# lh3/pangene

Measured on AMD Instinct MI355X. Metric: M PAF hits/sec through filter+overlap+graph, higher is better.
Workload: dtype int32

## Files before the change

### pangene_amd/csrc/hip/k_branch.hpp

```cpp
#pragma once

struct InWalkX { const uint32_t *flags; __device__ __forceinline__ I32 operator()(int64_t i) const { return I32{(flags[i] & (PGA_F_FLT | PGA_F_SHADOW)) ? 0 : 1}; } };
struct OutRank {
	int32_t *rx; const uint32_t *flags;
	__device__ __forceinline__ void operator()(int64_t i, I32, I32 ex) const
	{
		rx[i] = ex.v | ((flags[i] & F_CSTIE) ? (int32_t)0x80000000 : 0);
	}
};

constexpr int RK_T = 1024;
__device__ __forceinline__ void rank_genome_body(const uint32_t *flags, const int32_t *goff, int32_t *rx, const int g, int (*wtot)[RK_T / WAVE])
{
	const int h0 = goff[g], h1 = goff[g + 1], tid = threadIdx.x, lane = tid & 63, w = tid >> 6;
	const unsigned long long lt = lane == 0 ? 0ull : (~0ull >> (64 - lane));
	int carry = 0, par = 0;
	for (int base = h0; base < h1; base += RK_T, par ^= 1) {
		const int i = base + tid;
		const uint32_t f = i < h1 ? flags[i] : (uint32_t)PGA_F_FLT;
		const unsigned long long m = __ballot(!(f & (PGA_F_FLT | PGA_F_SHADOW)));
		if (lane == 0) wtot[par][w] = __popcll(m);
		__syncthreads();
		int pre = carry, tot = 0;
#pragma unroll
		for (int k = 0; k < RK_T / WAVE; ++k) { const int t = wtot[par][k]; tot += t; if (k < w) pre += t; }
		if (i < h1) rx[i] = (pre + __popcll(m & lt)) | ((f & F_CSTIE) ? (int32_t)0x80000000 : 0);
		carry += tot;
	}
}
constexpr int RK_CHUNK = 2048;
template <int NT>
__device__ __forceinline__ void rank_chunk_body(const uint32_t *flags, const int32_t *goff, int32_t *rx, const int g, const int k, int (*wtot)[NT / WAVE])
{
	const int h0 = goff[g], h1 = goff[g + 1], tid = threadIdx.x, lane = tid & 63, w = tid >> 6;
	const int64_t lo64 = (int64_t)h0 + (int64_t)k * RK_CHUNK;
	if (lo64 >= h1) return;
	const int lo = (int)lo64, hi = h1 - lo > RK_CHUNK ? lo + RK_CHUNK : h1;
	int cnt = 0;
	for (int i = h0 + tid; i < lo; i += NT) cnt += !(flags[i] & (PGA_F_FLT | PGA_F_SHADOW));
	cnt = wave_sum(cnt);
	if (lane == 0) wtot[0][w] = cnt;
	__syncthreads();
	int carry = 0;
#pragma unroll
	for (int q = 0; q < NT / WAVE; ++q) carry += wtot[0][q];
	const unsigned long long lt = lane == 0 ? 0ull : (~0ull >> (64 - lane));
	int par = 1;
	for (int base = lo; base < hi; base += NT, par ^= 1) {
		const int i = base + tid;
		const uint32_t f = i < hi ? flags[i] : (uint32_t)PGA_F_FLT;
		const unsigned long long m = __ballot(!(f & (PGA_F_FLT | PGA_F_SHADOW)));
		if (lane == 0) wtot[par][w] = __popcll(m);
		__syncthreads();
		int pre = carry, tot = 0;
#pragma unroll
		for (int q = 0; q < NT / WAVE; ++q) { const int t = wtot[par][q]; tot += t; if (q < w) pre += t; }
		if (i < hi) rx[i] = (pre + __popcll(m & lt)) | ((f & F_CSTIE) ? (int32_t)0x80000000 : 0);
		carry += tot;
	}
}

__global__ __launch_bounds__(RK_T) void k_rank_genome(const uint32_t *flags, const int32_t *goff, int32_t *rx, Gate gate)
{
	__shared__ int wtot[2][RK_T / WAVE];
	if (gate_closed(gate)) return;
	rank_genome_body(flags, goff, rx, blockIdx.x, wtot);
}

constexpr int RP_FULL = 0, RP_COMPACT = 1, RP_WIDE = 2;
__global__ __launch_bounds__(BLOCK) void k_tie_bounds(const int4 *A, const uint32_t *flags, int n, int2 *tg)
{
	const int x = blockIdx.x * BLOCK + threadIdx.x;
	if (x >= n || !(flags[x] & F_CSTIE)) return;
	const int4 ah = A[x];
	int ta = x, tb = x + 1;
	while (ta > 0) { const int4 ap = A[ta - 1]; if (ap.y != ah.y || ap.x != ah.x) break; --ta; }
	while (tb < n) { const int4 ap = A[tb]; if (ap.y != ah.y || ap.x != ah.x) break; ++tb; }
	tg[x] = make_int2(ta, tb);
}

struct RepFill {
	const int2 *tg;
	int64_t n_ent; int GL, Q, N , NZ ; const int32_t *zx, *zy, *zg; const int2 *zst; const int32_t *zoff; const uint32_t *hbk; uint32_t tag;
	const int4 *A; const int32_t *gid; const uint32_t *flags; const int32_t *rx, *goff, *ctg_base;
	void *rp_out; int32_t *iv; int64_t *dcnt; int32_t *hz_list;
	const int32_t *vfirst; const int64_t *vbase;
	Gate gate;
};

template <int FORM>
__device__ __forceinline__ void rep_absent(const RepFill &a, int64_t e0, int n)
{
	for (int k = 0; k < n; ++k) {
		if (FORM == RP_COMPACT) ((int2 *)a.rp_out)[e0 + k] = make_int2(0, -1); else ((int4 *)a.rp_out)[e0 + k] = make_int4(-1, 0, 0, 0);
	}
}
template <int FORM>
__global__ __launch_bounds__(BLOCK) void k_rep_clear(void *rp_out, int64_t n_ent, Gate gate)
{
	if (gate_closed(gate)) return;
	const int64_t e = (int64_t)blockIdx.x * BLOCK + threadIdx.x;
	if (e >= n_ent) return;
	if (FORM == RP_COMPACT) ((int2 *)rp_out)[e] = make_int2(0, -1); else ((int4 *)rp_out)[e] = make_int4(-1, 0, 0, 0);
}

template <int FORM, bool CLEARED>
__device__ __forceinline__ void rep_fill_body(const RepFill &a, const int t)
{
	if (!CLEARED && t < a.Q && a.zoff[t] == a.zoff[t + 1]) rep_absent<FORM>(a, (int64_t)t * a.GL, a.GL);
	if (t >= a.NZ) return;
	const int z = t;
	const int g = a.zg[z], y = a.zy[z] & 0x7fffffff, j = y >> 1;
	const bool has_n = z + 1 < a.NZ;
	const int gn = has_n ? a.zg[z + 1] : -1, yn = has_n ? (a.zy[z + 1] & 0x7fffffff) : 0;
	const uint32_t kb = a.hbk[z];
	if (gn == g && (yn >> 1) == j) return;
	const int z0 = a.zoff[g], gj = a.goff[j], cb = a.ctg_base[j], xz = a.zx[z];
	const int2 st_z = a.zst[z];
	const int64_t e = (int64_t)g * a.GL + j;
	if (!CLEARED) {
		int gs = z;
		while (gs > z0 && ((a.zy[gs - 1] & 0x7fffffff) >> 1) == j) --gs;
		if (gs == z0 && j > 0) rep_absent<FORM>(a, (int64_t)g * a.GL, j);
		const int jn = gn == g ? (yn >> 1) : a.GL;
		if (jn > j + 1) rep_absent<FORM>(a, e + 1, jn - j - 1);
	}
	int q = z;
	if (!hx_walk(kb, a.tag)) {
		q = z - 1;
		while (q >= z0 && ((a.zy[q] & 0x7fffffff) >> 1) == j && !hx_walk(a.hbk[q], a.tag)) --q;
		if (q < z0 || ((a.zy[q] & 0x7fffffff) >> 1) != j) { if (!CLEARED) rep_absent<FORM>(a, e, 1); return; }
	}
	const int h = q == z ? xz : a.zx[q];
	const int2 st = q == z ? st_z : a.zst[q];
	const int rxh = a.rx[h], r = (rxh & 0x7fffffff) - (a.rx[gj] & 0x7fffffff);
	int ivl = 0;
	if (rxh < 0) {
		const int hi = a.goff[j + 1];
		const int2 tgb = a.tg[h];
		const int ta = tgb.x, tb = tgb.y;
		const int re = tb < hi ? (a.rx[tb] & 0x7fffffff) : (a.rx[tb - 1] & 0x7fffffff) + ((a.flags[tb - 1] & (PGA_F_FLT | PGA_F_SHADOW)) ? 0 : 1);
		const int nb = (rxh & 0x7fffffff) - (a.rx[ta] & 0x7fffffff), na = re - (rxh & 0x7fffffff) - 1;
		if (nb + na > 0) {
			bool same_gene = false;
			for (int p = ta; p < tb; ++p) same_gene = same_gene || (p != h && a.gid[p] == g && !(a.flags[p] & (PGA_F_FLT | PGA_F_SHADOW)));
			if (same_gene || nb > 0xffff || na > 0xffff) {
				atomicAdd((unsigned long long *)&a.dcnt[6], 1ull);
				hz_note(&a.dcnt[14], a.hz_list, st.y);
			} else ivl = nb << 16 | na;
		}
	}
	const int cmw = st.x | (ivl ? (int)0x80000000 : 0);
	if (FORM == RP_COMPACT) {
		((int2 *)a.rp_out)[e] = make_int2(cmw, (st.y - cb) << 20 | r);
		if (ivl) a.iv[e] = ivl;
	} else if (FORM == RP_WIDE) {
		const long long cm64 = (long long)st.x + a.vbase[st.y];
		((int4 *)a.rp_out)[e] = make_int4(a.vfirst[st.y], r | (ivl ? (int)0x80000000 : 0), (int)(unsigned)(unsigned long long)cm64, (int)((unsigned long long)cm64 >> 32));
		if (ivl) a.iv[e] = ivl;
	} else ((int4 *)a.rp_out)[e] = make_int4(st.y, r, cmw, ivl);
}
template <int FORM, bool CLEARED>
__global__ __launch_bounds__(BLOCK) void k_rep_fill(RepFill a)
{
	if (gate_closed(a.gate)) return;
	rep_fill_body<FORM, CLEARED>(a, blockIdx.x * BLOCK + threadIdx.x);
}

struct NLocalHz { const int32_t *iv; const int32_t *ctg_base; int64_t *dcnt; int32_t *list; };

__device__ __noinline__ bool nl_hazard(const NLocalHz &z, int cc, int iv1, int iv2, int seg1, int seg2, int local_count)
{
	const int lo = cc - (iv1 >> 16) - (iv2 & 0xffff), hi = cc + (iv1 & 0xffff) + (iv2 >> 16);
	const bool all_in = lo >= -local_count && hi <= local_count, all_out = hi < -local_count || lo > local_count;
	if (all_in || all_out) return true;
	atomicAdd((unsigned long long *)&z.dcnt[6], 1ull);
	if (iv1) hz_note(&z.dcnt[14], z.list, seg1);
	if (iv2) hz_note(&z.dcnt[14], z.list, seg2);
	return false;
}

constexpr int nl_lanes_for(int GL) { return GL <= 256 ? 16 : GL <= 640 ? 32 : 64; }

template <int FORM, int NL_LANES>
__global__ __launch_bounds__(BLOCK) void k_n_local(const int32_t *pairs, int64_t n_cap, const int64_t *np_dev, int GL, const void *rp_in,
                                                     int local_dist, int local_count, int frag_mode, int32_t *cnt, NLocalHz hz, Gate gate)
{
	constexpr int NL_PAIRS = WAVE / NL_LANES;
	constexpr unsigned long long NL_MASK = NL_LANES == 64 ? ~0ull : ((1ull << (NL_LANES & 63)) - 1);
	if (gate_closed(gate)) return;
	const int lane = threadIdx.x & 63, grp = lane / NL_LANES, sub = lane & (NL_LANES - 1);
	int64_t n_pair = np_dev ? *np_dev : n_cap;
	if (n_pair > n_cap) return;
	const int64_t stride = (int64_t)gridDim.x * (BLOCK / WAVE) * NL_PAIRS;
	for (int64_t k0 = ((int64_t)blockIdx.x * (BLOCK / WAVE) + (threadIdx.x >> 6)) * NL_PAIRS; k0 < n_pair; k0 += stride) {
		const int64_t k = k0 + grp;
		const bool have = k < n_pair;
		const int64_t kk = have ? k : n_pair - 1;
		const int64_t g1 = (int64_t)pairs[2 * kk] * GL, g2 = (int64_t)pairs[2 * kk + 1] * GL;
		int c = 0;
		bool open = have;
		for (int j0 = 0; j0 < GL; j0 += NL_LANES) {
			if (__ballot(open) == 0) break;
			const int j = j0 + sub;
			const bool in = open && j < GL;
			const int jj = j < GL ? j : 0;
			bool hit = false, sure = false;
			if (FORM == RP_WIDE) {
				const int4 a = ((const int4 *)rp_in)[g1 + jj], b = ((const int4 *)rp_in)[g2 + jj];
				const long long d = (long long)((unsigned long long)(unsigned)a.w << 32 | (unsigned)a.z) - (long long)((unsigned long long)(unsigned)b.w << 32 | (unsigned)b.z);
				const int cc = (a.y & 0x7fffffff) - (b.y & 0x7fffffff);
				const bool cmp = in && a.x >= 0 && b.x >= 0 && (frag_mode || a.x == b.x);
				const bool near = d >= -(long long)local_dist && d <= (long long)local_dist;
				hit = cmp && (near || (cc >= -local_count && cc <= local_count));
				sure = hit;
				if (cmp && !near && (a.y | b.y) < 0) sure = nl_hazard(hz, cc, a.y < 0 ? hz.iv[g1 + jj] : 0, b.y < 0 ? hz.iv[g2 + jj] : 0, a.x, b.x, local_count) && hit;
			} else if (FORM == RP_COMPACT) {
				const int2 a = ((const int2 *)rp_in)[g1 + jj], b = ((const int2 *)rp_in)[g2 + jj];
				const int d = (a.x & 0x7fffffff) - (b.x & 0x7fffffff);
				const int cc = (a.y & 0xfffff) - (b.y & 0xfffff);
				const bool cmp = in && (a.y | b.y) >= 0 && (frag_mode || ((a.y ^ b.y) >> 20) == 0);
				const bool near = d >= -local_dist && d <= local_dist;
				hit = cmp && (near || (cc >= -local_count && cc <= local_count));
				sure = hit;
				if (cmp && !near && (a.x | b.x) < 0)
					sure = nl_hazard(hz, cc, a.x < 0 ? hz.iv[g1 + jj] : 0, b.x < 0 ? hz.iv[g2 + jj] : 0, hz.ctg_base[jj] + (a.y >> 20), hz.ctg_base[jj] + (b.y >> 20), local_count) && hit;
			} else {
				const int4 a = ((const int4 *)rp_in)[g1 + jj], b = ((const int4 *)rp_in)[g2 + jj];
				const int d = (a.z & 0x7fffffff) - (b.z & 0x7fffffff);
				const int cc = a.y - b.y;
				const bool cmp = in && a.x >= 0 && b.x >= 0 && (frag_mode || a.x == b.x);
				const bool near = d >= -local_dist && d <= local_dist;
				hit = cmp && (near || (cc >= -local_count && cc <= local_count));
				sure = hit;
				if (cmp && !near && (a.z | b.z) < 0) sure = nl_hazard(hz, cc, a.w, b.w, a.x, b.x, local_count) && hit;
			}
			const unsigned long long mh = __ballot(hit), ms = __ballot(sure);
			c += __popcll((mh >> (grp * NL_LANES)) & NL_MASK);
			if ((ms >> (grp * NL_LANES)) & NL_MASK) open = false;
		}
		if (have && sub == 0) cnt[k] = c;
	}
}

__global__ __launch_bounds__(BLOCK) void k_br_prep(const uint64_t *ax, int64_t n_arc, const int32_t *seg_gid, int32_t *agid, int32_t *vs, int32_t *ve)
{
	int64_t i = (int64_t)blockIdx.x * BLOCK + threadIdx.x;
	if (i >= n_arc) return;
	const uint64_t x = ax[i];
	const uint32_t v = (uint32_t)(x >> 32);
	agid[i] = seg_gid[(uint32_t)x >> 1];
	if (i == 0 || (uint32_t)(ax[i - 1] >> 32) != v) vs[v] = (int32_t)i;
	if (i == n_arc - 1 || (uint32_t)(ax[i + 1] >> 32) != v) ve[v] = (int32_t)i + 1;
}

__global__ __launch_bounds__(BLOCK) void k_seg_gid(const int32_t *g2s, int Q, int n_seg, int32_t *seg_gid)
{
	int g = blockIdx.x * BLOCK + threadIdx.x;
	if (g < Q) { int s = g2s[g]; if (s >= 0 && s < n_seg) seg_gid[s] = g; }
}

__global__ __launch_bounds__(BLOCK) void k_cur_prep(const pga_arc_part_t *arcs, int64_t n_arc, const int32_t *seg_gid, uint64_t *ax, int32_t *s1, int32_t *agid,
                                                      int32_t *vs, int32_t *ve)
{
	int64_t i = (int64_t)blockIdx.x * BLOCK + threadIdx.x;
	if (i >= n_arc) return;
	const pga_arc_part_t a = arcs[i];
	const uint32_t v = (uint32_t)(a.x >> 32);
	ax[i] = a.x;
	s1[i] = (int32_t)((double)a.sum_s1 / a.n_genome + .499);
	agid[i] = seg_gid[(uint32_t)a.x >> 1];
	if (i == 0 || (uint32_t)(arcs[i - 1].x >> 32) != v) vs[v] = (int32_t)i;
	if (i == n_arc - 1 || (uint32_t)(arcs[i + 1].x >> 32) != v) ve[v] = (int32_t)i + 1;
}

__global__ __launch_bounds__(BLOCK) void k_curx_table(const pga_arc_part_t *arcs, const int64_t *n_dev, int64_t cap, const int32_t *seg_gid, int n_vtx, uint64_t *ax, int32_t *s1, int32_t *agid, uint8_t *aw,
                                                        int32_t *vs, int32_t *ve, int32_t *deg, uint8_t *vwk)
{
	const int64_t i = (int64_t)blockIdx.x * BLOCK + threadIdx.x, n_arc = *n_dev;
	if (i >= n_arc) {
		if (i < cap) return;
		const int64_t u = (n_arc ? (int64_t)(uint32_t)(arcs[n_arc - 1].x >> 32) + 1 : 0) + (i - cap);
		if (u < n_vtx) vs[u] = 0, ve[u] = 0, deg[u] = 0, vwk[u] = 0;
		return;
	}
	const pga_arc_part_t a = arcs[i];
	const uint32_t v = (uint32_t)(a.x >> 32);
	ax[i] = a.x;
	s1[i] = (int32_t)((double)a.sum_s1 / a.n_genome + .499);
	agid[i] = seg_gid[(uint32_t)a.x >> 1];
	aw[i] = 0;
	const int64_t pv = i ? (int64_t)(uint32_t)(arcs[i - 1].x >> 32) : -1;
	if (pv == (int64_t)v) return;
	int64_t e = i + 1;
	while (e < n_arc && (uint32_t)(arcs[e].x >> 32) == v) ++e;
	vs[v] = (int32_t)i, ve[v] = (int32_t)e, deg[v] = (int32_t)(e - i), vwk[v] = 0;
	for (int64_t u = pv + 1; u < (int64_t)v; ++u) vs[u] = 0, ve[u] = 0, deg[u] = 0, vwk[u] = 0;
}

__global__ __launch_bounds__(BLOCK) void k_deg(const int32_t *vs, const int32_t *ve, int n_vtx, int32_t *deg)
{
	int v = blockIdx.x * BLOCK + threadIdx.x;
	if (v < n_vtx) deg[v] = ve[v] - vs[v];
}

__device__ __forceinline__ int br_count_one(const int v, const int32_t *vs, const int32_t *ve, const int32_t *s1, const double bd)
{
	const int a0 = vs[v], n = ve[v] - a0;
	if (n < 2) return 0;
	int max_s1 = 0, n_max = 0, n_weak = 0;
	for (int i = 0; i < n; ++i) max_s1 = max_s1 > s1[a0 + i] ? max_s1 : s1[a0 + i];
	for (int i = 0; i < n; ++i) {
		n_max += s1[a0 + i] == max_s1;
		n_weak += (1.0 - (double)s1[a0 + i] / max_s1) > bd;
	}
	return n_max * n_weak + n * (n - 1) / 2;
}
__global__ __launch_bounds__(BLOCK) void k_br_count(int n_vtx, const int32_t *vs, const int32_t *ve, const int32_t *s1, double bd, int32_t *pc, Gate gate)
{
	const int v = blockIdx.x * BLOCK + threadIdx.x;
	if (v >= n_vtx || gate_closed(gate)) return;
	pc[v] = br_count_one(v, vs, ve, s1, bd);
}

constexpr int PO_THREADS = 1024, PO_MAX_ITEMS = 64;
__global__ __launch_bounds__(PO_THREADS) void k_pair_offsets(const int32_t *pc, int n, int32_t *poff, int64_t *dcnt, int64_t *host_box, long long cap , Gate gate)
{
	__shared__ int32_t part[PO_THREADS];
	if (gate_closed(gate)) return;
	const int t = threadIdx.x, per = (n + PO_THREADS - 1) / PO_THREADS, i0 = t * per, i1 = i0 + per < n ? i0 + per : n;
	int32_t s = 0;
	for (int i = i0; i < i1; ++i) s += pc[i];
	part[t] = s;
	__syncthreads();
	for (int d = 1; d < PO_THREADS; d <<= 1) {
		const int32_t v = t >= d ? part[t - d] : 0;
		__syncthreads();
		part[t] += v;
		__syncthreads();
	}
	int32_t run = part[t] - s;
	for (int i = i0; i < i1; ++i) { poff[i] = run; run += pc[i]; }
	if (t == PO_THREADS - 1) { dcnt[15] = part[t]; if (cap >= 0 && part[t] > cap) { dcnt[11] = 1; if (part[t] > dcnt[16]) dcnt[16] = part[t]; } }
	__syncthreads();
	if (t < 16) sys_store(&host_box[t], dcnt[t]);
}

template <int MODE>
__device__ void br_vertex_seq(int a0, int n, const int32_t *s1, const int32_t *agid, double bd, int64_t k, int32_t *pairs, const int32_t *cnt,
                              double bdist, double bcut, uint8_t *weak, int32_t *grp, int32_t *ndl_out, int64_t *dcnt)
{
	int max_s1 = 0;
	for (int i = 0; i < n; ++i) max_s1 = max_s1 > s1[a0 + i] ? max_s1 : s1[a0 + i];
	for (int i = 0; i < n; ++i) {
		const double r = 1.0 - (double)s1[a0 + i] / max_s1;
		if (!(r > bd)) continue;
		int n_local = 0;
		for (int j = 0; j < n; ++j) {
			if (s1[a0 + j] != max_s1) continue;
			if (MODE == 1) pairs[2 * k] = agid[a0 + j], pairs[2 * k + 1] = agid[a0 + i];
			if (MODE == 2) n_local += cnt[k];
			++k;
		}
		if (MODE == 2) {
			weak[a0 + i] = ((n_local == 0 && r > bdist) || r > bcut) ? 2 : 1;
			if (dcnt) atomicAdd((unsigned long long *)&dcnt[weak[a0 + i] - 1], 1ull);
		}
	}
	int n_group = 0;
	for (int i = 0; i < n; ++i) {
		if (MODE == 2 && grp[a0 + i] == 0) grp[a0 + i] = ++n_group;
		for (int j = i + 1; j < n; ++j) {
			if (MODE == 1) pairs[2 * k] = agid[a0 + i], pairs[2 * k + 1] = agid[a0 + j];
			if (MODE == 2 && cnt[k] > 0 && grp[a0 + j] == 0) grp[a0 + j] = grp[a0 + i];
			++k;
		}
	}
	if (MODE == 2) *ndl_out = n_group;
}

constexpr int BR_WIDE_CAP = 2048;
template <int MODE>
__device__ void br_vertex_wide(const int lane, int a0, int n, const int32_t *s1, const int32_t *agid, double bd, int64_t k0, int32_t *pairs, const int32_t *cnt,
                               double bdist, double bcut, uint8_t *weak, uint16_t *grp , int32_t *ndl_out, int64_t *dcnt)
{
	const unsigned long long lt = lane == 0 ? 0ull : (~0ull >> (64 - lane));
	int max_s1 = 0;
	for (int c = 0; c < n; c += WAVE) { const int j = c + lane; const int v = j < n ? s1[a0 + j] : 0; max_s1 = max_s1 > v ? max_s1 : v; }
	max_s1 = wave_max(max_s1);
	int n_max = 0;
	for (int c = 0; c < n; c += WAVE) { const int j = c + lane; n_max += __popcll(__ballot(j < n && s1[a0 + j] == max_s1)); }
	int64_t k = k0;
	for (int ci = 0; ci < n; ci += WAVE) {
		const int ii = ci + lane;
		const double r_l = ii < n ? 1.0 - (double)s1[a0 + ii] / max_s1 : 0.0;
		unsigned long long m_weak = __ballot(ii < n && r_l > bd);
		for (; m_weak; m_weak &= m_weak - 1, k += n_max) {
			const int bit = __ffsll((long long)m_weak) - 1, i = ci + bit;
			const int gid_i = agid[a0 + i];
			bool any_local = false;
			int base = 0;
			for (int cj = 0; cj < n; cj += WAVE) {
				const int j = cj + lane;
				const bool is_max = j < n && s1[a0 + j] == max_s1;
				const unsigned long long mm = __ballot(is_max);
				const int64_t kk = k + base + __popcll(mm & lt);
				if (MODE == 1) { if (is_max) pairs[2 * kk] = agid[a0 + j], pairs[2 * kk + 1] = gid_i; }
				else any_local = any_local || __ballot(is_max && cnt[kk] != 0) != 0;
				base += __popcll(mm);
			}
			if (MODE == 2 && lane == bit) {
				const int wk = ((!any_local && r_l > bdist) || r_l > bcut) ? 2 : 1;
				weak[a0 + i] = (uint8_t)wk;
				if (dcnt) atomicAdd((unsigned long long *)&dcnt[wk - 1], 1ull);
			}
		}
	}
	if (MODE == 2) { for (int j = lane; j < n; j += WAVE) grp[j] = 0; wave_sync(); }
	int n_group = 0;
	for (int i = 0; i < n; ++i) {
		const int64_t row = k + (int64_t)i * n - (int64_t)i * (i + 1) / 2 - i - 1;
		if (MODE == 1) {
			const int gid_i = agid[a0 + i];
			for (int j = i + 1 + lane; j < n; j += WAVE) pairs[2 * (row + j)] = gid_i, pairs[2 * (row + j) + 1] = agid[a0 + j];
		} else {
			int gi = grp[i];
			if (gi == 0) { gi = ++n_group; if (lane == 0) grp[i] = (uint16_t)gi; }
			for (int j = i + 1 + lane; j < n; j += WAVE) if (grp[j] == 0 && cnt[row + j] > 0) grp[j] = (uint16_t)gi;
			wave_sync();
		}
	}
	if (MODE == 2 && lane == 0) *ndl_out = n_group;
}

template <int MODE>
__device__ __forceinline__ void br_wave_body(const int v, const int lane, uint16_t *s_grp , const int64_t k0 , const int32_t *vs, const int32_t *ve, const int32_t *s1g, const int32_t *agidg, double bd,
                                             int32_t *pairs, int64_t pair_cap, const int32_t *pcnt, const int32_t *cnt, double bdist, double bcut,
                                             uint8_t *weak, int32_t *grpg, int32_t *ndl, int64_t *dcnt, uint8_t *vwk)
{
	const int a0 = vs[v], n = ve[v] - a0;
	if (n < 2) { if (MODE == 2 && lane == 0) ndl[v] = 0; return; }
	if (MODE == 1 && k0 + pcnt[v] > pair_cap) return;
	if (n > WAVE && n <= BR_WIDE_CAP) {
		int32_t g = 0;
		br_vertex_wide<MODE>(lane, a0, n, s1g, agidg, bd, k0, pairs, cnt, bdist, bcut, weak, MODE == 2 ? s_grp + (threadIdx.x >> 6) * BR_WIDE_CAP : (uint16_t *)nullptr, &g, dcnt);
		if (MODE == 2 && lane == 0) ndl[v] = g, vwk[v] = 1;
		return;
	}
	if (n > WAVE) {
		if (lane == 0) {
			int32_t g = 0;
			if (MODE == 2) for (int i = 0; i < n; ++i) grpg[a0 + i] = 0;
			br_vertex_seq<MODE>(a0, n, s1g, agidg, bd, k0, pairs, cnt, bdist, bcut, weak, grpg, &g, dcnt);
			if (MODE == 2) ndl[v] = g, vwk[v] = 1;
		}
		return;
	}
	const bool in = lane < n;
	const int my_s1 = in ? s1g[a0 + lane] : 0, my_gid = in ? agidg[a0 + lane] : 0;
	const int max_s1 = wave_max(my_s1);
	const double r = in ? 1.0 - (double)my_s1 / max_s1 : 0.0;
	const bool is_weak = in && r > bd, is_max = in && my_s1 == max_s1;
	const unsigned long long m_weak = __ballot(is_weak), m_max = __ballot(is_max);
	if (MODE == 2 && lane == 0 && m_weak) vwk[v] = 1;
	const unsigned long long lt = lane == 0 ? 0ull : (~0ull >> (64 - lane));
	const int n_max = __popcll(m_max), mrank = __popcll(m_max & lt);
	int wb = 0;
	for (unsigned long long m = m_weak; m; m &= m - 1, ++wb) {
		const int i = __ffsll((long long)m) - 1;
		const int gid_i = __builtin_amdgcn_readlane(my_gid, i);
		const int64_t k = k0 + (int64_t)wb * n_max + mrank;
		if (MODE == 1) { if (is_max) pairs[2 * k] = my_gid, pairs[2 * k + 1] = gid_i; }
		else {
			const bool none_local = __ballot(is_max && cnt[k] != 0) == 0;
			if (lane == i) {
				const int wk = ((none_local && r > bdist) || r > bcut) ? 2 : 1;
				weak[a0 + i] = (uint8_t)wk;
				if (dcnt) atomicAdd((unsigned long long *)&dcnt[wk - 1], 1ull);
			}
		}
	}
	const int64_t k2 = k0 + (int64_t)n_max * __popcll(m_weak);
	int grp = 0, n_group = 0;
	for (int i = 0; i < n; ++i) {
		const int64_t k = k2 + (int64_t)i * n - (int64_t)i * (i + 1) / 2 + (lane - i - 1);
		if (MODE == 1) {
			const int gid_i = __builtin_amdgcn_readlane(my_gid, i);
			if (lane > i && in) pairs[2 * k] = gid_i, pairs[2 * k + 1] = my_gid;
		} else {
			int gi = __builtin_amdgcn_readlane(grp, i);
			if (gi == 0) { gi = ++n_group; if (lane == i) grp = gi; }
			if (lane > i && in && grp == 0 && cnt[k] > 0) grp = gi;
		}
	}
	if (MODE == 2 && lane == 0) ndl[v] = n_group;
}
template <int MODE>
__global__ __launch_bounds__(BLOCK) void k_br_wave(int n_vtx, const int32_t *vs, const int32_t *ve, const int32_t *s1g, const int32_t *agidg, double bd,
                                                     const int32_t *poff, int32_t *pairs, int64_t pair_cap , const int32_t *pcnt , const int32_t *cnt, double bdist, double bcut,
                                                     uint8_t *weak, int32_t *grpg, int32_t *ndl, int64_t *dcnt, uint8_t *vwk ,
                                                     const int64_t *np_dev = nullptr , Gate gate = Gate{nullptr, 0})
{
	__shared__ uint16_t s_grp[MODE == 2 ? (BLOCK / WAVE) * BR_WIDE_CAP : 1];
	const int v = blockIdx.x * (BLOCK / WAVE) + (threadIdx.x >> 6), lane = threadIdx.x & 63;
	if (v >= n_vtx || gate_closed(gate)) return;
	if (MODE == 2 && np_dev && *np_dev > pair_cap) return;
	br_wave_body<MODE>(v, lane, s_grp, poff[v], vs, ve, s1g, agidg, bd, pairs, pair_cap, pcnt, cnt, bdist, bcut, weak, grpg, ndl, dcnt, vwk);
}

struct LoopFront {
	int n_vtx, nbc, GL; const int32_t *vs, *ve, *s1; double bd; int32_t *pc, *poff, *btot;
	const uint32_t *flags; const int32_t *goff; int32_t *rx;
	void *rp_out; int64_t n_ent; int clear_bytes;
	Gate gate;
};
__global__ __launch_bounds__(RK_T) void k_loop_front1(LoopFront a)
{
	__shared__ int wtot[2][RK_T / WAVE];
	if (gate_closed(a.gate)) return;
	const int b = blockIdx.x, tid = threadIdx.x;
	if (b < a.nbc) {
		const int v = b * RK_T + tid, lane = tid & 63, w = tid >> 6;
		const int pc = v < a.n_vtx ? br_count_one(v, a.vs, a.ve, a.s1, a.bd) : 0;
		const I32 incl = wave_scan_incl(I32{pc}, OpSum{}, lane);
		if (lane == 63) wtot[0][w] = incl.v;
		__syncthreads();
		int pre = 0, tot = 0;
#pragma unroll
		for (int k = 0; k < RK_T / WAVE; ++k) { const int t = wtot[0][k]; tot += t; if (k < w) pre += t; }
		if (v < a.n_vtx) a.pc[v] = pc, a.poff[v] = pre + incl.v - pc;
		if (tid == 0) a.btot[b] = tot;
	} else if (b < a.nbc + a.GL) {
		rank_genome_body(a.flags, a.goff, a.rx, b - a.nbc, wtot);
	} else {
		const int64_t e = (int64_t)(b - a.nbc - a.GL) * RK_T + tid;
		if (e < a.n_ent) { if (a.clear_bytes == 8) ((int2 *)a.rp_out)[e] = make_int2(0, -1); else ((int4 *)a.rp_out)[e] = make_int4(-1, 0, 0, 0); }
	}
}
struct LoopFront2 {
	int nb_rep, n_vtx, nbc; const int32_t *vs, *ve, *s1, *agid; double bd; int32_t *poff; const int32_t *btot, *pc; int32_t *pairs; int64_t pair_cap; int64_t *dcnt;
};
template <int FORM, bool CLEARED>
__global__ __launch_bounds__(BLOCK) void k_loop_front2(RepFill rf, LoopFront2 a)
{
	if (gate_closed(rf.gate)) return;
	if ((int)blockIdx.x < a.nb_rep) { rep_fill_body<FORM, CLEARED>(rf, blockIdx.x * BLOCK + threadIdx.x); return; }
	const int v = (blockIdx.x - a.nb_rep) * (BLOCK / WAVE) + (threadIdx.x >> 6), lane = threadIdx.x & 63;
	if (v >= a.n_vtx) return;
	const int part = lane < a.nbc ? a.btot[lane] : 0, bv = v / RK_T;
	const int base = wave_sum(lane < bv ? part : 0);
	const int64_t k0 = (int64_t)base + a.poff[v];
	if (lane == 0) a.poff[v] = (int32_t)k0;
	if (v == 0) {
		const int tot = wave_sum(part);
		if (lane == 0) { a.dcnt[15] = tot; if (tot > a.pair_cap) { a.dcnt[11] = 1; if (tot > a.dcnt[16]) a.dcnt[16] = tot; } }
	}
	br_wave_body<1>(v, lane, nullptr, k0, a.vs, a.ve, a.s1, a.agid, a.bd, a.pairs, a.pair_cap, a.pc, nullptr, 0.0, 0.0, nullptr, nullptr, nullptr, a.dcnt, nullptr);
}

__global__ __launch_bounds__(BLOCK) void k_round_filter(int S, const int32_t *seg_cnt, const int32_t *deg, const int32_t *ndl, int max_tot_cnt, int max_degree, int max_dist_loci, uint8_t *del)
{
	const int s = blockIdx.x * BLOCK + threadIdx.x;
	if (s >= S) return;
	const int l0 = ndl[2 * s], l1 = ndl[2 * s + 1];
	del[s] = (seg_cnt[S + s] > max_tot_cnt || deg[2 * s] > max_degree || deg[2 * s + 1] > max_degree || (l0 > l1 ? l0 : l1) > max_dist_loci) ? 1 : 0;
}

__global__ __launch_bounds__(BLOCK) void k_round_del(int S, const int32_t *ndl, int max_tot_cnt, int max_degree, int max_dist_loci, const int32_t *seg_gid, int32_t *g2s, int32_t *vs, int32_t *ve, int32_t *deg, int32_t *seg_cnt, uint8_t *vwk, uint8_t *alive, int4 *gmeta ,
                 int32_t *stamp = nullptr , int round = 0)
{
	const int s = blockIdx.x * BLOCK + threadIdx.x;
	if (s >= S || !alive[s]) return;
	const int l0 = ndl[2 * s], l1 = ndl[2 * s + 1];
	if (!(seg_cnt[S + s] > max_tot_cnt || deg[2 * s] > max_degree || deg[2 * s + 1] > max_degree || (l0 > l1 ? l0 : l1) > max_dist_loci)) return;
	alive[s] = 0;
	if (stamp) stamp[0] = round;
	g2s[seg_gid[s]] = -1;
	vs[2 * s] = ve[2 * s] = vs[2 * s + 1] = ve[2 * s + 1] = 0;
	deg[2 * s] = deg[2 * s + 1] = 0;
	seg_cnt[s] = seg_cnt[S + s] = 0;
	vwk[2 * s] = vwk[2 * s + 1] = 0;
	if (gmeta) gmeta[s] = make_int4(0, 0, 0, 0);
}

__device__ __forceinline__ int arc_weak(const uint64_t *ax, const uint8_t *aw, int64_t n, uint64_t x)
{
	int64_t lo = 0, hi = n;
	while (lo < hi) { int64_t mid = (lo + hi) >> 1; if (ax[mid] < x) lo = mid + 1; else hi = mid; }
	return (lo < n && ax[lo] == x) ? aw[lo] : 0;
}

__device__ __forceinline__ int arc_weak_v(const uint64_t *ax, const uint8_t *aw, const int32_t *vs, const int32_t *ve, uint32_t v, uint32_t w)
{
	const int e = ve[v];
	for (int i = vs[v]; i < e; i += 4) {
		const uint32_t t0 = (uint32_t)ax[i], t1 = i + 1 < e ? (uint32_t)ax[i + 1] : ~0u, t2 = i + 2 < e ? (uint32_t)ax[i + 2] : ~0u, t3 = i + 3 < e ? (uint32_t)ax[i + 3] : ~0u;
		const int k = t0 == w ? 0 : t1 == w ? 1 : t2 == w ? 2 : t3 == w ? 3 : -1;
		if (k >= 0) return aw[i + k];
	}
	return 0;
}

__global__ __launch_bounds__(BLOCK) void k_mark_hits(const int32_t *val, const int32_t *prev, const int4 *YA, const int4 *YB, const int32_t *g2s, int n,
                                                       const uint64_t *ax, const uint8_t *aw, int64_t n_arc, const int32_t *vs, const int32_t *ve, const uint8_t *vwk, int32_t *weak_new)
{
	int y = blockIdx.x * BLOCK + threadIdx.x;
	if (y >= n || val[y] < 0) return;
	int p = prev[y];
	if (p < 0) return;
	const int4 aA = YA[y], bA = YA[p];
	if (aA.x != bA.x) return;
	const int aw_ = YB[y].w, bw_ = YB[p].w;
	uint32_t w = (uint32_t)g2s[aA.y] << 1 | (uint32_t)(aw_ & 1);
	uint32_t v = (uint32_t)g2s[bA.y] << 1 | (uint32_t)(bw_ & 1);
	if (vwk && !vwk[v] && !vwk[w ^ 1]) return;
	int e1 = vs ? arc_weak_v(ax, aw, vs, ve, v, w) : arc_weak(ax, aw, n_arc, (uint64_t)v << 32 | w);
	if (e1) atomicMax(&weak_new[bw_ >> 1], e1);
	int e2 = vs ? arc_weak_v(ax, aw, vs, ve, w ^ 1, v ^ 1) : arc_weak(ax, aw, n_arc, (uint64_t)(w ^ 1) << 32 | (v ^ 1));
	if (e2) atomicMax(&weak_new[aw_ >> 1], e2);
}

__global__ __launch_bounds__(BLOCK) void k_weak_merge(uint32_t *flags, const int32_t *weak_new, int n, int64_t *cnt)
{
	int h = blockIdx.x * BLOCK + threadIdx.x;
	const bool in = h < n;
	if (!in) h = n - 1;
	uint32_t f = flags[h];
	int cur = in ? (int)((f & PGA_F_WEAK_MASK) >> PGA_F_WEAK_SHIFT) : 0, nw = in ? weak_new[h] : 0;
	if (nw > cur) { cur = nw; flags[h] = (f & ~PGA_F_WEAK_MASK) | (uint32_t)nw << PGA_F_WEAK_SHIFT; }
	if (cnt) {
		const unsigned long long m = __ballot(cur != 0);
		if (m && (threadIdx.x & 63) == (unsigned)__ffsll((long long)m) - 1) atomicAdd((unsigned long long *)cnt, (unsigned long long)__popcll(m));
	}
}
```

### pangene_amd/csrc/hip/k_genes.hpp

```cpp
#pragma once


__global__ __launch_bounds__(BLOCK) void k_zkey(const int32_t *gid, int n, uint64_t *key, uint32_t *val)
{
	int h = blockIdx.x * BLOCK + threadIdx.x;
	if (h < n) key[h] = (uint64_t)(uint32_t)gid[h], val[h] = (uint32_t)h;
}

struct InLiveX { const uint32_t *flags; __device__ __forceinline__ I32 operator()(int64_t i) const { return I32{(flags[i] & PGA_F_FLT) ? 0 : 1}; } };
struct OutLiveX {
	uint32_t *flags; int32_t *lx; const int32_t *gid; uint64_t *key; uint32_t *val; int64_t n;
	__device__ __forceinline__ void operator()(int64_t i, I32 in, I32 ex) const
	{
		const uint32_t f = flags[i], nf = (f & PGA_F_FLT) ? (f & ~F_MEMBER) : (f | F_MEMBER);
		if (nf != f) flags[i] = nf;
		lx[i] = ex.v;
		if (!(f & PGA_F_FLT)) key[ex.v] = (uint64_t)(uint32_t)gid[i], val[ex.v] = (uint32_t)i;
		if (i == n - 1) lx[n] = in.v;
	}
};
struct InLiveY { const uint32_t *flags; const int32_t *yperm; __device__ __forceinline__ I32 operator()(int64_t y) const { return I32{(flags[yperm[y]] & PGA_F_FLT) ? 0 : 1}; } };
struct OutLiveY {
	const uint32_t *flags; const int32_t *yperm; int32_t *ylist;
	__device__ __forceinline__ void operator()(int64_t y, I32, I32 ex) const { const int x = yperm[y]; if (!(flags[x] & PGA_F_FLT)) ylist[ex.v] = x; }
};
__global__ __launch_bounds__(BLOCK) void k_live_records(const uint32_t *flags, const int32_t *lx, const int4 *A, const int4 *B, const int4 *C, int n, int4 *cA, int4 *cB, int4 *cC, int32_t *cx)
{
	const int x = blockIdx.x * BLOCK + threadIdx.x;
	if (x >= n || !(flags[x] & F_MEMBER)) return;
	const int i = lx[x];
	cA[i] = A[x], cB[i] = B[x], cC[i] = C[x], cx[i] = x;
}
__global__ __launch_bounds__(BLOCK) void k_ovl_records(const int32_t *ov_pos, const int32_t *lpos, int64_t t, const int4 *A, const int4 *B, const int4 *C, int4 *cA, int4 *cB, int4 *cC, int32_t *cx)
{
	const int64_t k = (int64_t)blockIdx.x * BLOCK + threadIdx.x;
	if (k >= t || lpos[k] < 0) return;
	const int i = lpos[k], x = ov_pos[k];
	cA[i] = A[x], cB[i] = B[x], cC[i] = C[x], cx[i] = x;
}
struct InSegMaxListL { const int4 *A; const int32_t *lpos; __device__ __forceinline__ SegMax operator()(int64_t i) const { const int p = lpos[i]; if (p < 0) return SegMax{SEG_EMPTY, 0}; const int4 a = A[p]; return SegMax{a.y, a.z}; } };
struct OutSegMaxListL { int4 *A; const int32_t *lpos; __device__ __forceinline__ void operator()(int64_t i, SegMax in, SegMax) const { const int p = lpos[i]; if (p >= 0) ((int32_t *)&A[p])[3] = in.v; } };

__global__ void k_mail_live(const int32_t *lx, int64_t n, int64_t *dcnt, int64_t *host_box)
{
	if (threadIdx.x == 0) dcnt[10] = lx[n];
	__syncthreads();
	if (threadIdx.x < 16) sys_store(&host_box[threadIdx.x], dcnt[threadIdx.x]);
}

struct ZIndex { int32_t *zx, *zy, *zg; int2 *zst; int32_t *zpos; };
__global__ __launch_bounds__(BLOCK) void k_zrec(const uint32_t *perm, const uint64_t *ks, const int32_t *ctg_base, int n_genome, const uint32_t *flags, const int32_t *cm, const int32_t *seg, int n, ZIndex o)
{
	const int z = blockIdx.x * BLOCK + threadIdx.x, lane = threadIdx.x & 63;
	const bool v = z < n;
	const int x = v ? (int)perm[z] : 0;
	const int sg = v ? seg[x] : 0;
	const int gn = v ? genome_of(ctg_base, n_genome, sg) : -1;
	const unsigned long long kz = v ? ks[z] : ~0ull;
	int gn_p = __shfl_up(gn, 1, WAVE), gn_n = __shfl_down(gn, 1, WAVE);
	unsigned long long k_p = (unsigned long long)(unsigned)__shfl_up((int)(unsigned)(kz >> 32), 1, WAVE) << 32 | (unsigned)__shfl_up((int)(unsigned)kz, 1, WAVE);
	unsigned long long k_n = (unsigned long long)(unsigned)__shfl_down((int)(unsigned)(kz >> 32), 1, WAVE) << 32 | (unsigned)__shfl_down((int)(unsigned)kz, 1, WAVE);
	if (lane == 0) { const bool h = v && z > 0; k_p = h ? ks[z - 1] : ~0ull; gn_p = h ? genome_of(ctg_base, n_genome, seg[(int)perm[z - 1]]) : -1; }
	if (lane == 63) { const bool h = v && z + 1 < n; k_n = h ? ks[z + 1] : ~0ull; gn_n = h ? genome_of(ctg_base, n_genome, seg[(int)perm[z + 1]]) : -1; }
	if (!v) return;
	const bool grp_prev = z > 0 && k_p == kz && gn_p == gn, grp_next = z + 1 < n && k_n == kz && gn_n == gn;
	o.zx[z] = x, o.zg[z] = (int)kz;
	o.zy[z] = gn << 1 | ((flags[x] & PGA_F_REV) ? 1 : 0) | ((grp_prev || grp_next) ? 0 : (int)0x80000000);
	o.zst[z] = make_int2(cm[x], sg);
	o.zpos[x] = z;
}

__global__ __launch_bounds__(BLOCK) void k_zoff(const uint64_t *ks, int n, int Q, int32_t *zoff)
{
	int g = blockIdx.x * BLOCK + threadIdx.x;
	if (g > Q) return;
	int lo = 0, hi = n;
	while (lo < hi) { const int mid = (lo + hi) >> 1; if (ks[mid] < (uint64_t)g) lo = mid + 1; else hi = mid; }
	zoff[g] = lo;
}

struct WrecSrc { const int32_t *yperm, *seg, *gid, *cm, *sori, *sdom, *pdom0, *prot_gid; const uint32_t *flags; const int32_t *zpos; const int32_t *vfirst; const int64_t *vbase; };
__device__ __forceinline__ void pack_wrec_one(const WrecSrc &s, int64_t y, int4 *W)
{
	const int a = s.yperm[y], p0 = s.pdom0[a];
	int sg = s.seg[a], cmv = s.cm[a];
	if (s.vfirst) { cmv = (int)(unsigned)((unsigned long long)s.vbase[sg] + (unsigned long long)(long long)cmv); sg = s.vfirst[sg]; }
	W[2 * y] = make_int4(sg, s.gid[a] << 1 | ((s.flags[a] & PGA_F_REV) ? 1 : 0), cmv, s.sori[a]);
	W[2 * y + 1] = make_int4(s.sdom[a], p0 < 0 ? -1 : s.prot_gid[p0], s.zpos[a], 0);
}
__global__ __launch_bounds__(BLOCK) void k_pack_wrec(WrecSrc s, int n, int4 *W)
{
	const int y = blockIdx.x * BLOCK + threadIdx.x;
	if (y < n) pack_wrec_one(s, y, W);
}
__global__ __launch_bounds__(BLOCK) void k_pack_wrec_list(WrecSrc s, const int32_t *pos, int64_t T, int4 *W)
{
	const int64_t t = (int64_t)blockIdx.x * BLOCK + threadIdx.x;
	if (t < T && pos[t] >= 0) pack_wrec_one(s, pos[t], W);
}

constexpr int WK_FEW_FROM = 1 << 25;
struct Walk {
	const uint32_t *__restrict__ flags; const int32_t *__restrict__ yperm; const int4 *__restrict__ W; const int32_t *__restrict__ g2s;
	uint32_t *__restrict__ hfk, *__restrict__ hbk; int4 *__restrict__ hfp, *__restrict__ hbp;
	uint32_t tag; int ori; int n; int64_t *dcnt; int32_t *hz_list; Gate gate;
};
__device__ __forceinline__ int walk_score(const int4 w0, const int4 w1, int ori, const int32_t *g2s)
{
	return (ori || w0.w > w1.x || w1.y < 0 || g2s[w1.y] >= 0) ? w0.w : w1.x;
}
struct WalkRide { int n_ride, GL, cpg; const int32_t *goff; int32_t *rx; void *rp_out; int64_t n_clear; int clear_bytes; };
template <int WK_IPT>
__global__ __launch_bounds__(BLOCK) void k_walk(Walk a, WalkRide rd)
{
	constexpr int WK_TILE = BLOCK * WK_IPT;
	__shared__ int32_t s_wave[BLOCK / WAVE], s_carry;
	if (gate_closed(a.gate)) return;
	if ((int)blockIdx.x < rd.n_ride) {
		__shared__ int wtot[2][BLOCK / WAVE];
		const int b = (int)blockIdx.x;
		if (b < rd.GL * rd.cpg) rank_chunk_body<BLOCK>(a.flags, rd.goff, rd.rx, b / rd.cpg, b % rd.cpg, wtot);
		else {
			const int64_t e = (int64_t)(b - rd.GL * rd.cpg) * BLOCK + threadIdx.x;
			if (e < rd.n_clear) { if (rd.clear_bytes == 8) ((int2 *)rd.rp_out)[e] = make_int2(0, -1); else ((int4 *)rd.rp_out)[e] = make_int4(-1, 0, 0, 0); }
		}
		return;
	}
	const int tid = threadIdx.x, lane = tid & 63, w = tid >> 6;
	const int64_t tile0 = (int64_t)((int)blockIdx.x - rd.n_ride) * WK_TILE, base = tile0 + (int64_t)tid * WK_IPT;
	int mark[WK_IPT];
#pragma unroll
	for (int k = 0; k < WK_IPT; ++k) { const int64_t i = base + k; mark[k] = (i < a.n && !(a.flags[a.yperm[i]] & (PGA_F_FLT | PGA_F_SHADOW))) ? (int)i : -1; }
	if (w == 0) {
		int carry = -1;
		for (int64_t j0 = tile0 - 1; j0 >= 0 && carry < 0; j0 -= 64) {
			const int64_t j = j0 - lane;
			const bool ok = j >= 0 && !(a.flags[a.yperm[j]] & (PGA_F_FLT | PGA_F_SHADOW));
			const unsigned long long mk = __ballot(ok);
			if (mk) carry = (int)(j0 - (__ffsll((long long)mk) - 1));
		}
		if (lane == 0) s_carry = carry;
	}
	int t_max = mark[0];
#pragma unroll
	for (int k = 1; k < WK_IPT; ++k) t_max = t_max > mark[k] ? t_max : mark[k];
	I32 incl = wave_scan_incl(I32{t_max}, OpMax{}, lane);
	if (lane == 63) s_wave[w] = incl.v;
	__syncthreads();
	int run = s_carry;
	for (int k = 0; k < w; ++k) run = run > s_wave[k] ? run : s_wave[k];
	{ const int pv = incl.shfl_up(1).v; if (lane > 0) run = run > pv ? run : pv; }
	int prev[WK_IPT];
#pragma unroll
	for (int k = 0; k < WK_IPT; ++k) { prev[k] = run; run = mark[k] >= 0 ? mark[k] : run; }
	int4 A0[WK_IPT], A1[WK_IPT], B0[WK_IPT], B1[WK_IPT];
#pragma unroll
	for (int k = 0; k < WK_IPT; ++k) {
		const int i = mark[k] >= 0 ? mark[k] : 0, pp = prev[k] >= 0 ? prev[k] : i;
		if (mark[k] >= 0) A0[k] = a.W[2 * (int64_t)i], A1[k] = a.W[2 * (int64_t)i + 1], B0[k] = a.W[2 * (int64_t)pp], B1[k] = a.W[2 * (int64_t)pp + 1];
	}
	int SA[WK_IPT], SB[WK_IPT];
#pragma unroll
	for (int k = 0; k < WK_IPT; ++k)
		if (mark[k] >= 0 && prev[k] >= 0 && B0[k].x == A0[k].x) SA[k] = walk_score(A0[k], A1[k], a.ori, a.g2s), SB[k] = walk_score(B0[k], B1[k], a.ori, a.g2s);
#pragma unroll
	for (int k = 0; k < WK_IPT; ++k) {
		if (mark[k] < 0) continue;
		const int p = prev[k];
		const int4 a0 = A0[k], a1 = A1[k], b0 = B0[k], b1 = B1[k];
		const int zi = a1.z, zp = b1.z;
		uint32_t key = a.tag << HA_TAG_SHIFT | HA_NONE;
		if (p >= 0 && b0.x == a0.x) {
			const uint32_t wv = (uint32_t)a0.y, v = (uint32_t)b0.y;
			const int sa = SA[k], sb = SB[k], d = (int)((unsigned)a0.z - (unsigned)b0.z);
			if (a0.z == b0.z) { atomicAdd((unsigned long long *)&a.dcnt[5], 1ull); hz_note(&a.dcnt[14], a.hz_list, a0.x); }
			a.hfk[zp] = a.tag << HA_TAG_SHIFT | wv, a.hfp[zp] = make_int4(d, sb, sa, 0);
			key = a.tag << HA_TAG_SHIFT | (v ^ 1u), a.hbp[zi] = make_int4(d, sa, sb, 0);
		}
		a.hbk[zi] = key;
	}
}

__global__ __launch_bounds__(BLOCK) void k_walk_list(Walk a, const int32_t *pos, int64_t T)
{
	const int64_t t = (int64_t)blockIdx.x * BLOCK + threadIdx.x;
	if (t >= T) return;
	const int i = pos[t];
	if (i < 0) return;
	auto walkable = [&](int y) { return !(a.flags[a.yperm[y]] & (PGA_F_FLT | PGA_F_SHADOW)); };
	const int4 a0 = a.W[2 * (int64_t)i], a1 = a.W[2 * (int64_t)i + 1];
	const int zi = a1.z;
	if (!walkable(i)) { a.hbk[zi] = 0, a.hfk[zi] = 0; return; }
	int p = -1, q = -1;
	for (int j = i - 1; j >= 0; --j) { if (a.W[2 * (int64_t)j].x != a0.x) break; if (walkable(j)) { p = j; break; } }
	for (int j = i + 1; j < a.n; ++j) { if (a.W[2 * (int64_t)j].x != a0.x) break; if (walkable(j)) { q = j; break; } }
	const int sa = walk_score(a0, a1, a.ori, a.g2s);
	uint32_t key = a.tag << HA_TAG_SHIFT | HA_NONE;
	if (p >= 0) {
		const int4 b0 = a.W[2 * (int64_t)p], b1 = a.W[2 * (int64_t)p + 1];
		const int sb = walk_score(b0, b1, a.ori, a.g2s), d = (int)((unsigned)a0.z - (unsigned)b0.z);
		if (a0.z == b0.z) { atomicAdd((unsigned long long *)&a.dcnt[5], 1ull); hz_note(&a.dcnt[14], a.hz_list, a0.x); }
		key = a.tag << HA_TAG_SHIFT | ((uint32_t)b0.y ^ 1u), a.hbp[zi] = make_int4(d, sa, sb, 0);
	}
	a.hbk[zi] = key;
	if (q >= 0) {
		const int4 c0 = a.W[2 * (int64_t)q], c1 = a.W[2 * (int64_t)q + 1];
		const int sc = walk_score(c0, c1, a.ori, a.g2s), d = (int)((unsigned)c0.z - (unsigned)a0.z);
		a.hfk[zi] = a.tag << HA_TAG_SHIFT | (uint32_t)c0.y, a.hfp[zi] = make_int4(d, sa, sc, 0);
	} else a.hfk[zi] = 0;
}

constexpr int GA_CAP_WAVE = 128, GA_CAP = 512;
constexpr int GA_WAVE_HITS = 512;
constexpr int GA_BIG_STAGE = 2048;

struct GeneArcs {
	const int32_t *zy; const int32_t *zoff; const uint32_t *hfk, *hbk; const int4 *hfp, *hbp; const int32_t *g2s;
	int Q, S; uint32_t tag; int cap_log2;
	int32_t *seg_cnt, *seg_gid;
	pga_arc_part_t *stage; int4 *gmeta;
	uint64_t *ax; int32_t *s1, *agid; uint8_t *aw; int32_t *vs, *ve, *deg; uint8_t *vwk;
	int32_t *h_round;
	int32_t *big_list;
	int32_t *big_ctl;
	int64_t *dcnt;
	Gate gate; int32_t *tag_out;
};


template <int CAP, int STAGE> struct GeneTable {
	uint32_t key[CAP]; int32_t ng[CAP], tot[CAP]; unsigned long long sd[CAP], s1[CAP], s2[CAP]; uint16_t dense[CAP];
	int32_t zy[STAGE]; uint32_t fx[STAGE], bx[STAGE];
	int n_tot, n_gen, over, m, m0, base;
};

template <int CAP, int STAGE> struct GeneWin {
	const GeneArcs &a; const GeneTable<CAP, STAGE> &T; int lo, hi;
	__device__ __forceinline__ int zy(int z) const { return ((z >= lo && z < hi) ? T.zy[z - lo] : a.zy[z]) & 0x7fffffff; }
	__device__ __forceinline__ uint32_t fx(int z) const { return (z >= lo && z < hi) ? T.fx[z - lo] : a.hfk[z]; }
	__device__ __forceinline__ uint32_t bx(int z) const { return (z >= lo && z < hi) ? T.bx[z - lo] : a.hbk[z]; }
};

template <int CAP, class Table>
__device__ __forceinline__ bool ga_flush(Table &T, int cap, int cap_log2, uint32_t key, int ng, int tot, unsigned long long sd, unsigned long long s1, unsigned long long s2)
{
	uint32_t slot = (key * 2654435761u) >> (32 - cap_log2);
	int probes = 0;
	for (; probes < cap; ++probes, slot = (slot + 1) & (cap - 1)) {
		const uint32_t old = atomicCAS(&T.key[slot], 0xffffffffu, key);
		if (old == 0xffffffffu || old == key) break;
	}
	if (probes == cap) return false;
	atomicAdd(&T.ng[slot], ng); atomicAdd(&T.tot[slot], tot);
	atomicAdd(&T.sd[slot], sd); atomicAdd(&T.s1[slot], s1); atomicAdd(&T.s2[slot], s2);
	return true;
}

template <int NT, int CAP, int STAGE>
__device__ __forceinline__ bool gene_arcs_one(const GeneArcs &a, GeneTable<CAP, STAGE> &T, const int g, const int sid, const int tid, const int cap_log2)
{
	constexpr int HALO = STAGE >= 1024 ? 32 : 0;
	const int z0 = a.zoff[g], z1 = a.zoff[g + 1], cap = 1 << cap_log2;
	for (int k = tid; k < cap; k += NT) T.key[k] = 0xffffffffu, T.ng[k] = 0, T.tot[k] = 0, T.sd[k] = 0, T.s1[k] = 0, T.s2[k] = 0;
	if (tid == 0) T.n_tot = 0, T.n_gen = 0, T.over = 0, T.m = 0, T.m0 = 0;
	int n_tot = 0, n_gen = 0;
	uint32_t pk[2] = { 0xffffffffu, 0xffffffffu };
	int png[2] = { 0, 0 }, ptot[2] = { 0, 0 };
	unsigned long long psd[2] = { 0, 0 }, ps1[2] = { 0, 0 }, ps2[2] = { 0, 0 };
	for (int c0 = z0; c0 < z1; c0 += STAGE - 2 * HALO) {
		const int c1 = c0 + (STAGE - 2 * HALO) < z1 ? c0 + (STAGE - 2 * HALO) : z1;
		GeneWin<CAP, STAGE> W = { a, T, c0 - HALO > z0 ? c0 - HALO : z0, c1 + HALO < z1 ? c1 + HALO : z1 };
		if (NT == 64) wave_sync(); else __syncthreads();
		for (int z = W.lo + tid; z < W.hi; z += NT) T.zy[z - W.lo] = a.zy[z], T.fx[z - W.lo] = a.hfk[z], T.bx[z - W.lo] = a.hbk[z];
		if (NT == 64) wave_sync(); else __syncthreads();
		for (int z = c0 + tid; z < c1; z += NT) {
			if (!hx_walk(T.bx[z - W.lo], a.tag)) continue;
			const int zyw = T.zy[z - W.lo], zy = zyw & 0x7fffffff, genome = zy >> 1, rev = zy & 1;
			int gs = z, ge = z + 1;
			bool first = true;
			if (zyw >= 0) {
				while (gs > z0 && (W.zy(gs - 1) >> 1) == genome) --gs;
				while (ge < z1 && (W.zy(ge) >> 1) == genome) ++ge;
				for (int q = gs; q < z; ++q) first = first && !hx_walk(W.bx(q), a.tag);
			}
			n_tot += 1, n_gen += first ? 1 : 0;
#pragma unroll
			for (int dir = 0; dir < 2; ++dir) {
				const uint32_t hx = dir ? T.bx[z - W.lo] : T.fx[z - W.lo];
				if (!hx_valid(hx, a.tag)) continue;
				const uint32_t key = (uint32_t)(dir ? !rev : rev) << HA_TAG_SHIFT | (hx & HA_NONE);
				bool leader = true;
				int n = 1;
				for (int q = gs; q < ge && leader && ge - gs > 1; ++q) {
					if (q == z) continue;
					const int rq = W.zy(q) & 1;
#pragma unroll
					for (int d2 = 0; d2 < 2; ++d2) {
						const uint32_t ox = d2 ? W.bx(q) : W.fx(q);
						if (!hx_valid(ox, a.tag) || ((uint32_t)(d2 ? !rq : rq) << HA_TAG_SHIFT | (ox & HA_NONE)) != key) continue;
						if (q < z) { leader = false; break; }
						++n;
					}
				}
				if (!leader) continue;
				const int4 h = dir ? a.hbp[z] : a.hfp[z];
				int m1 = h.y, m2 = h.z;
				unsigned long long sd = (unsigned long long)(long long)h.x;
				if (n > 1)
					for (int q = z + 1; q < ge; ++q) {
						const int rq = W.zy(q) & 1;
#pragma unroll
						for (int d2 = 0; d2 < 2; ++d2) {
							const uint32_t ox = d2 ? W.bx(q) : W.fx(q);
							if (!hx_valid(ox, a.tag) || ((uint32_t)(d2 ? !rq : rq) << HA_TAG_SHIFT | (ox & HA_NONE)) != key) continue;
							const int4 o = d2 ? a.hbp[q] : a.hfp[q];
							sd += (unsigned long long)(long long)o.x, m1 = m1 > o.y ? m1 : o.y, m2 = m2 > o.z ? m2 : o.z;
						}
					}
				m1 = m1 > 0 ? m1 : 0, m2 = m2 > 0 ? m2 : 0;
				const int dg = cvt_i32_x86((double)sd / n + .499);
				if (key != pk[dir]) {
					if (pk[dir] != 0xffffffffu && !ga_flush<CAP>(T, cap, cap_log2, pk[dir], png[dir], ptot[dir], psd[dir], ps1[dir], ps2[dir])) T.over = 1;
					pk[dir] = key, png[dir] = 0, ptot[dir] = 0, psd[dir] = 0, ps1[dir] = 0, ps2[dir] = 0;
				}
				png[dir] += 1, ptot[dir] += n;
				psd[dir] += (unsigned long long)(long long)dg * (unsigned long long)n;
				ps1[dir] += (unsigned long long)(long long)m1, ps2[dir] += (unsigned long long)(long long)m2;
			}
		}
	}
#pragma unroll
	for (int dir = 0; dir < 2; ++dir)
		if (pk[dir] != 0xffffffffu && !ga_flush<CAP>(T, cap, cap_log2, pk[dir], png[dir], ptot[dir], psd[dir], ps1[dir], ps2[dir])) T.over = 1;
	{
		const int wt = wave_sum(n_tot), wg = wave_sum(n_gen);
		if ((tid & 63) == 0) { if (NT == 64) T.n_tot = wt, T.n_gen = wg; else atomicAdd(&T.n_tot, wt), atomicAdd(&T.n_gen, wg); }
	}
	if (NT == 64) wave_sync(); else __syncthreads();
	if (T.over) return false;
	for (int k = tid; k < cap; k += NT)
		if (T.key[k] != 0xffffffffu) { const int at = atomicAdd(&T.m, 1); T.dense[at] = (uint16_t)k; if (!(T.key[k] >> HA_TAG_SHIFT)) atomicAdd(&T.m0, 1); }
	if (NT == 64) wave_sync(); else __syncthreads();
	const int m = T.m;
	if (tid == 0) {
		const int b = 2 * z0, m0 = T.m0;
		T.base = b;
		a.seg_cnt[sid] = T.n_gen, a.seg_cnt[a.S + sid] = T.n_tot, a.seg_gid[sid] = g;
		a.gmeta[sid] = make_int4(b, m0, m - m0, 0);
		a.vs[2 * sid] = b, a.ve[2 * sid] = b + m0, a.vs[2 * sid + 1] = b + m0, a.ve[2 * sid + 1] = b + m;
		a.deg[2 * sid] = m0, a.deg[2 * sid + 1] = m - m0;
		a.vwk[2 * sid] = 0, a.vwk[2 * sid + 1] = 0;
		if (a.h_round) {
			a.h_round[sid] = T.n_gen, a.h_round[a.S + sid] = T.n_tot;
			a.h_round[2 * a.S + 2 * sid] = m0, a.h_round[2 * a.S + 2 * sid + 1] = m - m0;
		}
	}
	if (NT == 64) wave_sync(); else __syncthreads();
	for (int e = tid; e < m; e += NT) {
		const int k = T.dense[e];
		const uint32_t key = T.key[k];
		int r = 0;
		for (int j = 0; j < m; ++j) r += T.key[T.dense[j]] < key;
		pga_arc_part_t o;
		const uint32_t t = key & HA_NONE;
		o.x = (uint64_t)((uint32_t)sid << 1 | (key >> HA_TAG_SHIFT)) << 32 | (uint32_t)((uint32_t)a.g2s[t >> 1] << 1 | (t & 1u));
		o.n_genome = T.ng[k], o.tot_cnt = T.tot[k], o.sum_dist = T.sd[k], o.sum_s1 = (int64_t)T.s1[k], o.sum_s2 = (int64_t)T.s2[k];
		const int at = T.base + r;
		a.stage[at] = o;
		a.ax[at] = o.x;
		a.s1[at] = (int32_t)((double)o.sum_s1 / o.n_genome + .499);
		a.agid[at] = (int32_t)(t >> 1);
		a.aw[at] = 0;
	}
	return true;
}

constexpr int GA_WAVE_NT = 128;
template <int NT, int CAP, int HITS, int CAP_LOG2>
__global__ __launch_bounds__(NT) __attribute__((amdgpu_waves_per_eu(7))) void k_gene_arcs_wave_t(GeneArcs a, RepFill rf, int ride_form)
{
	__shared__ GeneTable<CAP, HITS> T;
	if (gate_closed(a.gate)) return;
	if ((int)blockIdx.x >= a.Q) {
		const int t = ((int)blockIdx.x - a.Q) * NT + (int)threadIdx.x;
		switch (ride_form) {
		case RP_FULL * 2: rep_fill_body<RP_FULL, false>(rf, t); break;
		case RP_FULL * 2 + 1: rep_fill_body<RP_FULL, true>(rf, t); break;
		case RP_COMPACT * 2: rep_fill_body<RP_COMPACT, false>(rf, t); break;
		case RP_COMPACT * 2 + 1: rep_fill_body<RP_COMPACT, true>(rf, t); break;
		case RP_WIDE * 2: rep_fill_body<RP_WIDE, false>(rf, t); break;
		case RP_WIDE * 2 + 1: rep_fill_body<RP_WIDE, true>(rf, t); break;
		}
		return;
	}
	const int g = blockIdx.x, tid = threadIdx.x;
	const int sid = a.g2s[g], z0 = a.zoff[g], z1 = a.zoff[g + 1];
	if (sid < 0) {
		for (int z = z0 + tid; z < z1; z += NT)
			if (hx_walk(a.hbk[z], a.tag)) atomicAdd((unsigned long long *)&a.dcnt[3], 1ull), a.dcnt[11] = 1;
		return;
	}
	const int cl = a.cap_log2 < CAP_LOG2 ? a.cap_log2 : CAP_LOG2;
	const bool done = z1 - z0 <= HITS && gene_arcs_one<NT, CAP, HITS>(a, T, g, sid, tid, cl);
	if (tid == 0 && !done) a.big_list[atomicAdd(&a.big_ctl[0], 1)] = g;
}

constexpr int GA_BIG_NT = 512;
__global__ __launch_bounds__(GA_BIG_NT) __attribute__((amdgpu_waves_per_eu(6))) void k_gene_arcs_big(GeneArcs a)
{
	__shared__ GeneTable<GA_CAP, GA_BIG_STAGE> T;
	if (gate_closed(a.gate)) return;
	if (a.tag_out && blockIdx.x == 0 && threadIdx.x == 0) *a.tag_out = (int32_t)a.tag;
	__shared__ int s_next;
	const int n_big = a.big_ctl[0];
	for (int at = blockIdx.x; at < n_big; ) {
		const int g = a.big_list[at];
		const int sid = a.g2s[g];
		if (!gene_arcs_one<GA_BIG_NT, GA_CAP, GA_BIG_STAGE>(a, T, g, sid, threadIdx.x, a.cap_log2) && threadIdx.x == 0)
			atomicAdd((unsigned long long *)&a.dcnt[9], 1ull), a.dcnt[11] = 1, a.gmeta[sid] = make_int4(0, 0, 0, 0);
		if (threadIdx.x == 0) s_next = (int)gridDim.x + atomicAdd(&a.big_ctl[1], 1);
		__syncthreads();
		at = s_next;
		__syncthreads();
	}
}

struct InGmeta { const int4 *gm; __device__ __forceinline__ I32 operator()(int64_t i) const { const int4 m = gm[i]; return I32{m.y + m.z}; } };

__global__ __launch_bounds__(BLOCK) void k_arc_compact(const int4 *gmeta, const int32_t *off, int S, const pga_arc_part_t *stage, pga_arc_part_t *arcs, int64_t *dcnt, int64_t *host_box)
{
	const int lane = threadIdx.x & 63;
	for (int sid = blockIdx.x * (BLOCK / WAVE) + (threadIdx.x >> 6); sid < S; sid += gridDim.x * (BLOCK / WAVE)) {
		const int4 m = gmeta[sid];
		const int o = off[sid], n = m.y + m.z;
		for (int i = lane; i < n; i += WAVE) arcs[o + i] = stage[m.x + i];
		if (lane == 0 && sid == S - 1) {
			dcnt[10] = o + n;
			for (int t = 0; t < 16; ++t) sys_store(&host_box[t], dcnt[t]);
		}
	}
}

struct I32x2 {
	int32_t a, b;
	__device__ __forceinline__ I32x2 shfl_up(int d) const { return I32x2{__shfl_up(a, d, WAVE), __shfl_up(b, d, WAVE)}; }
	__device__ __forceinline__ I32x2 shfl(int l) const { return I32x2{__shfl(a, l, WAVE), __shfl(b, l, WAVE)}; }
};
struct OpSum2 { __device__ __forceinline__ I32x2 operator()(I32x2 x, I32x2 y) const { return I32x2{x.a + y.a, x.b + y.b}; } };
struct InAliveGmeta { const uint8_t *alive; const int4 *gm; __device__ __forceinline__ I32x2 operator()(int64_t i) const { const int4 m = gm[i]; return I32x2{alive[i] != 0, m.y + m.z}; } };
struct OutExclI32x2 { int32_t *pa, *pb; __device__ __forceinline__ void operator()(int64_t i, I32x2, I32x2 ex) const { pa[i] = ex.a, pb[i] = ex.b; } };

__device__ __forceinline__ int4 arc_final_lo(uint64_t x, const pga_arc_part_t &p) { return make_int4((int32_t)(uint32_t)x, (int32_t)(uint32_t)(x >> 32), p.n_genome, p.tot_cnt); }
__device__ __forceinline__ int4 arc_final_hi(const pga_arc_part_t &p)
{
	return make_int4(cvt_i64lo_x86((double)(int64_t)p.sum_dist / p.tot_cnt + .499), cvt_i32_x86((double)p.sum_s1 / p.n_genome + .499), cvt_i32_x86((double)p.sum_s2 / p.n_genome + .499), 0);
}

__global__ __launch_bounds__(BLOCK) void k_arc_final(const int4 *gmeta, const int32_t *off, const int32_t *newid, int S, const pga_arc_part_t *stage, int4 *out, int64_t cap, int64_t *dcnt)
{
	const int lane = threadIdx.x & 63;
	const int4 ml = gmeta[S - 1];
	const int64_t total = (int64_t)off[S - 1] + ml.y + ml.z;
	if (blockIdx.x == 0 && threadIdx.x == 0) dcnt[10] = total;
	if (total > cap) return;
	for (int sid = blockIdx.x * (BLOCK / WAVE) + (threadIdx.x >> 6); sid < S; sid += gridDim.x * (BLOCK / WAVE)) {
		const int4 m = gmeta[sid];
		const int o = off[sid], n = m.y + m.z;
		for (int i = lane; i < n; i += WAVE) {
			const pga_arc_part_t p = stage[m.x + i];
			const uint32_t v = (uint32_t)(p.x >> 32), w = (uint32_t)p.x;
			const uint32_t sv = v >> 1, sw = w >> 1;
			const uint64_t x = (uint64_t)((uint32_t)(sv < (uint32_t)S ? newid[sv] : 0) << 1 | (v & 1u)) << 32 | ((uint32_t)(sw < (uint32_t)S ? newid[sw] : 0) << 1 | (w & 1u));
			out[2 * (size_t)(o + i)] = arc_final_lo(x, p);
			out[2 * (size_t)(o + i) + 1] = arc_final_hi(p);
		}
	}
}

__global__ void k_arc_final_probe(const pga_arc_part_t *in, int64_t n, int4 *out)
{
	const int64_t i = (int64_t)blockIdx.x * BLOCK + threadIdx.x;
	if (i < n) out[i] = arc_final_hi(in[i]);
}

__global__ __launch_bounds__(BLOCK) void k_xs_compact(const int4 *gmeta, const int32_t *off, int S, const pga_arc_part_t *stage, const int32_t *seg_cnt, int32_t *slot, int64_t arc_cap, const int64_t *dcnt, Gate gate = Gate{nullptr, 0},
                                                        const int32_t *stamp = nullptr , int round = 0)
{
	if (blockIdx.x == 0 && threadIdx.x == 0) slot[3] = (stamp && stamp[1] == round) ? 1 : 0;
	if (gate_closed(gate)) return;
	const int lane = threadIdx.x & 63;
	int32_t *segc = slot + XS_HDR;
	pga_arc_part_t *arcs = (pga_arc_part_t *)(slot + XS_HDR + xs_seg_words(S));
	for (int sid = blockIdx.x * (BLOCK / WAVE) + (threadIdx.x >> 6); sid < S; sid += gridDim.x * (BLOCK / WAVE)) {
		const int4 m = gmeta[sid];
		const int o = off[sid], n = m.y + m.z;
		if ((int64_t)o + n <= arc_cap)
			for (int i = lane; i < n; i += WAVE) arcs[o + i] = stage[m.x + i];
		if (lane == 0) {
			segc[sid] = seg_cnt[sid], segc[S + sid] = seg_cnt[S + sid];
			if (sid == S - 1) { slot[0] = o + n, slot[1] = dcnt[9] != 0, slot[2] = dcnt[3] != 0; for (int t = 4; t < XS_HDR; ++t) slot[t] = 0; }
		}
	}
}

__global__ __launch_bounds__(BLOCK) void k_mark_hits_z(const int32_t *zx, const int32_t *zy, const int32_t *zg, const uint32_t *hfk, const uint32_t *hbk, uint32_t tag, int n, const int32_t *g2s,
                                                        const uint64_t *ax, const uint8_t *aw, const int32_t *vs, const int32_t *ve, const uint8_t *vwk,
                                                        uint32_t *flags, int64_t *cnt, int then_filter, Gate gate, int32_t *stamp , int round)
{
	int z = blockIdx.x * BLOCK + threadIdx.x;
	bool marked = false;
	if (gate_closed(gate)) return;
	if (z < n) {
		const uint32_t kb = hbk[z], kf = hfk[z];
		const int y = zy[z], g = zg[z];
		if (hx_walk(kb, tag)) {
			const int sid = g2s[g], rev = y & 1;
			int nw = 0;
#pragma unroll
			for (int dir = 0; dir < 2; ++dir) {
				const uint32_t h = dir ? kb : kf;
				if (!hx_valid(h, tag) || sid < 0) continue;
				const uint32_t u = (uint32_t)sid << 1 | (uint32_t)(dir ? !rev : rev), t = h & HA_NONE;
				if (!vwk[u]) continue;
				const uint32_t w = (uint32_t)g2s[t >> 1] << 1 | (t & 1u);
				const int e = arc_weak_v(ax, aw, vs, ve, u, w);
				nw = nw > e ? nw : e;
			}
			if (nw) {
				const int x = zx[z];
				const uint32_t f = flags[x];
				if (nw > (int)((f & PGA_F_WEAK_MASK) >> PGA_F_WEAK_SHIFT)) {
					flags[x] = (f & ~PGA_F_WEAK_MASK) | (uint32_t)nw << PGA_F_WEAK_SHIFT | ((then_filter && nw == 2) ? PGA_F_FLT : 0u);
					if (stamp) stamp[1] = round;
				}
				marked = true;
			}
		}
		if (cnt && !marked) marked = (flags[zx[z]] & PGA_F_WEAK_MASK) != 0;
	}
	if (cnt) {
		const unsigned long long mk = __ballot(marked);
		if (mk && (threadIdx.x & 63) == (unsigned)__ffsll((long long)mk) - 1) atomicAdd((unsigned long long *)cnt, (unsigned long long)__popcll(mk));
	}
}
```

### pangene_amd/csrc/hip/pga_host_branch.hpp

```cpp
#pragma once


struct RepDefer { bool on; RepFill rf; int32_t *rx; unsigned nb; bool cleared; int rode; };

static int rep_pos_impl(pga_ctx *c, RepDefer *df)
{
	const int N = c->N, GL = c->n_genome, Q = c->Q;
	if (df) df->on = false, df->rode = 0;
	const int64_t n_ent = (int64_t)Q * GL;
	RepFill rf; int32_t *rx;
	TRY(rep_fill_args(c, &rf, &rx));
	int4 *rp = (int4 *)rf.rp_out;
	if (N) {
		I32 *tile = (I32 *)c->pool.get(S_TILE, tile_buf_bytes(N));
		if (!tile) return PGA_ERR_NOMEM;
		const int want = c->ride_want;
		c->ride_want = 0;
		TRY(ensure_half_arcs(c, c->ha_ori < 0 ? 0 : c->ha_ori));
		c->ride_want = want;
		TRY(rep_fill_args(c, &rf, &rx));
		static const bool rank_scan = env_has("PANGENE_RANK", "scan");
		const bool defer = df && c->gs_np <= (1 << 15) && !rank_scan;
		const int rode = (defer && c->in_loop && c->ride_done && c->ride_tag == c->round_tag && c->tg_valid) ? c->ride_done : 0;
		if (defer) ;
		else if (c->gs_np <= (1 << 15) && !rank_scan) hipLaunchKernelGGL(k_rank_genome, dim3((unsigned)GL), dim3(RK_T), 0, c->st, (const uint32_t *)c->flags, (const int32_t *)c->goff, rx, c->gate);
		else device_scan<I32>(InWalkX{c->flags}, OutRank{rx, c->flags}, N, tile, OpSum{}, I32{0}, c->st, c->gate);
		if (!c->tg_valid) { hipLaunchKernelGGL(k_tie_bounds, dim3(nblk(N)), dim3(BLOCK), 0, c->st, (const int4 *)c->recA, (const uint32_t *)c->flags, N, c->tg); c->tg_valid = true; }
		if (defer) { df->on = true, df->rf = rf, df->rx = rx, df->cleared = c->live_on, df->nb = nblk(c->live_on ? std::max(c->NL, 1) : std::max(c->NL, Q)), df->rode = rode; return 0; }
		if (c->live_on) {
			const unsigned nb = nblk(std::max(c->NL, 1));
			if (c->rp_form == RP_COMPACT) {
				if (n_ent) hipLaunchKernelGGL((k_rep_clear<RP_COMPACT>), dim3(nblk(n_ent)), dim3(BLOCK), 0, c->st, (void *)rp, n_ent, c->gate);
				hipLaunchKernelGGL((k_rep_fill<RP_COMPACT, true>), dim3(nb), dim3(BLOCK), 0, c->st, rf);
			} else {
				if (n_ent) hipLaunchKernelGGL((k_rep_clear<RP_FULL>), dim3(nblk(n_ent)), dim3(BLOCK), 0, c->st, (void *)rp, n_ent, c->gate);
				if (c->rp_form == RP_WIDE) hipLaunchKernelGGL((k_rep_fill<RP_WIDE, true>), dim3(nb), dim3(BLOCK), 0, c->st, rf);
				else hipLaunchKernelGGL((k_rep_fill<RP_FULL, true>), dim3(nb), dim3(BLOCK), 0, c->st, rf);
			}
		} else {
			const unsigned nb = nblk(std::max(c->NL, Q));
			if (c->rp_form == RP_COMPACT) hipLaunchKernelGGL((k_rep_fill<RP_COMPACT, false>), dim3(nb), dim3(BLOCK), 0, c->st, rf);
			else if (c->rp_form == RP_WIDE) hipLaunchKernelGGL((k_rep_fill<RP_WIDE, false>), dim3(nb), dim3(BLOCK), 0, c->st, rf);
			else hipLaunchKernelGGL((k_rep_fill<RP_FULL, false>), dim3(nb), dim3(BLOCK), 0, c->st, rf);
		}
	} else if (n_ent) {
		hipLaunchKernelGGL(k_fill_i32, dim3(nblk(4 * n_ent)), dim3(BLOCK), 0, c->st, (int32_t *)rp, 4 * n_ent, -1);
	}
	return 0;
}

extern "C" int pga_rep_pos(pga_ctx_t *c) { return rep_pos_impl(c, nullptr); }

static int n_local_dev(pga_ctx *c, const int32_t *d_pairs, int64_t n, const int64_t *np_dev, int32_t local_dist, int32_t local_count, int32_t frag_mode, int32_t **cnt)
{
	int32_t *d_cnt = (int32_t *)c->pool.get(S_NLCNT, sizeof(int32_t) * (size_t)n + 16);
	int4 *rp = (int4 *)c->pool.get(S_RP_SEG, 0);
	if (!d_cnt || !rp) return PGA_ERR_NOMEM;
	*cnt = d_cnt;
	NLocalHz hz = { (const int32_t *)c->pool.get(S_RP_IV, 0), c->ctg_base, c->dcnt, (int32_t *)c->pool.get(S_HZLIST, sizeof(int32_t) * PGA_HAZARD_CAP) };
	if (!hz.iv || !hz.list) return PGA_ERR_NOMEM;
	const int64_t est = np_dev ? (c->br_np_seen > 0 ? c->br_np_seen : std::min<int64_t>(n, 1 << 18)) : n;
	static const int lanes_env = [] { const char *e = getenv("PANGENE_NL_LANES"); return e ? atoi(e) : 0; }();
	const int lanes = (lanes_env == 16 || lanes_env == 32 || lanes_env == 64) ? lanes_env : nl_lanes_for(c->n_genome);
	const unsigned grid = (unsigned)std::max<int64_t>(1, std::min<int64_t>(nblk(est, BLOCK / WAVE * (WAVE / lanes)), 1 << 20));
#define NL_LAUNCH(FORM, LANES) hipLaunchKernelGGL((k_n_local<FORM, LANES>), dim3(grid), dim3(BLOCK), 0, c->st, d_pairs, n, np_dev, c->n_genome, (const void *)rp, local_dist, local_count, frag_mode, d_cnt, hz, c->gate)
#define NL_FORM(FORM) do { if (lanes == 16) NL_LAUNCH(FORM, 16); else if (lanes == 32) NL_LAUNCH(FORM, 32); else NL_LAUNCH(FORM, 64); } while (0)
	if (n && c->rp_form == RP_COMPACT) NL_FORM(RP_COMPACT);
	else if (n && c->rp_form == RP_WIDE) NL_FORM(RP_WIDE);
	else if (n) NL_FORM(RP_FULL);
#undef NL_FORM
#undef NL_LAUNCH
	return 0;
}

extern "C" int pga_n_local(pga_ctx_t *c, const int32_t *pairs, int64_t n, int32_t local_dist, int32_t local_count, int32_t frag_mode, int32_t **cnt)
{
	int32_t *d_pairs = (int32_t *)c->pool.get(S_PAIRS, sizeof(int32_t) * 2 * (size_t)n + 16);
	if (!d_pairs) return PGA_ERR_NOMEM;
	if (n) TRY(upload(c, d_pairs, pairs, 2 * (size_t)n));
	TRY(n_local_dev(c, d_pairs, n, nullptr, local_dist, local_count, frag_mode, cnt));
	return sync_st(c);
}

static inline bool loop_cap_forced(const pga_ctx *c) { static const bool on = getenv("PANGENE_LOOP_PAIR_CAP") != nullptr; return on && c->in_loop && !c->loop_room_given; }
static inline size_t loop_btot_at(int n_vtx) { return ((size_t)n_vtx + 7) & ~(size_t)3; }

static void rep_launch_deferred(pga_ctx *c, const RepDefer &d)
{
	const RepFill &rf = d.rf;
	if (d.rode >= 2) return;
	if (d.rode == 0) hipLaunchKernelGGL(k_rank_genome, dim3((unsigned)rf.GL), dim3(RK_T), 0, c->st, rf.flags, rf.goff, d.rx, rf.gate);
	const int form = c->rp_form;
	if (d.cleared) {
		if (d.rode) ;
		else if (rf.n_ent && form == RP_COMPACT) hipLaunchKernelGGL((k_rep_clear<RP_COMPACT>), dim3(nblk(rf.n_ent)), dim3(BLOCK), 0, c->st, rf.rp_out, rf.n_ent, rf.gate);
		else if (rf.n_ent) hipLaunchKernelGGL((k_rep_clear<RP_FULL>), dim3(nblk(rf.n_ent)), dim3(BLOCK), 0, c->st, rf.rp_out, rf.n_ent, rf.gate);
		if (form == RP_COMPACT) hipLaunchKernelGGL((k_rep_fill<RP_COMPACT, true>), dim3(d.nb), dim3(BLOCK), 0, c->st, rf);
		else if (form == RP_WIDE) hipLaunchKernelGGL((k_rep_fill<RP_WIDE, true>), dim3(d.nb), dim3(BLOCK), 0, c->st, rf);
		else hipLaunchKernelGGL((k_rep_fill<RP_FULL, true>), dim3(d.nb), dim3(BLOCK), 0, c->st, rf);
	} else {
		if (form == RP_COMPACT) hipLaunchKernelGGL((k_rep_fill<RP_COMPACT, false>), dim3(d.nb), dim3(BLOCK), 0, c->st, rf);
		else if (form == RP_WIDE) hipLaunchKernelGGL((k_rep_fill<RP_WIDE, false>), dim3(d.nb), dim3(BLOCK), 0, c->st, rf);
		else hipLaunchKernelGGL((k_rep_fill<RP_FULL, false>), dim3(d.nb), dim3(BLOCK), 0, c->st, rf);
	}
}

static int branch_enumerate(pga_ctx *c, int32_t **cnt, const RepDefer *df = nullptr)
{
	const int n_vtx = 2 * c->br_S;
	int32_t *s1 = (int32_t *)c->pool.get(S_BR_S1, 0), *agid = (int32_t *)c->pool.get(S_BR_GID, 0), *vs = (int32_t *)c->pool.get(S_BR_VS, 0), *ve = (int32_t *)c->pool.get(S_BR_VE, 0);
	int32_t *poff = (int32_t *)c->pool.get(S_BR_POFF, 0);
	int32_t *pairs = (int32_t *)c->pool.get(S_PAIRS, sizeof(int32_t) * 2 * (size_t)c->br_cap + 16);
	if (!pairs || !s1 || !agid || !vs || !ve || !poff) return PGA_ERR_NOMEM;
	if (df) {
		const int32_t *pc = (const int32_t *)c->pool.get(S_BR_PC, 0);
		const unsigned nb_rep = df->rode >= 2 ? 0u : df->nb;
		const LoopFront2 a = { (int)nb_rep, n_vtx, (n_vtx + RK_T - 1) / RK_T, vs, ve, s1, agid, c->br_par.diff, poff, pc + loop_btot_at(n_vtx), pc, pairs, c->br_cap, c->dcnt };
		const dim3 grid(nb_rep + nblk(n_vtx, BLOCK / WAVE));
		const int form = c->rp_form;
		if (df->cleared) {
			if (form == RP_COMPACT) hipLaunchKernelGGL((k_loop_front2<RP_COMPACT, true>), grid, dim3(BLOCK), 0, c->st, df->rf, a);
			else if (form == RP_WIDE) hipLaunchKernelGGL((k_loop_front2<RP_WIDE, true>), grid, dim3(BLOCK), 0, c->st, df->rf, a);
			else hipLaunchKernelGGL((k_loop_front2<RP_FULL, true>), grid, dim3(BLOCK), 0, c->st, df->rf, a);
		} else {
			if (form == RP_COMPACT) hipLaunchKernelGGL((k_loop_front2<RP_COMPACT, false>), grid, dim3(BLOCK), 0, c->st, df->rf, a);
			else if (form == RP_WIDE) hipLaunchKernelGGL((k_loop_front2<RP_WIDE, false>), grid, dim3(BLOCK), 0, c->st, df->rf, a);
			else hipLaunchKernelGGL((k_loop_front2<RP_FULL, false>), grid, dim3(BLOCK), 0, c->st, df->rf, a);
		}
	} else
	hipLaunchKernelGGL((k_br_wave<1>), dim3(nblk(n_vtx, BLOCK / WAVE)), dim3(BLOCK), 0, c->st, n_vtx, vs, ve, s1, agid, c->br_par.diff, poff, pairs, c->br_cap, (const int32_t *)c->pool.get(S_BR_PC, 0),
	                   (const int32_t *)nullptr, 0.0, 0.0, (uint8_t *)nullptr, (int32_t *)nullptr, (int32_t *)nullptr, c->dcnt, (uint8_t *)nullptr, (const int64_t *)nullptr, c->gate);
	return n_local_dev(c, pairs, c->br_cap, c->dcnt + 15, c->br_par.local_dist, c->br_par.local_count, c->br_par.frag_mode, cnt);
}

static int branch_pairs_impl(pga_ctx *c, const uint64_t *arc_x, const int32_t *arc_s1, int64_t n_arc, const int32_t *seg_gid, int32_t n_seg,
                             double branch_diff, int32_t local_dist, int32_t local_count, int32_t frag_mode, int32_t **cnt, int64_t *n_pairs, const RepDefer *df)
{
	if (arc_x == nullptr) n_arc = c->br_n, n_seg = c->br_S;
	const int n_vtx = 2 * n_seg;
	uint64_t *ax = (uint64_t *)c->pool.get(S_ARCX, sizeof(uint64_t) * (size_t)n_arc + 16);
	uint8_t *aw = (uint8_t *)c->pool.get(S_ARCW, (size_t)n_arc + 16);
	int32_t *s1 = (int32_t *)c->pool.get(S_BR_S1, sizeof(int32_t) * (size_t)n_arc + 16), *agid = (int32_t *)c->pool.get(S_BR_GID, sizeof(int32_t) * (size_t)n_arc + 16);
	int32_t *vs = (int32_t *)c->pool.get(S_BR_VS, sizeof(int32_t) * (size_t)n_vtx + 16), *ve = (int32_t *)c->pool.get(S_BR_VE, sizeof(int32_t) * (size_t)n_vtx + 16);
	int32_t *pc = (int32_t *)c->pool.get(S_BR_PC, sizeof(int32_t) * (loop_btot_at(n_vtx) + 64) + 16), *poff = (int32_t *)c->pool.get(S_BR_POFF, sizeof(int32_t) * (size_t)n_vtx + 16);
	int32_t *sg = (int32_t *)c->pool.get(S_BR_SEGGID, sizeof(int32_t) * (size_t)n_seg + 16);
	if (!ax || !aw || !s1 || !agid || !vs || !ve || !pc || !poff || !sg) return PGA_ERR_NOMEM;
	c->br_n = n_arc, c->br_S = n_seg, c->br_np = -1;
	c->br_par.diff = branch_diff, c->br_par.local_dist = local_dist, c->br_par.local_count = local_count, c->br_par.frag_mode = frag_mode;
	if (n_pairs) *n_pairs = 0;
	*cnt = (int32_t *)c->pool.get(S_NLCNT, 16);
	if (df && !df->on) df = nullptr;
	if (n_arc == 0 || n_vtx == 0) { if (df) rep_launch_deferred(c, *df); c->br_np = 0; return sync_st(c); }
	if (arc_x) {
		TRY(upload(c, ax, arc_x, (size_t)n_arc)); TRY(upload(c, s1, arc_s1, (size_t)n_arc)); TRY(upload(c, sg, seg_gid, (size_t)n_seg));
		HIPCHK(hipMemsetAsync(vs, 0, sizeof(int32_t) * (size_t)n_vtx, c->st)); HIPCHK(hipMemsetAsync(ve, 0, sizeof(int32_t) * (size_t)n_vtx, c->st));
		hipLaunchKernelGGL(k_br_prep, dim3(nblk(n_arc)), dim3(BLOCK), 0, c->st, ax, n_arc, sg, agid, vs, ve);
		HIPCHK(hipMemsetAsync(aw, 0, (size_t)n_arc, c->st));
	}
	static const bool general_scan = getenv("PANGENE_PAIR_SCAN_GENERAL") != nullptr;
	const bool one_wg = n_vtx <= PO_THREADS * PO_MAX_ITEMS && !general_scan;
	if (df && !(one_wg && n_pairs == nullptr)) { rep_launch_deferred(c, *df); df = nullptr; }
	if (df) {
		const int nbc = (n_vtx + RK_T - 1) / RK_T;
		const RepFill &rf = df->rf;
		const int64_t n_clear = (df->cleared && !df->rode) ? rf.n_ent : 0;
		const int gl = df->rode ? 0 : rf.GL;
		const LoopFront a = { n_vtx, nbc, gl, vs, ve, s1, branch_diff, pc, poff, pc + loop_btot_at(n_vtx), rf.flags, rf.goff, df->rx, rf.rp_out, n_clear, c->rp_form == RP_COMPACT ? 8 : 16, c->gate };
		hipLaunchKernelGGL(k_loop_front1, dim3((unsigned)(nbc + gl + (n_clear + RK_T - 1) / RK_T)), dim3(RK_T), 0, c->st, a);
		if (c->br_cap < 4 * (int64_t)n_vtx && !loop_cap_forced(c)) c->br_cap = 4 * (int64_t)n_vtx;
		return branch_enumerate(c, cnt, df);
	}
	hipLaunchKernelGGL(k_br_count, dim3(nblk(n_vtx)), dim3(BLOCK), 0, c->st, n_vtx, vs, ve, s1, branch_diff, pc, c->gate);
	if (one_wg) hipLaunchKernelGGL(k_pair_offsets, dim3(1), dim3(PO_THREADS), 0, c->st, (const int32_t *)pc, n_vtx, poff, c->dcnt, c->h_box, n_pairs ? -1ll : loop_cap_forced(c) ? (long long)c->br_cap : (long long)std::max<int64_t>(c->br_cap, 4 * (int64_t)n_vtx), c->gate);
	else {
		I32 *tile = (I32 *)c->pool.get(S_TILE, tile_buf_bytes(n_vtx));
		device_scan<I32>(InI32{pc}, OutExclI32{poff}, n_vtx, tile, OpSum{}, I32{0}, c->st, c->gate);
		hipLaunchKernelGGL(k_mail_pairs, dim3(1), dim3(64), 0, c->st, poff + (n_vtx - 1), pc + (n_vtx - 1), c->dcnt, c->h_box);
	}
	if (n_pairs) {
		TRY(sync_st(c));
		c->br_np = c->h_cnt[15], *n_pairs = c->br_np;
		c->br_cap = std::max<int64_t>(c->br_cap, std::max<int64_t>(c->br_np, 16));
		return c->br_np ? branch_enumerate(c, cnt) : 0;
	}
	if (c->br_cap < 4 * (int64_t)n_vtx && !loop_cap_forced(c)) c->br_cap = 4 * (int64_t)n_vtx;
	return branch_enumerate(c, cnt);
}

extern "C" int pga_branch_pairs(pga_ctx_t *c, const uint64_t *arc_x, const int32_t *arc_s1, int64_t n_arc, const int32_t *seg_gid, int32_t n_seg,
                                double branch_diff, int32_t local_dist, int32_t local_count, int32_t frag_mode, int32_t **cnt, int64_t *n_pairs)
{
	return branch_pairs_impl(c, arc_x, arc_s1, n_arc, seg_gid, n_seg, branch_diff, local_dist, local_count, frag_mode, cnt, n_pairs, nullptr);
}

struct RoundFilter { int on; int32_t max_tot_cnt, max_degree, max_dist_loci; uint8_t *del_host; };

static int decide_impl(pga_ctx *c, double branch_diff, double branch_diff_dist, double branch_diff_cut, uint8_t *arc_weak,
                       int32_t *n_dist_loci, int64_t *n_flt1, int64_t *n_flt2, const RoundFilter *rf)
{
	const int n_vtx = 2 * c->br_S, S = c->br_S;
	const int64_t n_arc = c->br_n;
	if (n_flt1) *n_flt1 = 0;
	if (n_flt2) *n_flt2 = 0;
	if (n_arc == 0 || n_vtx == 0) {
		if (n_vtx && n_dist_loci) memset(n_dist_loci, 0, sizeof(int32_t) * (size_t)n_vtx);
		if (rf && rf->on && S) memset(rf->del_host, 0, (size_t)S);
		return rf ? sync_st(c) : 0;
	}
	uint8_t *aw = (uint8_t *)c->pool.get(S_ARCW, 0);
	int32_t *s1 = (int32_t *)c->pool.get(S_BR_S1, 0), *agid = (int32_t *)c->pool.get(S_BR_GID, 0), *vs = (int32_t *)c->pool.get(S_BR_VS, 0), *ve = (int32_t *)c->pool.get(S_BR_VE, 0);
	int32_t *poff = (int32_t *)c->pool.get(S_BR_POFF, 0);
	int32_t *grp = (int32_t *)c->pool.get(S_BR_GRP, sizeof(int32_t) * (size_t)n_arc + 16);
	uint8_t *vwk = (uint8_t *)c->pool.get(S_VWK, (size_t)n_vtx + 16);
	const size_t need = sizeof(int32_t) * (size_t)n_vtx + 64;
	if (c->h_ndl_cap < need) {
		if (c->h_ndl) HIPCHK(hipStreamSynchronize(c->st));
		c->h_ndl = (int32_t *)c->pin.get(need + need / 2);
		if (!c->h_ndl) return PGA_ERR_NOMEM;
		c->h_ndl_cap = need + need / 2;
	}
	int32_t *ndl_dev = nullptr;
	HIPCHK(hipHostGetDevicePointer((void **)&ndl_dev, c->h_ndl, 0));
	int32_t *ndl_out = ndl_dev;
	if (rf) {
		ndl_out = (int32_t *)c->pool.get(S_BR_NDL, sizeof(int32_t) * (size_t)n_vtx + 16);
		if (!ndl_out) return PGA_ERR_NOMEM;
	}
	if (!grp || !vwk) return PGA_ERR_NOMEM;
	for (int attempt = 0;; ++attempt) {
		int32_t *cnt = (int32_t *)c->pool.get(S_NLCNT, 0);
		if (n_flt1 || n_flt2) HIPCHK(hipMemsetAsync(c->dcnt, 0, 2 * sizeof(int64_t), c->st));
		hipLaunchKernelGGL((k_br_wave<2>), dim3(nblk(n_vtx, BLOCK / WAVE)), dim3(BLOCK), 0, c->st, n_vtx, vs, ve, s1, agid, branch_diff, poff, (int32_t *)nullptr, (int64_t)c->br_cap, (const int32_t *)nullptr, cnt,
		                   branch_diff_dist, branch_diff_cut, aw, grp, ndl_out, (n_flt1 || n_flt2) ? c->dcnt : (int64_t *)nullptr, vwk, c->br_np < 0 ? c->dcnt + 15 : (const int64_t *)nullptr);
		if (rf && rf->on)
			hipLaunchKernelGGL(k_round_filter, dim3(nblk(S)), dim3(BLOCK), 0, c->st, S, (const int32_t *)c->pool.get(S_SEGCNT, 0), (const int32_t *)c->pool.get(S_DEG, 0), (const int32_t *)ndl_out,
			                   rf->max_tot_cnt, rf->max_degree, rf->max_dist_loci, (uint8_t *)ndl_dev);
		if (arc_weak && !c->table_sparse) HIPCHK(hipMemcpyAsync(arc_weak, aw, (size_t)n_arc, hipMemcpyDeviceToHost, c->st));
		if (n_flt1 || n_flt2) hipLaunchKernelGGL(k_mail_flush, dim3(1), dim3(64), 0, c->st, c->dcnt, c->h_box);
		TRY(sync_st(c));
		if (c->br_np >= 0 || c->h_cnt[15] <= c->br_cap || attempt) { if (c->br_np < 0) c->br_np = c->h_cnt[15]; c->br_np_seen = c->br_np; break; }
		c->br_cap = c->h_cnt[15] + c->h_cnt[15] / 2;
		HIPCHK(hipMemsetAsync(aw, 0, (size_t)n_arc, c->st)); HIPCHK(hipMemsetAsync(vwk, 0, (size_t)n_vtx, c->st));
		int32_t *dummy;
		TRY(branch_enumerate(c, &dummy));
	}
	if (n_dist_loci && !rf) memcpy(n_dist_loci, c->h_ndl, sizeof(int32_t) * (size_t)n_vtx);
	if (rf && rf->on) memcpy(rf->del_host, c->h_ndl, (size_t)S);
	if (n_flt1) *n_flt1 = c->h_cnt[0];
	if (n_flt2) *n_flt2 = c->h_cnt[1];
	return 0;
}

extern "C" int pga_branch_decide(pga_ctx_t *c, double branch_diff, double branch_diff_dist, double branch_diff_cut, uint8_t *arc_weak,
                                 int32_t *n_dist_loci, int64_t *n_flt1, int64_t *n_flt2)
{
	if (n_dist_loci == nullptr) return PGA_ERR_ARG;
	return decide_impl(c, branch_diff, branch_diff_dist, branch_diff_cut, arc_weak, n_dist_loci, n_flt1, n_flt2, nullptr);
}

extern "C" int pga_branch_decide_filter(pga_ctx_t *c, double branch_diff, double branch_diff_dist, double branch_diff_cut, int32_t do_filter,
                                        int32_t max_tot_cnt, int32_t max_degree, int32_t max_dist_loci, uint8_t *del)
{
	if (!(c->arc_deferred && !c->arc_done && c->table_sparse) || c->br_S != c->n_seg || (do_filter && del == nullptr)) return 2;
	RoundFilter rf = { do_filter, max_tot_cnt, max_degree, max_dist_loci, del };
	return decide_impl(c, branch_diff, branch_diff_dist, branch_diff_cut, nullptr, nullptr, nullptr, nullptr, &rf);
}

static int64_t x_arc_cap(const pga_ctx *c, const pga_loop_xchg_t *x)
{
	const int64_t m = std::max<int64_t>(c->x_arcs_seen, x->arc_cap_hint);
	return std::max<int64_t>(c->x_arc_floor, c->x_arcs_seen > 0 ? m + m / 8 + 1024 : 5 * m + 4096);
}

struct LoopX { const pga_loop_xchg_t *x; int64_t arc_cap, pair_cap, ecap; int32_t *gbuf; int64_t slot_words; pga_arc_part_t *merged; int64_t *xstat, *d_off; };

static int loop_exchange_table(pga_ctx *c, const LoopX &L, Gate local_gate = Gate{nullptr, 0}, int32_t *stamp = nullptr, int round = 0)
{
	const int S = c->n_seg, n_vtx = 2 * S, W = L.x->world;
	const int64_t mcap = (int64_t)W * L.arc_cap;
	pga_arc_part_t *stage = (pga_arc_part_t *)c->pool.get(S_ARC_STAGE, 0);
	int4 *gmeta = (int4 *)c->pool.get(S_GMETA, 0);
	int32_t *goff = (int32_t *)c->pool.get(S_GOFF, sizeof(int32_t) * (size_t)S);
	int32_t *seg_cnt = (int32_t *)c->pool.get(S_SEGCNT, sizeof(int32_t) * 2 * (size_t)std::max(1, S) * SEGCNT_COPIES);
	I32 *tile = (I32 *)c->pool.get(S_TILE, tile_buf_bytes(std::max<int64_t>(std::max<int64_t>(S, mcap), 2 * (int64_t)c->N + 2)));
	uint64_t *key = (uint64_t *)c->pool.get(S_MG_KEY, sizeof(uint64_t) * (size_t)mcap + 64);
	uint32_t *val = (uint32_t *)c->pool.get(S_MG_VAL, sizeof(uint32_t) * (size_t)mcap + 64);
	int32_t *slot = (int32_t *)c->pool.get(S_MG_SLOT, sizeof(int32_t) * (size_t)mcap + 64);
	if (!goff || !tile || !key || !val || !slot || (c->N && (!stage || !gmeta || !seg_cnt))) return PGA_ERR_NOMEM;
	if (c->N) {
		device_scan<I32>(InGmeta{gmeta}, OutExclI32{goff}, S, tile, OpSum{}, I32{0}, c->st, local_gate);
		hipLaunchKernelGGL(k_xs_compact, dim3(nblk(S, BLOCK / WAVE)), dim3(BLOCK), 0, c->st, gmeta, goff, S, stage, seg_cnt, L.gbuf, L.arc_cap, (const int64_t *)c->dcnt, local_gate, (const int32_t *)stamp, round);
	}
	else HIPCHK(hipMemsetAsync(L.gbuf, 0, sizeof(int32_t) * (size_t)(XS_HDR + xs_seg_words(S)), c->st));
	{ const int rc = L.x->allgather(L.x->user, L.gbuf, L.gbuf + L.slot_words, L.slot_words * (int64_t)sizeof(int32_t)); if (rc) return rc; }
	XSlots X = { L.gbuf + L.slot_words, L.slot_words, L.arc_cap, W, S };
	hipLaunchKernelGGL(k_xs_sum_rank, dim3(nblk(std::max<int64_t>(mcap, n_vtx))), dim3(BLOCK), 0, c->st, X, seg_cnt, L.d_off, c->dcnt, L.xstat, key, val, stamp, round);
	device_scan<I32>(InMgHeadN{key, L.d_off + W}, OutExclI32{slot}, mcap, tile, OpSum{}, I32{0}, c->st);
	hipLaunchKernelGGL(k_mgx_heads_sum, dim3(nblk(mcap)), dim3(BLOCK), 0, c->st, X, (const uint64_t *)key, (const uint32_t *)val, (const int32_t *)slot, (const int64_t *)(L.d_off + W), L.merged, c->dcnt + 10);
	CurTable t;
	TRY(cur_table(c, L.ecap, S, &t));
	hipLaunchKernelGGL(k_curx_table, dim3(nblk(mcap + n_vtx)), dim3(BLOCK), 0, c->st, (const pga_arc_part_t *)L.merged, (const int64_t *)(c->dcnt + 10), mcap, (const int32_t *)t.sg, n_vtx, t.ax, t.s1, t.agid, t.aw, t.vs, t.ve, t.dg, t.vwk);
	c->table_sparse = false, c->cur_tab = L.merged, c->cur_tab_n = 0;
	return 0;
}

extern "C" int pga_arc_round_x(pga_ctx_t *c, int32_t use_ori, int32_t n_seg, const pga_loop_xchg_t *x, int32_t *seg_cnt_host, int32_t *deg_host, int64_t *n_arc)
{
	const int S = n_seg, n_vtx = 2 * S, N = c->N;
	if (x == nullptr || x->world < 1 || x->allgather == nullptr || S != c->n_seg || S == 0 || arc_sort_path_forced()) return 2;
	if (c->x_arcs_seen <= 0 && x->arc_cap_hint <= 0) return 2;
	LoopX L = { x, 0, 0, 0, nullptr, 0, nullptr, nullptr, nullptr };
	L.arc_cap = x_arc_cap(c, x);
	{ const long long ea = xloop_cap(1); if (ea && c->x_arcs_seen == 0) L.arc_cap = std::max<int64_t>(ea, 1); }
	if ((int64_t)x->world * L.arc_cap >= ((int64_t)1 << 31)) return 2;
	L.ecap = std::max<int64_t>(2 * (int64_t)N + 2, (int64_t)x->world * L.arc_cap);
	L.slot_words = xs_slot_words(S, L.arc_cap);
	L.gbuf = (int32_t *)c->pool.get(S_XG_BUF, sizeof(int32_t) * (size_t)L.slot_words * ((size_t)x->world + 1) + 64);
	L.merged = (pga_arc_part_t *)c->pool.get(S_XG_OUT, sizeof(pga_arc_part_t) * (size_t)x->world * (size_t)L.arc_cap + 64);
	L.xstat = (int64_t *)c->pool.get(S_XSTAT, sizeof(int64_t) * 8);
	L.d_off = (int64_t *)c->pool.get(S_MG_SRC, sizeof(int64_t) * ((size_t)x->world + 2));
	if (!L.gbuf || !L.merged || !L.xstat || !L.d_off) return PGA_ERR_NOMEM;
	const size_t need = sizeof(int32_t) * (2 * (size_t)n_vtx) + 8 * sizeof(int64_t) + 64;
	if (c->h_round_cap < need) {
		if (c->h_round) HIPCHK(hipStreamSynchronize(c->st));
		c->h_round = (int32_t *)c->pin.get(need + need / 2);
		if (!c->h_round) return PGA_ERR_NOMEM;
		c->h_round_cap = need + need / 2;
	}
	c->arc_deferred = false, c->arc_done = false;
	HIPCHK(hipMemsetAsync(L.xstat, 0, sizeof(int64_t) * 8, c->st));
	HIPCHK(hipMemsetAsync(c->dcnt + 9, 0, sizeof(int64_t), c->st));
	HIPCHK(hipMemsetAsync(c->dcnt + 11, 0, sizeof(int64_t), c->st));
	CurTable t;
	TRY(cur_table(c, L.ecap, S, &t));
	if (N) { int32_t *seg_cnt, *deg; TRY(arc_round_genes(c, use_ori, &seg_cnt, &deg, nullptr, false)); }
	hipLaunchKernelGGL(k_seg_gid, dim3(nblk(c->Q)), dim3(BLOCK), 0, c->st, c->g2s, c->Q, S, t.sg);
	TRY(loop_exchange_table(c, L));
	int32_t *seg_cnt = (int32_t *)c->pool.get(S_SEGCNT, 0);
	int64_t *tail = (int64_t *)(c->h_round + 2 * (size_t)n_vtx + ((2 * (size_t)n_vtx) & 1));
	HIPCHK(hipMemcpyAsync(c->h_round, seg_cnt, sizeof(int32_t) * (size_t)n_vtx, hipMemcpyDeviceToHost, c->st));
	HIPCHK(hipMemcpyAsync(c->h_round + n_vtx, t.dg, sizeof(int32_t) * (size_t)n_vtx, hipMemcpyDeviceToHost, c->st));
	HIPCHK(hipMemcpyAsync(tail, L.xstat, 8 * sizeof(int64_t), hipMemcpyDeviceToHost, c->st));
	hipLaunchKernelGGL(k_mail_flush, dim3(1), dim3(64), 0, c->st, c->dcnt, c->h_box);
	TRY(sync_st(c));
	c->br_n = L.ecap, c->br_S = S, c->br_np = 0;
	if (tail[4] || c->h_cnt[3]) return PGA_ERR_INVARIANT;
	c->x_arcs_run = std::max<int64_t>(c->x_arcs_run, tail[1]);
	if (tail[2]) c->x_arcs_seen = std::max<int64_t>(c->x_arcs_seen, tail[1]), c->x_arc_floor = std::max<int64_t>(c->x_arc_floor, tail[1] + tail[1] / 4 + 1024);
	if (tail[2] || tail[3]) { c->x_redo = true; return 1; }
	memcpy(seg_cnt_host, c->h_round, sizeof(int32_t) * (size_t)n_vtx), memcpy(deg_host, c->h_round + n_vtx, sizeof(int32_t) * (size_t)n_vtx);
	c->cur_tab = L.merged, c->cur_tab_n = c->h_cnt[10], c->table_sparse = false;
	*n_arc = c->h_cnt[10];
	return 0;
}

extern "C" int pga_branch_loop(pga_ctx_t *c, int32_t n_round, const pga_branch_par_t *par, const int32_t *max_tot_cnt, const int32_t *max_degree,
                               const int32_t *max_dist_loci, uint8_t *seg_alive, const pga_loop_xchg_t *x, int32_t *seg_cnt_host, int32_t *ndl_host)
{
	static const bool off = getenv("PANGENE_BRANCH_LOOP_HOST") != nullptr;
	const int S = c->n_seg, n_vtx = 2 * S, N = c->N;
	if (off || n_round <= 0 || par == nullptr || seg_alive == nullptr || N == 0 || S == 0 || c->br_S != S || n_vtx > PO_THREADS * PO_MAX_ITEMS) return 2;
	if (par->final_on && (seg_cnt_host == nullptr || ndl_host == nullptr)) return 2;
	if (x == nullptr ? !(c->arc_deferred && !c->arc_done && c->table_sparse) : (c->table_sparse || c->arc_deferred || x->world < 1 || x->allgather == nullptr || x->allreduce_i32_sum == nullptr)) return 2;
	uint8_t *alive = (uint8_t *)c->pool.get(S_MISC, (size_t)S + 64);
	int32_t *ndl = (int32_t *)c->pool.get(S_BR_NDL, sizeof(int32_t) * (size_t)n_vtx + 16);
	if (!alive || !ndl) return PGA_ERR_NOMEM;
	HIPCHK(hipMemsetAsync(alive, 1, (size_t)S, c->st));
	const int64_t br_cap_before = c->br_cap;
	LoopX L = { x, 0, 0, 0, nullptr, 0, nullptr, nullptr, nullptr };
	if (x == nullptr) {
		int64_t dmax = 8;
		for (int r = 1; r < n_round; ++r) dmax = std::max<int64_t>(dmax, max_degree[r]);
		c->br_cap = std::max<int64_t>(c->br_cap, std::min<int64_t>((int64_t)n_vtx * dmax * dmax, (int64_t)1 << 26));
		static const long long cap_env = [] { const char *e = getenv("PANGENE_LOOP_PAIR_CAP"); return e ? atoll(e) : 0ll; }();
		if (cap_env > 0 && !c->loop_room_given) c->br_cap = cap_env;
	} else {
		int64_t dmax = 8;
		for (int r = 1; r < n_round; ++r) dmax = std::max<int64_t>(dmax, max_degree[r]);
		const int64_t worst = std::min<int64_t>((int64_t)n_vtx * dmax * dmax, (int64_t)1 << 26);
		L.pair_cap = std::min<int64_t>(worst, c->x_pairs_seen > 0 ? c->x_pairs_seen + c->x_pairs_seen / 8 + 4096 : std::max<int64_t>((int64_t)1 << 20, 4 * (int64_t)n_vtx));
		L.pair_cap = std::max<int64_t>(std::max<int64_t>(L.pair_cap, std::min<int64_t>(worst, c->x_pair_floor)), 4 * (int64_t)n_vtx);
		L.arc_cap = x_arc_cap(c, x);
		if (c->x_pairs_seen == 0) {
			const long long ep = xloop_cap(0), ea = xloop_cap(1);
			if (ep) L.pair_cap = std::max<int64_t>(ep, 4 * (int64_t)n_vtx);
			if (ea && c->x_arcs_seen == 0) L.arc_cap = std::max<int64_t>(ea, 1);
		}
		c->br_cap = L.pair_cap;
		if ((int64_t)x->world * L.arc_cap >= ((int64_t)1 << 31)) return 2;
		L.ecap = std::max<int64_t>(2 * (int64_t)N + 2, (int64_t)x->world * L.arc_cap);
		L.slot_words = xs_slot_words(S, L.arc_cap);
		L.gbuf = (int32_t *)c->pool.get(S_XG_BUF, sizeof(int32_t) * (size_t)L.slot_words * ((size_t)x->world + 1) + 64);
		L.merged = (pga_arc_part_t *)c->pool.get(S_XG_OUT2, sizeof(pga_arc_part_t) * (size_t)x->world * (size_t)L.arc_cap + 64);
		L.xstat = (int64_t *)c->pool.get(S_XSTAT, sizeof(int64_t) * 8);
		L.d_off = (int64_t *)c->pool.get(S_MG_SRC, sizeof(int64_t) * ((size_t)x->world + 2));
		if (!L.gbuf || !L.merged || !L.xstat || !L.d_off) return PGA_ERR_NOMEM;
		HIPCHK(hipMemsetAsync(L.xstat, 0, sizeof(int64_t) * 8, c->st));
		HIPCHK(hipMemsetAsync(c->dcnt + 11, 0, sizeof(int64_t), c->st));
		HIPCHK(hipMemsetAsync(c->dcnt + 9, 0, sizeof(int64_t), c->st));
		CurTable t;
		const pga_arc_part_t *tab = c->cur_tab; const int64_t n0 = c->cur_tab_n;
		if (n0 > L.ecap) return 2;
		TRY(cur_table(c, L.ecap, S, &t));
		if (!c->pool.get(S_BR_GRP, sizeof(int32_t) * (size_t)L.ecap + 16)) return PGA_ERR_NOMEM;
		zero_multi(c, t.vs, sizeof(int32_t) * (size_t)n_vtx, t.ve, sizeof(int32_t) * (size_t)n_vtx, t.aw, (size_t)L.ecap, t.vwk, (size_t)n_vtx);
		if (n0) {
			hipLaunchKernelGGL(k_seg_gid, dim3(nblk(c->Q)), dim3(BLOCK), 0, c->st, c->g2s, c->Q, S, t.sg);
			hipLaunchKernelGGL(k_cur_prep, dim3(nblk(n0)), dim3(BLOCK), 0, c->st, tab, n0, t.sg, t.ax, t.s1, t.agid, t.vs, t.ve);
		}
		hipLaunchKernelGGL(k_deg, dim3(nblk(n_vtx)), dim3(BLOCK), 0, c->st, t.vs, t.ve, n_vtx, t.dg);
		c->br_n = L.ecap;
	}
	bool first_x = true;
	if (par->pre_on) {
		HIPCHK(hipMemsetAsync(ndl, 0, sizeof(int32_t) * (size_t)n_vtx, c->st));
		int32_t *vs = (int32_t *)c->pool.get(S_BR_VS, 0), *ve = (int32_t *)c->pool.get(S_BR_VE, 0), *sg = (int32_t *)c->pool.get(S_BR_SEGGID, 0), *dg = (int32_t *)c->pool.get(S_DEG, 0), *seg_cnt = (int32_t *)c->pool.get(S_SEGCNT, 0);
		uint8_t *vwk = (uint8_t *)c->pool.get(S_VWK, (size_t)n_vtx + 16);
		if (!vs || !ve || !sg || !dg || !seg_cnt || !vwk) return PGA_ERR_NOMEM;
		hipLaunchKernelGGL(k_round_del, dim3(nblk(S)), dim3(BLOCK), 0, c->st, S, (const int32_t *)ndl, par->pre_max_tot_cnt, par->pre_max_degree, par->pre_max_dist_loci, (const int32_t *)sg, c->g2s, vs, ve, dg, seg_cnt, vwk, alive,
		                   (x || par->final_on) ? (int4 *)c->pool.get(S_GMETA, 0) : (int4 *)nullptr);
		hipLaunchKernelGGL(k_flag_vtx, dim3(nblk(N)), dim3(BLOCK), 0, c->st, c->flags, c->gid, N, c->g2s, 1);
		c->walk_valid = false, c->ha_valid = false;
		int32_t *sc2, *deg2;
		TRY(arc_round_genes(c, par->use_ori, &sc2, &deg2, nullptr, false));
		c->br_n = 2 * (int64_t)N + 2, c->br_S = S, c->br_np = 0;
		if (x) { TRY(loop_exchange_table(c, L)); c->br_n = L.ecap; first_x = false; }
	}
	static const bool no_skip = env_has("PANGENE_LOOP", "noskip");
	const bool gated = !no_skip && (int64_t)c->round_tag + n_round + 4 < (int64_t)HA_TAG_MAX;
	struct GateScope { pga_ctx *c; ~GateScope() { c->gate = Gate{nullptr, 0}, c->loop_gated = false, c->in_loop = false, c->ride_want = 0, c->ride_done = 0; } } gate_scope{c};
	c->loop_gated = gated, c->in_loop = true;
	static const int ride_env = [] { const char *e = getenv("PANGENE_LOOP_RIDE"); const int v = e ? atoi(e) : 2; return v < 0 ? 0 : v > 2 ? 2 : v; }();
	int ride = 0;
	c->ride_want = 0, c->ride_done = 0;
	if (ride_env && x == nullptr && !c->timing_rounds && !env_has("PANGENE_LOOP_FUSE", "0") && !env_has("PANGENE_RANK", "scan") && c->gs_np <= (1 << 15)) {
		int64_t maxg = 0;
		for (size_t g = 0; g + 1 < c->h_goff.size(); ++g) maxg = std::max<int64_t>(maxg, (int64_t)c->h_goff[g + 1] - c->h_goff[g]);
		if (maxg <= (1 << 15)) ride = ride_env, c->ride_cpg = (int)std::max<int64_t>(1, (maxg + RK_CHUNK - 1) / RK_CHUNK);
	}
	const uint32_t tag_before = c->round_tag;
	HIPCHK(hipMemsetAsync(c->dcnt + 16, 0, sizeof(int64_t), c->st));
	if (gated) HIPCHK(hipMemsetAsync(c->loopctl, 0xff, 4 * sizeof(int32_t), c->st));
	static const int live_env = [] { const char *e = getenv("PANGENE_LIVE_LISTS"); return e ? atoi(e) : -1; }();
	const bool live_ask = live_env != 0 && (live_env == 2 || N >= (1 << 21));
	for (int r = 0; r < n_round; ++r) {
		c->loop_round = r;
		bool rebuilt = false;
		c->gate = gated ? Gate{c->loopctl, r - 1} : Gate{nullptr, 0};
		static const bool fuse = !env_has("PANGENE_LOOP_FUSE", "0");
		RepDefer df;
		TRY(rep_pos_impl(c, fuse ? &df : nullptr));
		int32_t *cnt;
		TRY(branch_pairs_impl(c, nullptr, nullptr, 0, nullptr, S, par->branch_diff, par->local_dist, par->local_count, par->frag_mode, &cnt, nullptr, fuse ? &df : nullptr));
		if (x) { const int rc = x->allreduce_i32_sum(x->user, cnt, L.pair_cap); if (rc) return rc; }
		{
			const int64_t n_arc = c->br_n;
			uint8_t *aw = (uint8_t *)c->pool.get(S_ARCW, 0), *vwk = (uint8_t *)c->pool.get(S_VWK, (size_t)n_vtx + 16);
			int32_t *s1 = (int32_t *)c->pool.get(S_BR_S1, 0), *agid = (int32_t *)c->pool.get(S_BR_GID, 0), *vs = (int32_t *)c->pool.get(S_BR_VS, 0), *ve = (int32_t *)c->pool.get(S_BR_VE, 0);
			int32_t *poff = (int32_t *)c->pool.get(S_BR_POFF, 0), *grp = (int32_t *)c->pool.get(S_BR_GRP, sizeof(int32_t) * (size_t)n_arc + 16);
			int32_t *sg = (int32_t *)c->pool.get(S_BR_SEGGID, 0), *dg = (int32_t *)c->pool.get(S_DEG, 0), *seg_cnt = (int32_t *)c->pool.get(S_SEGCNT, 0);
			if (!aw || !vwk || !s1 || !agid || !vs || !ve || !poff || !grp || !sg || !dg || !seg_cnt) return PGA_ERR_NOMEM;
			hipLaunchKernelGGL((k_br_wave<2>), dim3(nblk(n_vtx, BLOCK / WAVE)), dim3(BLOCK), 0, c->st, n_vtx, vs, ve, s1, agid, par->branch_diff, poff, (int32_t *)nullptr, (int64_t)c->br_cap, (const int32_t *)nullptr, (const int32_t *)c->pool.get(S_NLCNT, 0),
			                   par->branch_diff_dist, par->branch_diff_cut, aw, grp, ndl, (int64_t *)nullptr, vwk, c->dcnt + 15, c->gate);
			TRY(pga_mark_hits(c, nullptr, nullptr, 0, nullptr, 1));
			c->gate = gated ? Gate{c->loopctl, r} : Gate{nullptr, 0};
			if (r > 0) {
				hipLaunchKernelGGL(k_round_del, dim3(nblk(S)), dim3(BLOCK), 0, c->st, S, (const int32_t *)ndl, max_tot_cnt[r], max_degree[r], max_dist_loci[r], (const int32_t *)sg, c->g2s, vs, ve, dg, seg_cnt, vwk, alive,
				                   (x || par->final_on) ? (int4 *)c->pool.get(S_GMETA, 0) : (int4 *)nullptr,
				                   gated ? c->loopctl : (int32_t *)nullptr, r);
				const bool ask = live_ask && (live_env == 2 || r == 1 || r == 2 || r == 4 || r == 8) && (r + 1 < n_round || par->final_on);
				if (ask) HIPCHK(hipMemsetAsync(c->live_cnt, 0, sizeof(int64_t) * LIVE_CNT_N, c->st));
				static const bool fv_x = env_has("PANGENE_FLAG_VTX", "x");
				if (c->live_on && c->z_valid && !fv_x && (int64_t)c->NL * 5 < (int64_t)N)
					hipLaunchKernelGGL(k_flag_vtx_z, dim3(nblk(std::max(c->NL, 1))), dim3(BLOCK), 0, c->st, c->flags, (const int32_t *)c->zx, (const int32_t *)c->zg, c->NL, (const int32_t *)c->g2s, c->gate, ask ? c->live_cnt : (int64_t *)nullptr);
				else
				hipLaunchKernelGGL(k_flag_vtx, dim3(nblk(N)), dim3(BLOCK), 0, c->st, c->flags, c->gid, N, c->g2s, 1, c->gate, ask ? c->live_cnt : (int64_t *)nullptr);
				c->walk_valid = false, c->ha_valid = false;
				if (ask) {
					hipLaunchKernelGGL(k_live_sum, dim3(1), dim3(BLOCK), 0, c->st, (const int64_t *)c->live_cnt, c->dcnt);
					hipLaunchKernelGGL(k_mail_flush, dim3(1), dim3(64), 0, c->st, c->dcnt, c->h_box);
					TRY(sync_st(c));
					const int64_t left = c->h_cnt[8];
					if (left > 0 && left * 4 <= (int64_t)c->NL * 3) {
						if (getenv("PANGENE_TIMING")) fprintf(stderr, "[pga_branch_loop] round %d: %lld of %d hits are without flt, the lists hold %d: built again\n", r, (long long)left, N, c->NL);
						TRY(build_z(c, left));
						rebuilt = true;
					}
				}
			}
		}
		if (r + 1 < n_round || par->final_on) {
			int32_t *seg_cnt, *deg;
			if (rebuilt || (x && first_x)) c->gate = Gate{nullptr, 0};
			c->ride_want = r + 1 < n_round ? ride : 0;
			const int rc_arc = arc_round_genes(c, par->use_ori, &seg_cnt, &deg, nullptr, false);
			c->ride_want = 0;
			if (rc_arc) return rc_arc;
			c->br_n = 2 * (int64_t)N + 2, c->br_S = S, c->br_np = 0;
			if (x) { TRY(loop_exchange_table(c, L, first_x ? Gate{nullptr, 0} : c->gate, gated ? c->loopctl : (int32_t *)nullptr, r)); c->br_n = L.ecap; first_x = false; }
		}
	}
	c->gate = Gate{nullptr, 0};
	c->arc_deferred = false, c->arc_done = false;
	static const bool no_tail = env_has("PANGENE_LOOP", "notail");
	const bool tail_on = par->final_on && x == nullptr && !no_tail;
	c->shadow_queued = false, c->fin_on = false;
	bool fin_queued = false;
	if (tail_on) {
		TRY(pga_set_filter(c, PGA_FLT_SHADOW));
		TRY(arc_table_final_queue(c, alive, &fin_queued));
	}
	int32_t *h_ctl = nullptr;
	if (gated) {
		if (!c->h_loopctl) c->h_loopctl = (int32_t *)c->pin.get(64);
		h_ctl = c->h_loopctl;
		if (!h_ctl) return PGA_ERR_NOMEM;
		HIPCHK(hipMemcpyAsync(h_ctl, c->loopctl, 4 * sizeof(int32_t), hipMemcpyDeviceToHost, c->st));
	}
	const size_t fetch_need = (((size_t)S + 128 + (par->final_on ? 4 * sizeof(int32_t) * (size_t)S + 64 : 0) + 15) & ~(size_t)15) + 64 + 16;
	if (c->h_fetch_cap < fetch_need) {
		c->h_fetch = c->pin.get(fetch_need + fetch_need / 2 + 512);
		if (!c->h_fetch) return PGA_ERR_NOMEM;
		c->h_fetch_cap = fetch_need + fetch_need / 2 + 512;
	}
	HIPCHK(hipMemcpyAsync(c->h_fetch, alive, (size_t)S, hipMemcpyDeviceToHost, c->st));
	int64_t *h_need = (int64_t *)((char *)c->h_fetch + fetch_need - 16);
	HIPCHK(hipMemcpyAsync(h_need, c->dcnt + 16, sizeof(int64_t), hipMemcpyDeviceToHost, c->st));
	int32_t *h_fin = (int32_t *)((char *)c->h_fetch + (((size_t)S + 127) & ~(size_t)63));
	if (par->final_on) {
		HIPCHK(hipMemcpyAsync(h_fin, (const int32_t *)c->pool.get(S_SEGCNT, 0), sizeof(int32_t) * (size_t)n_vtx, hipMemcpyDeviceToHost, c->st));
		HIPCHK(hipMemcpyAsync(h_fin + n_vtx, ndl, sizeof(int32_t) * (size_t)n_vtx, hipMemcpyDeviceToHost, c->st));
	}
	int64_t *h_x = nullptr;
	if (x) {
		int32_t *flags4 = L.gbuf;
		hipLaunchKernelGGL(k_xs_flags, dim3(1), dim3(64), 0, c->st, c->dcnt, L.xstat, (long long)L.pair_cap, flags4);
		{ const int rc = x->allreduce_i32_sum(x->user, flags4, 4); if (rc) return rc; }
		h_x = (int64_t *)((char *)c->h_fetch + (((size_t)S + 7) & ~(size_t)7));
		HIPCHK(hipMemcpyAsync(h_x, flags4, 16, hipMemcpyDeviceToHost, c->st));
		HIPCHK(hipMemcpyAsync(h_x + 2, L.xstat, 4 * sizeof(int64_t), hipMemcpyDeviceToHost, c->st));
	}
	hipLaunchKernelGGL(k_mail_flush, dim3(1), dim3(64), 0, c->st, c->dcnt, c->h_box);
	TRY(sync_st(c));
	if (gated) {
		c->round_tag = h_ctl[2] >= 0 ? (uint32_t)h_ctl[2] : tag_before;
		if (getenv("PANGENE_TIMING")) fprintf(stderr, "[pga_branch_loop] %d rounds queued; the last round that deleted a segment: %d, that marked a hit: %d (-1: none) -- the rounds after both found their kernels closed\n", n_round, h_ctl[0], h_ctl[1]);
	}
	c->br_np_seen = std::max<int64_t>(c->br_np_seen, c->h_cnt[15]);
	if (getenv("PANGENE_TIMING")) fprintf(stderr, "[pga_branch_loop] counters after %d rounds: invariant %lld, table overflows (last round) %lld, sticky %lld, pairs (last round) %lld of capacity %lld\n", n_round, (long long)c->h_cnt[3], (long long)c->h_cnt[9], (long long)c->h_cnt[11], (long long)c->h_cnt[15], (long long)c->br_cap);
	if (x && par->final_on) c->cur_tab = L.merged, c->cur_tab_n = c->h_cnt[10], c->table_sparse = false;
	if (x) {
		const int32_t *f = (const int32_t *)h_x;
		c->x_pairs_run = std::max<int64_t>(c->x_pairs_run, h_x[2]), c->x_arcs_run = std::max<int64_t>(c->x_arcs_run, h_x[3]);
		if (f[0] && f[2]) {
			c->x_pairs_seen = std::max<int64_t>(c->x_pairs_seen, c->x_pairs_run), c->x_arcs_seen = std::max<int64_t>(c->x_arcs_seen, c->x_arcs_run);
			c->x_pair_floor = std::max<int64_t>(c->x_pair_floor, h_x[2] > L.pair_cap ? std::max<int64_t>(2 * L.pair_cap, h_x[2] + h_x[2] / 4) : L.pair_cap);
			c->x_arc_floor = std::max<int64_t>(c->x_arc_floor, h_x[3] > L.arc_cap ? std::max<int64_t>(2 * L.arc_cap, h_x[3] + h_x[3] / 4) : L.arc_cap);
		}
		else if (!f[0]) c->x_pair_floor = 0, c->x_arc_floor = 0;
		c->br_np_seen = std::max<int64_t>(c->br_np_seen, h_x[2]);
		c->br_cap = std::max<int64_t>(br_cap_before, c->br_cap);
		if (getenv("PANGENE_TIMING")) fprintf(stderr, "[pga_branch_loop] sharded over %d ranks: flags (summed) void %d invariant %d capacity %d hub %d; longest pair list %lld of %lld, largest local table %lld of %lld\n", x->world, f[0], f[1], f[2], f[3],
		                                          (long long)h_x[2], (long long)L.pair_cap, (long long)h_x[3], (long long)L.arc_cap);
		if (f[1]) return PGA_ERR_INVARIANT;
		if (f[0]) return (f[2] && !f[3]) ? 3 : 1;
	}
	else if (c->h_cnt[11]) {
		if (c->h_cnt[3]) return PGA_ERR_INVARIANT;
		const int64_t need = *h_need;
		if (getenv("PANGENE_TIMING")) fprintf(stderr, "[pga_branch_loop] the longest pair list that did not fit: %lld (capacity %lld)\n", (long long)need, (long long)c->br_cap);
		if (need > c->br_cap && c->h_cnt[9] == 0 && need + need / 4 <= ((int64_t)1 << 27)) { c->br_cap = need + need / 4, c->loop_room_given = true; return 4; }
		return 1;
	}
	memcpy(seg_alive, c->h_fetch, (size_t)S);
	c->shadow_queued = tail_on;
	if (fin_queued) c->fin_n = c->h_cnt[10], c->fin_on = c->fin_n >= 0 && c->fin_n <= c->fin_cap;
	if (par->final_on) memcpy(seg_cnt_host, h_fin, sizeof(int32_t) * (size_t)n_vtx), memcpy(ndl_host, h_fin + n_vtx, sizeof(int32_t) * (size_t)n_vtx);
	return 0;
}

extern "C" int pga_mark_hits(pga_ctx_t *c, const uint64_t *arc_x, const uint8_t *arc_weak, int64_t n_arc, int64_t *n_marked, int32_t then_filter)
{
	const int N = c->N;
	if (n_marked) *n_marked = 0;
	if (N == 0) return 0;
	if (arc_x == nullptr) {
		TRY(ensure_half_arcs(c, c->ha_ori < 0 ? 0 : c->ha_ori));
		const uint64_t *ax = (const uint64_t *)c->pool.get(S_ARCX, 0); const uint8_t *aw = (const uint8_t *)c->pool.get(S_ARCW, 0);
		const int32_t *vs = (const int32_t *)c->pool.get(S_BR_VS, 0), *ve = (const int32_t *)c->pool.get(S_BR_VE, 0);
		const uint8_t *vwk = (const uint8_t *)c->pool.get(S_VWK, 0);
		if (!ax || !aw || !vs || !ve || !vwk) return PGA_ERR_NOMEM;
		if (n_marked) HIPCHK(hipMemsetAsync(c->dcnt + 2, 0, sizeof(int64_t), c->st));
		if (c->NL) hipLaunchKernelGGL(k_mark_hits_z, dim3(nblk(c->NL)), dim3(BLOCK), 0, c->st, c->zx, c->zy, c->zg, c->hfk, c->hbk, c->round_tag, c->NL, c->g2s, ax, aw, vs, ve, vwk, c->flags,
		                   n_marked ? c->dcnt + 2 : (int64_t *)nullptr, then_filter, n_marked ? Gate{nullptr, 0} : c->gate, c->gate.w ? c->loopctl : (int32_t *)nullptr, c->loop_round);
		if (then_filter) c->walk_valid = false, c->ha_valid = false;
	} else {
		uint64_t *ax = (uint64_t *)c->pool.get(S_ARCX, sizeof(uint64_t) * (size_t)n_arc + 16);
		uint8_t *aw = (uint8_t *)c->pool.get(S_ARCW, (size_t)n_arc + 16);
		int32_t *wn = (int32_t *)c->pool.get(S_WEAKNEW, sizeof(int32_t) * (size_t)N);
		if (!ax || !aw || !wn) return PGA_ERR_NOMEM;
		TRY(upload(c, ax, arc_x, (size_t)n_arc)); TRY(upload(c, aw, arc_weak, (size_t)n_arc));
		zero_multi(c, wn, sizeof(int32_t) * (size_t)N, c->dcnt + 2, sizeof(int64_t));
		int32_t *val, *prev;
		TRY(walk_prev(c, &val, &prev));
		ensure_yrec(c);
		hipLaunchKernelGGL(k_mark_hits, dim3(nblk(N)), dim3(BLOCK), 0, c->st, val, prev, c->yrecA, c->yrecB, c->g2s, N, ax, aw, n_arc, (const int32_t *)nullptr, (const int32_t *)nullptr, (const uint8_t *)nullptr, wn);
		hipLaunchKernelGGL(k_weak_merge, dim3(nblk(N)), dim3(BLOCK), 0, c->st, c->flags, wn, N, n_marked ? c->dcnt + 2 : (int64_t *)nullptr);
		if (then_filter) TRY(pga_set_filter(c, PGA_FLT_WEAK2));
	}
	if (n_marked) {
		HIPCHK(hipMemcpyAsync(c->h_cnt, c->dcnt, 16 * sizeof(int64_t), hipMemcpyDeviceToHost, c->st));
		TRY(sync_st(c));
		*n_marked = c->h_cnt[2];
	}
	return 0;
}
```

### pangene_amd/csrc/hip/pga_host_context.hpp

```cpp
#pragma once


static inline size_t tile_buf_bytes(int64_t n) { return std::max<size_t>(sizeof(int64_t) * (size_t)(scan_tiles(std::max<int64_t>(rs_table_len(n), n)) + 8), 256 * sizeof(uint32_t) + 64); }

static inline unsigned nblk(int64_t n, int per = BLOCK) { return (unsigned)((n + per - 1) / per); }

struct DevBlock { void *p; size_t cap; int dev; };
static std::atomic<int> g_last_dev{-1};
static int cur_dev() { int d = 0; return hipGetDevice(&d) == hipSuccess ? d : 0; }
static std::mutex g_dev_mu;
static std::vector<DevBlock> g_dev_cache;
static std::condition_variable g_dev_cv; static int g_dev_reserving = 0;
static bool dev_cache_on() { static const bool on = [] { const char *e = getenv("PANGENE_DEV_CACHE"); return !(e && *e == '0'); }(); return on; }

static void *dev_big_alloc(size_t want, size_t *got)
{
	{
		std::unique_lock<std::mutex> lk(g_dev_mu);
		g_dev_cv.wait(lk, [] { return g_dev_reserving == 0; });
		size_t best = (size_t)-1;
		const int dev = cur_dev();
		for (size_t i = 0; i < g_dev_cache.size(); ++i)
			if (g_dev_cache[i].dev == dev && g_dev_cache[i].cap >= want && g_dev_cache[i].cap <= 2 * want + ((size_t)64 << 20) && (best == (size_t)-1 || g_dev_cache[i].cap < g_dev_cache[best].cap)) best = i;
		if (best != (size_t)-1) {
			DevBlock b = g_dev_cache[best];
			g_dev_cache.erase(g_dev_cache.begin() + (long)best);
			*got = b.cap;
			return b.p;
		}
	}
	void *q = nullptr;
	if (dev_cache_on() && want >= ((size_t)1 << 20)) {
		const size_t padded = (want + want / 8 + ((size_t)64 << 20) - 1) & ~(((size_t)64 << 20) - 1);
		if (hipMalloc(&q, padded) == hipSuccess) { *got = padded; return q; }
		(void)hipGetLastError(), q = nullptr;
	}
	if (hipMalloc(&q, want) != hipSuccess) {
		(void)hipGetLastError();
		{
			std::lock_guard<std::mutex> lk(g_dev_mu);
			for (DevBlock &b : g_dev_cache) (void)hipFree(b.p);
			g_dev_cache.clear();
		}
		if (hipMalloc(&q, want) != hipSuccess) { (void)hipGetLastError(); return nullptr; }
	}
	*got = want;
	return q;
}

static void dev_big_free(void *p, size_t cap)
{
	if (p == nullptr) return;
	if (dev_cache_on() && cap >= ((size_t)1 << 20)) {
		std::lock_guard<std::mutex> lk(g_dev_mu);
		if (g_dev_cache.size() >= 2) {
			size_t small = 0;
			for (size_t i = 1; i < g_dev_cache.size(); ++i) if (g_dev_cache[i].cap < g_dev_cache[small].cap) small = i;
			if (g_dev_cache[small].cap >= cap) { (void)hipFree(p); return; }
			(void)hipFree(g_dev_cache[small].p);
			g_dev_cache.erase(g_dev_cache.begin() + (long)small);
		}
		g_dev_cache.push_back(DevBlock{p, cap, cur_dev()});
		return;
	}
	(void)hipFree(p);
}

struct DevPool {
	std::vector<void *> p; std::vector<size_t> cap; std::vector<char> own;
	char *arena = nullptr; size_t arena_cap = 0, arena_off = 0;
	void *get(int slot, size_t bytes)
	{
		if ((int)p.size() <= slot) p.resize(slot + 1, nullptr), cap.resize(slot + 1, 0), own.resize(slot + 1, 0);
		if (bytes == 0) bytes = 16;
		if (cap[slot] < bytes) {
			if (p[slot] && own[slot]) (void)hipFree(p[slot]);
			size_t want = (bytes + bytes / 4 + 256 + 255) & ~(size_t)255;
			if (arena && arena_off + want <= arena_cap) { p[slot] = arena + arena_off, arena_off += want, own[slot] = 0; }
			else if (hipMalloc(&p[slot], want) == hipSuccess) { own[slot] = 1; if (poison_on()) (void)hipMemset(p[slot], 0x5a, want); }
			else { p[slot] = nullptr; cap[slot] = 0; own[slot] = 0; return nullptr; }
			cap[slot] = want;
		}
		return p[slot];
	}
	void release()
	{
		for (size_t i = 0; i < p.size(); ++i) if (p[i] && own[i]) (void)hipFree(p[i]);
		dev_big_free(arena, arena_cap);
		p.clear(); cap.clear(); own.clear(); arena = nullptr; arena_cap = arena_off = 0;
	}
};

struct PinBlock { char *p; size_t cap; };
static std::mutex g_pin_mu;
static std::vector<PinBlock> g_pin_cache;
struct PinArena {
	std::vector<PinBlock> blocks; size_t off = 0;
	void *get(size_t bytes)
	{
		bytes = (bytes + 255) & ~(size_t)255;
		if (blocks.empty() || off + bytes > blocks.back().cap) {
			PinBlock b = { nullptr, 0 };
			{
				std::lock_guard<std::mutex> lk(g_pin_mu);
				for (size_t i = 0; i < g_pin_cache.size(); ++i)
					if (g_pin_cache[i].cap >= bytes) { b = g_pin_cache[i]; g_pin_cache.erase(g_pin_cache.begin() + (long)i); break; }
			}
			if (b.p == nullptr) {
				b.cap = std::max<size_t>(bytes, (size_t)8 << 20);
				if (hipHostMalloc((void **)&b.p, b.cap, hipHostMallocDefault) != hipSuccess) return nullptr;
			}
			blocks.push_back(b), off = 0;
		}
		void *r = blocks.back().p + off;
		off += bytes;
		if (poison_on()) memset(r, 0x5a, bytes);
		return r;
	}
	void release()
	{
		std::lock_guard<std::mutex> lk(g_pin_mu);
		for (PinBlock &b : blocks) { if (g_pin_cache.size() < 16) g_pin_cache.push_back(b); else (void)hipHostFree(b.p); }
		blocks.clear(), off = 0;
	}
};

enum {
	S_KEY_A, S_KEY_B, S_VAL_A, S_VAL_B, S_TABLE, S_TILE, S_I32_A, S_I32_B, S_I32_C, S_TAB_A, S_TAB_B, S_TAB_C, S_TAB_D,
	S_TDIST, S_TS1, S_TS2, S_TGEN, S_SDIST, S_SS1, S_SS2, S_SGEN, S_HEAD, S_SLOT, S_ARCS, S_SEGCNT, S_BITS, S_TRIPLES,
	S_WALK_VAL, S_WALK_PREV, S_PERM, S_OVPOS, S_OVFILE, S_RUNSTART, S_CDN, S_MG_KEY, S_MG_VAL, S_MG_SRC, S_MG_OUT, S_MG_HEAD, S_MG_SLOT, S_MG_RUN, S_BR_S1, S_BR_GID, S_BR_VS, S_BR_VE, S_BR_PC, S_BR_POFF, S_BR_GRP, S_BR_NDL, S_BR_SEGGID, S_PAIRS, S_NLCNT, S_ARCX, S_ARCW, S_WEAKNEW, S_RP_SEG, S_RP_R, S_RP_CM, S_RP_POS, S_RP_IV, S_DL, S_SCRATCH, S_UPLOAD, S_RAW, S_ARC_STAGE, S_GMETA, S_GOFF, S_DEG, S_BIGLIST, S_STAGE_SID, S_STATS, S_G2S, S_MISC, S_SLOW, S_HZLIST, S_VWK, S_XG_BUF, S_XG_OUT, S_XG_OUT2, S_XSTAT, S_GSLIST, S_UPLOAD2, S_BINS, S_FIN_ID, S_FRONT,
	S_COUNT
};

constexpr int LIVE_CNT_N = 1024;
struct TimedLaunch { hipEvent_t a, b; int which; int64_t units; };

struct pga_ctx {
	hipStream_t st = nullptr; bool own_stream = false;
	int32_t n_genome = 0, n_genome_global = 0, P = 0, Q = 0, n_seg_ctg = 0;
	int32_t N = 0, E = 0;
	int n_cu = 256;
	uint32_t sweep_seq = 0;
	pga_params_t par;
	std::vector<int32_t> h_goff, h_ggl;
	int32_t *fidx = 0, *gnm = 0, *seg = 0, *pid = 0, *gid = 0, *cs = 0, *ce = 0, *cm = 0, *cds = 0, *nex = 0, *offx = 0, *sori = 0, *sadj = 0, *pm = 0;
	int32_t *rk = 0;
	int sc_bits = 64;
	int rk_shift = -1;
	int32_t *hrank = 0;
	bool any_multi = true;
	bool exon_regular = true;
	double list_density = 0; int64_t density_tiles = 0;
	bool lists_in_lds = true, density_known = false;
	int rp_form = 0;
	int32_t *vfirst = 0; int64_t *vbase = 0;
	int4 *recA = 0, *recB = 0, *recC = 0;
	int32_t *rank = 0, *sdom = 0, *pdom = 0, *pdom0 = 0; uint32_t *flags = 0;
	int32_t *yperm = 0, *goff = 0, *ggl = 0, *ctg_base = 0, *inv = 0, *headpos = 0, *eoff = 0; int64_t *woff = 0;
	int cs_bits = 1, cm_bits = 1, seg_bits = 1, ctg_bits = 1;
	bool inv_valid = false;
	bool sweep_init = false;
	bool bin_on = false; int32_t *up_grouped = nullptr; int4 *bins = nullptr; int bin_n_small = 0, bin_n_big = 0, bin_np_small = 64, bin_np_big = 64, bin_ctg_bits = 1;
	bool gs_ok = false; int gs_np = 64; int32_t *gs_list = nullptr; int gs_n[3] = { 0, 0, 0 }, gs_np_of[3] = { 64, 64, 64 };
	int2 *exon = 0; int32_t *prot_gid = 0; uint8_t *gene_pref = 0;
	int32_t *max_ori = 0; int64_t *sums = 0; int32_t *vtx_cnt = 0; int32_t *g2s = 0; int32_t n_seg = 0;
	uint64_t sync_epoch_reset = 0;
	bool gf_ok = false;
	bool gf_k32 = false; int gf_pos_bits = 0;
	bool x_redo = false;
	int64_t x_pairs_seen = 0, x_arcs_seen = 0;
	int64_t x_pairs_run = 0, x_arcs_run = 0;
	int64_t x_pair_floor = 0, x_arc_floor = 0;
	int64_t *dcnt = 0;
	int64_t *h_cnt = 0;
	int64_t *h_box = 0;
	void *h_stage = nullptr; size_t h_stage_cap = 0;
	void *h_fetch = nullptr; size_t h_fetch_cap = 0;
	int32_t *h_front = nullptr; size_t h_front_cap = 0;
	bool front_keys_on = true, front_keys_done = false;
	bool front_live = false; unsigned long long front_epoch = 0;
	size_t lds_post_set = 0, lds_vtx_set = 0;
	int32_t *h_g2s = nullptr; size_t h_g2s_cap = 0; hipEvent_t g2s_done = nullptr;
	DevPool pool; PinArena pin;
	bool walk_valid = false;
	int32_t *zx = 0, *zy = 0, *zg = 0; int2 *zst = 0; int32_t *zpos = 0, *zoff = 0;
	bool live_on = false;
	int32_t NL = 0;
	int32_t *lx = 0;
	int32_t *ylist_buf = 0;
	const int32_t *ylist = 0;
	bool z_early = false; hipEvent_t z_ev = nullptr;
	int32_t *ga_ctl = 0;
	int4 *cA = 0, *cB = 0, *cC = 0; int32_t *cx = 0;
	int2 *tg = 0; bool tg_valid = false;
	int64_t *live_cnt = 0;
	int64_t live_hint = -1;
	int4 *wrec = 0; bool wrec_valid = false;
	uint32_t *hfk = 0, *hbk = 0; int4 *hfp = 0, *hbp = 0;
	bool z_valid = false, ha_valid = false; uint32_t round_tag = 0; int ha_ori = -1;
	Gate gate = Gate{nullptr, 0};
	int32_t *loopctl = nullptr;
	int loop_round = 0;
	bool in_loop = false;
	bool loop_room_given = false;
	bool loop_gated = false;
	int32_t *h_loopctl = nullptr;
	int32_t *h_ov = nullptr; size_t h_ov_cap = 0;
	hipEvent_t ov_ev[2] = { nullptr, nullptr }; bool ov_ev_used[2] = { false, false }; unsigned ov_seq = 0;
	bool zposy_stale = false;
	const pga_arc_part_t *cur_tab = nullptr; int64_t cur_tab_n = 0;
	bool table_sparse = false;
	int32_t *h_round = nullptr; size_t h_round_cap = 0;
	void *h_fin = nullptr; int64_t h_fin_cap = 0, fin_cap = 0, fin_n = 0; bool fin_on = false;
	int ride_want = 0, ride_cpg = 1, ride_done = 0; uint32_t ride_tag = 0;
	bool shadow_queued = false;
	unsigned long long sync_epoch = 0, arc_epoch = 0; bool arc_deferred = false, arc_done = false, force_sort_once = false, sweep_done = false; std::vector<int32_t> def_host;
	int4 *yrecA = 0, *yrecB = 0; bool yrec_valid = false;
	int64_t br_np_seen = 0;
	int64_t br_n = 0, br_np = 0, br_cap = 0; int32_t br_S = 0;
	struct { double diff; int32_t local_dist, local_count, frag_mode; } br_par = { 0, 0, 0, 0 };
	int32_t *h_ndl = nullptr; size_t h_ndl_cap = 0;
	std::vector<TimedLaunch> timed; bool timing_on = false;
	bool timing_rounds = false;
	hipEvent_t span_a = nullptr;
	std::vector<void *> owned; void *arena = nullptr; size_t arena_cap = 0;
	std::vector<std::pair<void **, size_t>> plan;
};

template <class T> static int dalloc(pga_ctx *c, T **p, size_t n)
{
	c->plan.emplace_back((void **)p, (((n ? n : 1) * sizeof(T)) + 255) & ~(size_t)255);
	return 0;
}

static int dalloc_commit(pga_ctx *c)
{
	size_t tot = 0;
	if (getenv("PANGENE_NO_ARENA")) {
		for (auto &e : c->plan) { void *q = nullptr; if (hipMalloc(&q, e.second) != hipSuccess) return PGA_ERR_NOMEM; *e.first = q; c->owned.push_back(q); if (poison_on()) (void)hipMemset(q, 0x5a, e.second); }
		c->plan.clear();
		return 0;
	}
	for (auto &e : c->plan) tot += e.second;
	size_t got = 0;
	void *base = dev_big_alloc(tot ? tot : 256, &got);
	if (base == nullptr) return PGA_ERR_NOMEM;
	c->arena = base, c->arena_cap = got;
	if (poison_on()) (void)hipMemset(base, 0x5a, tot ? tot : 256);
	size_t off = 0;
	for (auto &e : c->plan) *e.first = (char *)base + off, off += e.second;
	c->plan.clear();
	return 0;
}
```

### pangene_amd/csrc/hip/pga_host_selftest.hpp

```cpp
#pragma once


extern "C" int pga_selftest_sort(uint64_t *keys, uint32_t *vals, int64_t n, int32_t n_bits)
{
	int ndev = 0;
	if (hipGetDeviceCount(&ndev) != hipSuccess || ndev <= 0) return PGA_ERR_NO_DEVICE;
	uint64_t *ka, *kb; uint32_t *va, *vb, *table; int32_t *tile;
	HIPCHK(hipMalloc((void **)&ka, sizeof(uint64_t) * (size_t)(n + 1))); HIPCHK(hipMalloc((void **)&kb, sizeof(uint64_t) * (size_t)(n + 1)));
	HIPCHK(hipMalloc((void **)&va, sizeof(uint32_t) * (size_t)(n + 1))); HIPCHK(hipMalloc((void **)&vb, sizeof(uint32_t) * (size_t)(n + 1)));
	HIPCHK(hipMalloc((void **)&table, sizeof(uint32_t) * (size_t)(rs_table_len(n) + 1)));
	HIPCHK(hipMalloc((void **)&tile, tile_buf_bytes(n)));
	HIPCHK(hipMemcpy(ka, keys, sizeof(uint64_t) * (size_t)n, hipMemcpyHostToDevice));
	HIPCHK(hipMemcpy(va, vals, sizeof(uint32_t) * (size_t)n, hipMemcpyHostToDevice));
	RadixBufs b = { kb, vb, table, tile };
	uint64_t *kr; uint32_t *vr;
	device_radix_sort(ka, va, n, n_bits, b, &kr, &vr, 0);
	HIPCHK(hipDeviceSynchronize());
	HIPCHK(hipMemcpy(keys, kr, sizeof(uint64_t) * (size_t)n, hipMemcpyDeviceToHost));
	HIPCHK(hipMemcpy(vals, vr, sizeof(uint32_t) * (size_t)n, hipMemcpyDeviceToHost));
	(void)hipFree(ka); (void)hipFree(kb); (void)hipFree(va); (void)hipFree(vb); (void)hipFree(table); (void)hipFree(tile);
	return 0;
}

extern "C" int pga_selftest_merge(const pga_arc_part_t *gathered, const int64_t *count, int32_t W, int64_t slot_sz, pga_arc_part_t *out, int64_t *n_out)
{
	int ndev = 0;
	if (hipGetDeviceCount(&ndev) != hipSuccess || ndev <= 0) return PGA_ERR_NO_DEVICE;
	pga_ctx c;
	HIPCHK(hipStreamCreateWithFlags(&c.st, hipStreamNonBlocking));
	TRY(dalloc(&c, &c.dcnt, 16)); TRY(dalloc_commit(&c));
	HIPCHK(hipHostMalloc((void **)&c.h_cnt, 16 * sizeof(int64_t), hipHostMallocDefault));
	pga_arc_part_t *dg = nullptr, *res = nullptr;
	HIPCHK(hipMalloc((void **)&dg, sizeof(pga_arc_part_t) * (size_t)(W * slot_sz + 1)));
	HIPCHK(hipMemcpy(dg, gathered, sizeof(pga_arc_part_t) * (size_t)(W * slot_sz), hipMemcpyHostToDevice));
	int rc = pga_arc_merge(&c, dg, count, W, slot_sz, &res, n_out);
	if (rc == 0 && *n_out) rc = hipMemcpyAsync(out, res, sizeof(pga_arc_part_t) * (size_t)*n_out, hipMemcpyDeviceToHost, c.st) == hipSuccess ? 0 : PGA_ERR_NO_DEVICE;
	(void)hipStreamSynchronize(c.st);
	(void)hipFree(dg); (void)hipFree(c.dcnt); (void)hipHostFree(c.h_cnt);
	c.pool.release();
	(void)hipStreamDestroy(c.st);
	return rc;
}

__device__ __forceinline__ int64_t cal_perm(int64_t i, int64_t n, int64_t window)
{
	const int64_t base = i & ~(window - 1), span = base + window <= n ? window : 0;
	return span ? base + (((i - base) * 40503 + 12345) & (window - 1)) : i;
}
__global__ __launch_bounds__(BLOCK) void k_cal_read16(const int4 *__restrict__ src, int64_t n, int32_t *sink)
{
	int acc = 0;
	for (int64_t i = (int64_t)blockIdx.x * BLOCK + threadIdx.x; i < n; i += (int64_t)gridDim.x * BLOCK) { const int4 v = src[i]; acc ^= v.x ^ v.y ^ v.z ^ v.w; }
	if (acc == 0x7fffffff) sink[0] = acc;
}
__global__ __launch_bounds__(BLOCK) void k_cal_read4(const int32_t *__restrict__ src, int64_t n, int32_t *sink)
{
	int acc = 0;
	for (int64_t i = (int64_t)blockIdx.x * BLOCK + threadIdx.x; i < n; i += (int64_t)gridDim.x * BLOCK) acc ^= src[i];
	if (acc == 0x7fffffff) sink[0] = acc;
}
__global__ __launch_bounds__(BLOCK) void k_cal_gather4(const int32_t *__restrict__ src, int64_t n, int64_t window, int32_t *sink)
{
	int acc = 0;
	for (int64_t i = (int64_t)blockIdx.x * BLOCK + threadIdx.x; i < n; i += (int64_t)gridDim.x * BLOCK) acc ^= src[cal_perm(i, n, window)];
	if (acc == 0x7fffffff) sink[0] = acc;
}
__global__ __launch_bounds__(BLOCK) void k_cal_gather16(const int4 *__restrict__ src, int64_t n, int64_t window, int32_t *sink)
{
	int acc = 0;
	for (int64_t i = (int64_t)blockIdx.x * BLOCK + threadIdx.x; i < n; i += (int64_t)gridDim.x * BLOCK) { const int4 v = src[cal_perm(i, n, window)]; acc ^= v.x ^ v.w; }
	if (acc == 0x7fffffff) sink[0] = acc;
}
__global__ __launch_bounds__(BLOCK) void k_cal_write16(int4 *__restrict__ dst, int64_t n)
{
	for (int64_t i = (int64_t)blockIdx.x * BLOCK + threadIdx.x; i < n; i += (int64_t)gridDim.x * BLOCK) dst[i] = make_int4((int)i, 1, 2, 3);
}
__global__ __launch_bounds__(BLOCK) void k_cal_write4(int32_t *__restrict__ dst, int64_t n)
{
	for (int64_t i = (int64_t)blockIdx.x * BLOCK + threadIdx.x; i < n; i += (int64_t)gridDim.x * BLOCK) dst[i] = (int)i;
}
__global__ __launch_bounds__(BLOCK) void k_cal_scatter4(int32_t *__restrict__ dst, int64_t n, int64_t window)
{
	for (int64_t i = (int64_t)blockIdx.x * BLOCK + threadIdx.x; i < n; i += (int64_t)gridDim.x * BLOCK) dst[cal_perm(i, n, window)] = (int)i;
}
__global__ __launch_bounds__(BLOCK) void k_cal_scatter16(int4 *__restrict__ dst, int64_t n, int64_t window)
{
	for (int64_t i = (int64_t)blockIdx.x * BLOCK + threadIdx.x; i < n; i += (int64_t)gridDim.x * BLOCK) dst[cal_perm(i, n, window)] = make_int4((int)i, 1, 2, 3);
}

extern "C" int pga_selftest_traffic(int64_t n, int64_t window)
{
	int ndev = 0;
	if (hipGetDeviceCount(&ndev) != hipSuccess || ndev <= 0) return PGA_ERR_NO_DEVICE;
	if (n < 1024) return PGA_ERR_ARG;
	if (window <= 0) { window = 1; while (window * 2 <= n) window *= 2; }
	if (window & (window - 1)) return PGA_ERR_ARG;
	int4 *a = nullptr, *b = nullptr; int32_t *sink = nullptr;
	HIPCHK(hipMalloc((void **)&a, sizeof(int4) * (size_t)n)); HIPCHK(hipMalloc((void **)&b, sizeof(int4) * (size_t)n)); HIPCHK(hipMalloc((void **)&sink, 256));
	HIPCHK(hipMemset(a, 1, sizeof(int4) * (size_t)n)); HIPCHK(hipMemset(b, 2, sizeof(int4) * (size_t)n));
	HIPCHK(hipDeviceSynchronize());
	const unsigned grid = (unsigned)std::min<int64_t>((n + BLOCK - 1) / BLOCK, (int64_t)256 * 64);
	hipLaunchKernelGGL(k_cal_read16, dim3(grid), dim3(BLOCK), 0, 0, (const int4 *)a, n, sink);
	hipLaunchKernelGGL(k_cal_read4, dim3(grid), dim3(BLOCK), 0, 0, (const int32_t *)b, n, sink);
	hipLaunchKernelGGL(k_cal_gather4, dim3(grid), dim3(BLOCK), 0, 0, (const int32_t *)a, n, window, sink);
	hipLaunchKernelGGL(k_cal_gather16, dim3(grid), dim3(BLOCK), 0, 0, (const int4 *)b, n, window, sink);
	hipLaunchKernelGGL(k_cal_write16, dim3(grid), dim3(BLOCK), 0, 0, a, n);
	hipLaunchKernelGGL(k_cal_write4, dim3(grid), dim3(BLOCK), 0, 0, (int32_t *)b, n);
	hipLaunchKernelGGL(k_cal_scatter4, dim3(grid), dim3(BLOCK), 0, 0, (int32_t *)a, n, window);
	hipLaunchKernelGGL(k_cal_scatter16, dim3(grid), dim3(BLOCK), 0, 0, b, n, window);
	HIPCHK(hipDeviceSynchronize());
	(void)hipFree(a); (void)hipFree(b); (void)hipFree(sink);
	return 0;
}

extern "C" int pga_selftest_scan(const int32_t *in, const int32_t *seg, int32_t *out, int64_t n, int32_t mode)
{
	int ndev = 0;
	if (hipGetDeviceCount(&ndev) != hipSuccess || ndev <= 0) return PGA_ERR_NO_DEVICE;
	int32_t *di, *ds, *dout; int64_t *tile;
	HIPCHK(hipMalloc((void **)&di, sizeof(int32_t) * (size_t)(n + 1))); HIPCHK(hipMalloc((void **)&ds, sizeof(int32_t) * (size_t)(n + 1)));
	HIPCHK(hipMalloc((void **)&dout, sizeof(int32_t) * (size_t)(n + 1))); HIPCHK(hipMalloc((void **)&tile, sizeof(int64_t) * (size_t)(scan_tiles(n) + 8)));
	HIPCHK(hipMemcpy(di, in, sizeof(int32_t) * (size_t)n, hipMemcpyHostToDevice));
	if (seg) HIPCHK(hipMemcpy(ds, seg, sizeof(int32_t) * (size_t)n, hipMemcpyHostToDevice));
	if (mode == 0) device_scan<I32>(InI32{di}, OutExclI32{dout}, n, (I32 *)tile, OpSum{}, I32{0}, 0);
	else if (mode == 1) device_scan<I32>(InI32{di}, OutExclI32{dout}, n, (I32 *)tile, OpMax{}, I32{-1}, 0);
	else device_scan<SegMax>(InSegMax{ds, di}, OutSegMax{dout}, n, (SegMax *)tile, OpSegMax{}, SegMax{SEG_EMPTY, 0}, 0);
	HIPCHK(hipDeviceSynchronize());
	HIPCHK(hipMemcpy(out, dout, sizeof(int32_t) * (size_t)n, hipMemcpyDeviceToHost));
	(void)hipFree(di); (void)hipFree(ds); (void)hipFree(dout); (void)hipFree(tile);
	return 0;
}

typedef struct {
	int32_t *recA, *recB, *recC;
	uint32_t *flags;
	int32_t *fidx, *gnm, *yperm;
	int32_t *headpos;
	uint32_t f_head, f_multi, f_cstie;
	int32_t route;
	int32_t n_unit[3];
	int32_t n_cu;
} pga_selftest_stage_a_t;
extern "C" int pga_selftest_stage_a(pga_ctx_t *c, pga_selftest_stage_a_t *out)
{
	if (c == nullptr || out == nullptr) return PGA_ERR_ARG;
	TRY(sync_st(c));
	const size_t N = (size_t)c->N, GL = (size_t)c->n_genome;
	auto fetch = [&](void *dst, const void *src, size_t bytes) { return (dst == nullptr || bytes == 0 || hipMemcpy(dst, src, bytes, hipMemcpyDeviceToHost) == hipSuccess) ? 0 : PGA_ERR_NO_DEVICE; };
	TRY(fetch(out->recA, c->recA, sizeof(int4) * N)); TRY(fetch(out->recB, c->recB, sizeof(int4) * N)); TRY(fetch(out->recC, c->recC, sizeof(int4) * N));
	TRY(fetch(out->flags, c->flags, sizeof(uint32_t) * N));
	TRY(fetch(out->fidx, c->fidx, sizeof(int32_t) * N)); TRY(fetch(out->gnm, c->gnm, sizeof(int32_t) * N)); TRY(fetch(out->yperm, c->yperm, sizeof(int32_t) * N));
	if (N) TRY(fetch(out->headpos, c->headpos, sizeof(int32_t) * (GL + 1)));
	out->f_head = F_HEAD, out->f_multi = F_MULTI, out->f_cstie = F_CSTIE;
	out->route = c->bin_on ? 2 : c->gs_ok ? 1 : 0, out->n_cu = c->n_cu;
	for (int k = 0; k < 3; ++k) out->n_unit[k] = out->route == 1 ? c->gs_n[k] : 0;
	if (out->route == 2) out->n_unit[0] = c->bin_n_small, out->n_unit[1] = c->bin_n_big;
	return 0;
}

extern "C" int pga_selftest_arc_final(const pga_arc_part_t *in, int64_t n, int32_t *out)
{
	int ndev = 0;
	if (hipGetDeviceCount(&ndev) != hipSuccess || ndev <= 0) return PGA_ERR_NO_DEVICE;
	if (n <= 0 || in == nullptr || out == nullptr) return PGA_ERR_ARG;
	pga_arc_part_t *di; int4 *dout;
	HIPCHK(hipMalloc((void **)&di, sizeof(pga_arc_part_t) * (size_t)n)); HIPCHK(hipMalloc((void **)&dout, sizeof(int4) * (size_t)n));
	HIPCHK(hipMemcpy(di, in, sizeof(pga_arc_part_t) * (size_t)n, hipMemcpyHostToDevice));
	hipLaunchKernelGGL(k_arc_final_probe, dim3(nblk(n)), dim3(BLOCK), 0, 0, (const pga_arc_part_t *)di, n, dout);
	HIPCHK(hipDeviceSynchronize());
	HIPCHK(hipMemcpy(out, dout, sizeof(int4) * (size_t)n, hipMemcpyDeviceToHost));
	(void)hipFree(di); (void)hipFree(dout);
	return 0;
}

extern "C" int pga_selftest_post_rep(const int64_t *sums, const int32_t *max_ori, const int32_t *prot_gid, int32_t P, int32_t Q, double min_cnt, int32_t joint_pseudo, int32_t drop_sgl_exon,
                                     int32_t *words, uint8_t *rep, uint8_t *pj)
{
	int ndev = 0;
	if (hipGetDeviceCount(&ndev) != hipSuccess || ndev <= 0) return PGA_ERR_NO_DEVICE;
	if (P <= 0 || Q <= 0 || !sums || !max_ori || !prot_gid || !words || !rep || !pj) return PGA_ERR_ARG;
	const size_t nw = 16 + 3 * (size_t)P + (size_t)Q;
	unsigned long long *d_sums, *d_key; int32_t *d_mx, *d_gid, *d_rep1, *d_words; uint8_t *d_rep;
	HIPCHK(hipMalloc((void **)&d_sums, sizeof(int64_t) * 6 * (size_t)P)); HIPCHK(hipMalloc((void **)&d_key, sizeof(int64_t) * (size_t)Q));
	HIPCHK(hipMalloc((void **)&d_mx, sizeof(int32_t) * (size_t)P)); HIPCHK(hipMalloc((void **)&d_gid, sizeof(int32_t) * (size_t)P));
	HIPCHK(hipMalloc((void **)&d_rep1, sizeof(int32_t) * (size_t)Q));
	HIPCHK(hipMalloc((void **)&d_words, sizeof(int32_t) * nw)); HIPCHK(hipMalloc((void **)&d_rep, 2 * (size_t)P));
	HIPCHK(hipMemcpy(d_sums, sums, sizeof(int64_t) * 6 * (size_t)P, hipMemcpyHostToDevice));
	HIPCHK(hipMemcpy(d_mx, max_ori, sizeof(int32_t) * (size_t)P, hipMemcpyHostToDevice)); HIPCHK(hipMemcpy(d_gid, prot_gid, sizeof(int32_t) * (size_t)P, hipMemcpyHostToDevice));
	HIPCHK(hipMemset(d_key, 0, sizeof(int64_t) * (size_t)Q)); HIPCHK(hipMemset(d_rep1, 0, sizeof(int32_t) * (size_t)Q));
	HIPCHK(hipMemset(d_words, 0, sizeof(int32_t) * 16)); HIPCHK(hipMemset(d_words + 16, 0xff, sizeof(int32_t) * (nw - 16)));
	hipLaunchKernelGGL(k_post_count, dim3(nblk(P)), dim3(BLOCK), 0, 0, d_sums, P, (const int32_t *)d_gid, Q, d_key);
	PostFront a = { d_sums, d_mx, d_gid, P, Q, min_cnt, joint_pseudo ? 1 : 0, drop_sgl_exon ? 1 : 0, d_key, d_rep1, d_rep, d_rep + P, d_words };
	hipLaunchKernelGGL(k_post_rep, dim3(nblk(P)), dim3(BLOCK), 0, 0, a);
	HIPCHK(hipDeviceSynchronize());
	HIPCHK(hipMemcpy(words, d_words, sizeof(int32_t) * nw, hipMemcpyDeviceToHost));
	HIPCHK(hipMemcpy(rep, d_rep, (size_t)P, hipMemcpyDeviceToHost)); HIPCHK(hipMemcpy(pj, d_rep + P, (size_t)P, hipMemcpyDeviceToHost));
	(void)hipFree(d_sums); (void)hipFree(d_key); (void)hipFree(d_mx); (void)hipFree(d_gid); (void)hipFree(d_rep1); (void)hipFree(d_words); (void)hipFree(d_rep);
	return 0;
}
```

Before: 227.4.

## Enumerate branch pairs lazily against first arc, resolve residual pairs in segmented pass

For vertices with at most one wave of arcs, the branch enumeration now emits only the n-1 pairs against the first arc instead of all n(n-1)/2 pairs. Arcs that fail the local-count test get their remaining pairs written to 32 atomically-filled residual segments, which a segmented n_local pass and a new k_br_finish kernel then resolve to assign groups. The residual n_local launch can also ride along with the mark-hits kernel in one fused launch. This is meant to cut pair-enumeration and local-check work, at the cost of extra kernels, atomics, residual capacity limits with an overflow-and-retry path, and more complex control flow.

```diff
diff --git a/pangene_amd/csrc/hip/k_branch.hpp b/pangene_amd/csrc/hip/k_branch.hpp
--- a/pangene_amd/csrc/hip/k_branch.hpp
+++ b/pangene_amd/csrc/hip/k_branch.hpp
@@ -182,21 +182,30 @@
 
 constexpr int nl_lanes_for(int GL) { return GL <= 256 ? 16 : GL <= 640 ? 32 : 64; }
 
+constexpr int BR_RSEG = 32, BR_RSTRIDE = 512;
+struct NLocalArgs { const int32_t *pairs; int64_t n_cap; const int64_t *np_dev; int GL; const void *rp_in; int local_dist, local_count, frag_mode; int32_t *cnt; NLocalHz hz; int seg_shift; };
 template <int FORM, int NL_LANES>
-__global__ __launch_bounds__(BLOCK) void k_n_local(const int32_t *pairs, int64_t n_cap, const int64_t *np_dev, int GL, const void *rp_in,
-                                                     int local_dist, int local_count, int frag_mode, int32_t *cnt, NLocalHz hz, Gate gate)
+__device__ __forceinline__ void n_local_body(const NLocalArgs &a, const unsigned bid, const unsigned nb)
 {
 	constexpr int NL_PAIRS = WAVE / NL_LANES;
 	constexpr unsigned long long NL_MASK = NL_LANES == 64 ? ~0ull : ((1ull << (NL_LANES & 63)) - 1);
-	if (gate_closed(gate)) return;
+	const int32_t *pairs = a.pairs; const int GL = a.GL; const void *rp_in = a.rp_in; const int local_dist = a.local_dist, local_count = a.local_count, frag_mode = a.frag_mode;
+	int32_t *cnt = a.cnt; const NLocalHz hz = a.hz;
 	const int lane = threadIdx.x & 63, grp = lane / NL_LANES, sub = lane & (NL_LANES - 1);
-	int64_t n_pair = np_dev ? *np_dev : n_cap;
-	if (n_pair > n_cap) return;
-	const int64_t stride = (int64_t)gridDim.x * (BLOCK / WAVE) * NL_PAIRS;
-	for (int64_t k0 = ((int64_t)blockIdx.x * (BLOCK / WAVE) + (threadIdx.x >> 6)) * NL_PAIRS; k0 < n_pair; k0 += stride) {
-		const int64_t k = k0 + grp;
-		const bool have = k < n_pair;
-		const int64_t kk = have ? k : n_pair - 1;
+	int64_t wid = (int64_t)bid * (BLOCK / WAVE) + (threadIdx.x >> 6), nw = (int64_t)nb * (BLOCK / WAVE), base = 0;
+	int64_t n_pair = (a.np_dev && a.seg_shift < 0) ? *a.np_dev : a.n_cap;
+	if (a.seg_shift >= 0) {
+		const int s = (int)(wid % BR_RSEG);
+		n_pair = a.np_dev[s * BR_RSTRIDE], base = (int64_t)s << a.seg_shift;
+		if (n_pair > ((int64_t)1 << a.seg_shift)) return;
+		wid /= BR_RSEG, nw /= BR_RSEG;
+	}
+	else if (n_pair > a.n_cap) return;
+	const int64_t stride = nw * NL_PAIRS;
+	for (int64_t k0 = wid * NL_PAIRS; k0 < n_pair; k0 += stride) {
+		const bool have = k0 + grp < n_pair;
+		const int64_t k = base + k0 + grp;
+		const int64_t kk = have ? k : base + n_pair - 1;
 		const int64_t g1 = (int64_t)pairs[2 * kk] * GL, g2 = (int64_t)pairs[2 * kk + 1] * GL;
 		int c = 0;
 		bool open = have;
@@ -242,6 +251,13 @@
 		if (have && sub == 0) cnt[k] = c;
 	}
 }
+template <int FORM, int NL_LANES>
+__global__ __launch_bounds__(BLOCK) void k_n_local(const int32_t *pairs, int64_t n_cap, const int64_t *np_dev, int GL, const void *rp_in,
+                                                     int local_dist, int local_count, int frag_mode, int32_t *cnt, NLocalHz hz, Gate gate, int seg_shift = -1)
+{
+	if (gate_closed(gate)) return;
+	n_local_body<FORM, NL_LANES>(NLocalArgs{pairs, n_cap, np_dev, GL, rp_in, local_dist, local_count, frag_mode, cnt, hz, seg_shift}, blockIdx.x, gridDim.x);
+}
 
 __global__ __launch_bounds__(BLOCK) void k_br_prep(const uint64_t *ax, int64_t n_arc, const int32_t *seg_gid, int32_t *agid, int32_t *vs, int32_t *ve)
 {
@@ -304,7 +320,7 @@
 	if (v < n_vtx) deg[v] = ve[v] - vs[v];
 }
 
-__device__ __forceinline__ int br_count_one(const int v, const int32_t *vs, const int32_t *ve, const int32_t *s1, const double bd)
+__device__ __forceinline__ int br_count_one(const int v, const int32_t *vs, const int32_t *ve, const int32_t *s1, const double bd, const bool lazy = false)
 {
 	const int a0 = vs[v], n = ve[v] - a0;
 	if (n < 2) return 0;
@@ -314,13 +330,14 @@
 		n_max += s1[a0 + i] == max_s1;
 		n_weak += (1.0 - (double)s1[a0 + i] / max_s1) > bd;
 	}
-	return n_max * n_weak + n * (n - 1) / 2;
-}
-__global__ __launch_bounds__(BLOCK) void k_br_count(int n_vtx, const int32_t *vs, const int32_t *ve, const int32_t *s1, double bd, int32_t *pc, Gate gate)
+	return n_max * n_weak + (lazy && n <= WAVE ? n - 1 : n * (n - 1) / 2);
+}
+__global__ __launch_bounds__(BLOCK) void k_br_count(int n_vtx, const int32_t *vs, const int32_t *ve, const int32_t *s1, double bd, int32_t *pc, Gate gate, int64_t *res_len = nullptr )
 {
 	const int v = blockIdx.x * BLOCK + threadIdx.x;
 	if (v >= n_vtx || gate_closed(gate)) return;
-	pc[v] = br_count_one(v, vs, ve, s1, bd);
+	if (v == 0 && res_len) for (int k = 0; k < BR_RSEG; ++k) res_len[k * BR_RSTRIDE] = 0;
+	pc[v] = br_count_one(v, vs, ve, s1, bd, res_len != nullptr);
 }
 
 constexpr int PO_THREADS = 1024, PO_MAX_ITEMS = 64;
@@ -433,10 +450,17 @@
 	if (MODE == 2 && lane == 0) *ndl_out = n_group;
 }
 
+struct BrLazy {
+	int on;
+	int32_t *rpairs; int seg_shift;
+	int64_t *rlen;
+	int32_t *roff;
+	unsigned long long *rmask;
+};
 template <int MODE>
 __device__ __forceinline__ void br_wave_body(const int v, const int lane, uint16_t *s_grp , const int64_t k0 , const int32_t *vs, const int32_t *ve, const int32_t *s1g, const int32_t *agidg, double bd,
                                              int32_t *pairs, int64_t pair_cap, const int32_t *pcnt, const int32_t *cnt, double bdist, double bcut,
-                                             uint8_t *weak, int32_t *grpg, int32_t *ndl, int64_t *dcnt, uint8_t *vwk)
+                                             uint8_t *weak, int32_t *grpg, int32_t *ndl, int64_t *dcnt, uint8_t *vwk, const BrLazy lz = BrLazy{0, nullptr, 0, nullptr, nullptr, nullptr})
 {
 	const int a0 = vs[v], n = ve[v] - a0;
 	if (n < 2) { if (MODE == 2 && lane == 0) ndl[v] = 0; return; }
@@ -481,6 +505,42 @@
 		}
 	}
 	const int64_t k2 = k0 + (int64_t)n_max * __popcll(m_weak);
+	if (lz.on) {
+		const int64_t k = k2 + (lane - 1);
+		if (MODE == 1) {
+			const int gid_0 = __builtin_amdgcn_readlane(my_gid, 0);
+			if (lane > 0 && in) pairs[2 * k] = gid_0, pairs[2 * k + 1] = my_gid;
+			return;
+		}
+		const bool un = lane > 0 && in && !(cnt[k] > 0);
+		const unsigned long long m_un = __ballot(un);
+		int n_group = 1, off = -1;
+		if (m_un) {
+			const int mine = un ? lane - 1 : 0;
+			const int incl = wave_scan_incl(I32{mine}, OpSum{}, lane).v, tot = __builtin_amdgcn_readlane(incl, 63);
+			if (tot == 0) n_group = 2;
+			else {
+				const int seg = v & (BR_RSEG - 1);
+				long long base = 0;
+				if (lane == 0) base = (long long)atomicAdd((unsigned long long *)(lz.rlen + seg * BR_RSTRIDE), (unsigned long long)tot);
+				base = __shfl(base, 0, WAVE);
+				n_group = 0;
+				if (base + tot <= ((long long)1 << lz.seg_shift)) {
+					base += (long long)seg << lz.seg_shift;
+					off = (int)base;
+					const int my_off = incl - mine;
+					for (unsigned long long m = m_un; m; m &= m - 1) {
+						const int j = __ffsll((long long)m) - 1;
+						const int gid_j = __builtin_amdgcn_readlane(my_gid, j), off_j = __builtin_amdgcn_readlane(my_off, j);
+						const int64_t q = base + off_j + (lane - 1);
+						if (lane >= 1 && lane < j) lz.rpairs[2 * q] = my_gid, lz.rpairs[2 * q + 1] = gid_j;
+					}
+				}
+			}
+		}
+		if (lane == 0) ndl[v] = n_group, lz.roff[v] = off, lz.rmask[v] = m_un;
+		return;
+	}
 	int grp = 0, n_group = 0;
 	for (int i = 0; i < n; ++i) {
 		const int64_t k = k2 + (int64_t)i * n - (int64_t)i * (i + 1) / 2 + (lane - i - 1);
@@ -499,13 +559,42 @@
 __global__ __launch_bounds__(BLOCK) void k_br_wave(int n_vtx, const int32_t *vs, const int32_t *ve, const int32_t *s1g, const int32_t *agidg, double bd,
                                                      const int32_t *poff, int32_t *pairs, int64_t pair_cap , const int32_t *pcnt , const int32_t *cnt, double bdist, double bcut,
                                                      uint8_t *weak, int32_t *grpg, int32_t *ndl, int64_t *dcnt, uint8_t *vwk ,
-                                                     const int64_t *np_dev = nullptr , Gate gate = Gate{nullptr, 0})
+                                                     const int64_t *np_dev = nullptr , Gate gate = Gate{nullptr, 0},
+                                                     BrLazy lz = BrLazy{0, nullptr, 0, nullptr, nullptr, nullptr})
 {
 	__shared__ uint16_t s_grp[MODE == 2 ? (BLOCK / WAVE) * BR_WIDE_CAP : 1];
 	const int v = blockIdx.x * (BLOCK / WAVE) + (threadIdx.x >> 6), lane = threadIdx.x & 63;
 	if (v >= n_vtx || gate_closed(gate)) return;
 	if (MODE == 2 && np_dev && *np_dev > pair_cap) return;
-	br_wave_body<MODE>(v, lane, s_grp, poff[v], vs, ve, s1g, agidg, bd, pairs, pair_cap, pcnt, cnt, bdist, bcut, weak, grpg, ndl, dcnt, vwk);
+	br_wave_body<MODE>(v, lane, s_grp, poff[v], vs, ve, s1g, agidg, bd, pairs, pair_cap, pcnt, cnt, bdist, bcut, weak, grpg, ndl, dcnt, vwk, lz);
+}
+
+__global__ __launch_bounds__(BLOCK) void k_br_finish(int n_vtx, const int32_t *vs, const int32_t *ve, const int32_t *rcnt, BrLazy lz, int32_t *ndl, int64_t *dcnt, const int64_t *np_dev, int64_t pair_cap, Gate gate)
+{
+	const int v = blockIdx.x * (BLOCK / WAVE) + (threadIdx.x >> 6), lane = threadIdx.x & 63;
+	if (v >= n_vtx || gate_closed(gate)) return;
+	if (np_dev && *np_dev > pair_cap) return;
+	if (v == 0) {
+		const int64_t l64 = lane < BR_RSEG ? lz.rlen[lane * BR_RSTRIDE] : 0;
+		const int64_t len = wave_max((int)(l64 < 0x7fffffff ? l64 : 0x7fffffff));
+		if (lane == 0) { if (len > dcnt[18]) dcnt[18] = len; if (len > ((int64_t)1 << lz.seg_shift)) dcnt[11] = 1; }
+	}
+	const int n = ve[v] - vs[v];
+	if (n < 2 || n > WAVE) return;
+	const int off = lz.roff[v];
+	if (off < 0) return;
+	const unsigned long long m_un = lz.rmask[v];
+	const bool in = lane < n, un = (m_un >> lane) & 1;
+	const int mine = un ? lane - 1 : 0;
+	const int my_off = wave_scan_incl(I32{mine}, OpSum{}, lane).v - mine;
+	int grp = in && !un ? 1 : 0, n_group = 1;
+	for (int i = 1; i < n; ++i) {
+		if (__ballot(in && grp == 0) == 0) break;
+		int gi = __builtin_amdgcn_readlane(grp, i);
+		if (gi == 0) { gi = ++n_group; if (lane == i) grp = gi; }
+		if (lane > i && un && grp == 0 && rcnt[(int64_t)off + my_off + (i - 1)] > 0) grp = gi;
+	}
+	if (lane == 0) ndl[v] = n_group;
 }
 
 struct LoopFront {
@@ -513,6 +602,7 @@
 	const uint32_t *flags; const int32_t *goff; int32_t *rx;
 	void *rp_out; int64_t n_ent; int clear_bytes;
 	Gate gate;
+	int64_t *res_len;
 };
 __global__ __launch_bounds__(RK_T) void k_loop_front1(LoopFront a)
 {
@@ -521,7 +611,8 @@
 	const int b = blockIdx.x, tid = threadIdx.x;
 	if (b < a.nbc) {
 		const int v = b * RK_T + tid, lane = tid & 63, w = tid >> 6;
-		const int pc = v < a.n_vtx ? br_count_one(v, a.vs, a.ve, a.s1, a.bd) : 0;
+		if (v < BR_RSEG && a.res_len) a.res_len[v * BR_RSTRIDE] = 0;
+		const int pc = v < a.n_vtx ? br_count_one(v, a.vs, a.ve, a.s1, a.bd, a.res_len != nullptr) : 0;
 		const I32 incl = wave_scan_incl(I32{pc}, OpSum{}, lane);
 		if (lane == 63) wtot[0][w] = incl.v;
 		__syncthreads();
@@ -538,7 +629,7 @@
 	}
 }
 struct LoopFront2 {
-	int nb_rep, n_vtx, nbc; const int32_t *vs, *ve, *s1, *agid; double bd; int32_t *poff; const int32_t *btot, *pc; int32_t *pairs; int64_t pair_cap; int64_t *dcnt;
+	int nb_rep, n_vtx, nbc; const int32_t *vs, *ve, *s1, *agid; double bd; int32_t *poff; const int32_t *btot, *pc; int32_t *pairs; int64_t pair_cap; int64_t *dcnt; int lazy;
 };
 template <int FORM, bool CLEARED>
 __global__ __launch_bounds__(BLOCK) void k_loop_front2(RepFill rf, LoopFront2 a)
@@ -555,7 +646,7 @@
 		const int tot = wave_sum(part);
 		if (lane == 0) { a.dcnt[15] = tot; if (tot > a.pair_cap) { a.dcnt[11] = 1; if (tot > a.dcnt[16]) a.dcnt[16] = tot; } }
 	}
-	br_wave_body<1>(v, lane, nullptr, k0, a.vs, a.ve, a.s1, a.agid, a.bd, a.pairs, a.pair_cap, a.pc, nullptr, 0.0, 0.0, nullptr, nullptr, nullptr, a.dcnt, nullptr);
+	br_wave_body<1>(v, lane, nullptr, k0, a.vs, a.ve, a.s1, a.agid, a.bd, a.pairs, a.pair_cap, a.pc, nullptr, 0.0, 0.0, nullptr, nullptr, nullptr, a.dcnt, nullptr, BrLazy{a.lazy, nullptr, 0, nullptr, nullptr, nullptr});
 }
 
 __global__ __launch_bounds__(BLOCK) void k_round_filter(int S, const int32_t *seg_cnt, const int32_t *deg, const int32_t *ndl, int max_tot_cnt, int max_degree, int max_dist_loci, uint8_t *del)
diff --git a/pangene_amd/csrc/hip/k_genes.hpp b/pangene_amd/csrc/hip/k_genes.hpp
--- a/pangene_amd/csrc/hip/k_genes.hpp
+++ b/pangene_amd/csrc/hip/k_genes.hpp
@@ -503,13 +503,16 @@
 	}
 }
 
-__global__ __launch_bounds__(BLOCK) void k_mark_hits_z(const int32_t *zx, const int32_t *zy, const int32_t *zg, const uint32_t *hfk, const uint32_t *hbk, uint32_t tag, int n, const int32_t *g2s,
-                                                        const uint64_t *ax, const uint8_t *aw, const int32_t *vs, const int32_t *ve, const uint8_t *vwk,
-                                                        uint32_t *flags, int64_t *cnt, int then_filter, Gate gate, int32_t *stamp , int round)
-{
-	int z = blockIdx.x * BLOCK + threadIdx.x;
+struct MarkHitsZ {
+	const int32_t *zx, *zy, *zg; const uint32_t *hfk, *hbk; uint32_t tag; int n; const int32_t *g2s;
+	const uint64_t *ax; const uint8_t *aw; const int32_t *vs, *ve; const uint8_t *vwk;
+	uint32_t *flags; int64_t *cnt; int then_filter; Gate gate; int32_t *stamp ; int round;
+};
+__device__ __forceinline__ void mark_hits_z_body(const MarkHitsZ &a, const int z)
+{
+	const int32_t *zx = a.zx, *zy = a.zy, *zg = a.zg, *g2s = a.g2s, *vs = a.vs, *ve = a.ve; const uint32_t *hfk = a.hfk, *hbk = a.hbk; const uint32_t tag = a.tag; const int n = a.n;
+	const uint64_t *ax = a.ax; const uint8_t *aw = a.aw, *vwk = a.vwk; uint32_t *flags = a.flags; int64_t *cnt = a.cnt; const int then_filter = a.then_filter, round = a.round; int32_t *stamp = a.stamp;
 	bool marked = false;
-	if (gate_closed(gate)) return;
 	if (z < n) {
 		const uint32_t kb = hbk[z], kf = hfk[z];
 		const int y = zy[z], g = zg[z];
@@ -543,3 +546,15 @@
 		if (mk && (threadIdx.x & 63) == (unsigned)__ffsll((long long)mk) - 1) atomicAdd((unsigned long long *)cnt, (unsigned long long)__popcll(mk));
 	}
 }
+__global__ __launch_bounds__(BLOCK) void k_mark_hits_z(MarkHitsZ a)
+{
+	if (gate_closed(a.gate)) return;
+	mark_hits_z_body(a, blockIdx.x * BLOCK + threadIdx.x);
+}
+template <int FORM, int NL_LANES>
+__global__ __launch_bounds__(BLOCK) void k_mark_hits_nl(MarkHitsZ a, NLocalArgs nl, int nb_nl)
+{
+	if (gate_closed(a.gate)) return;
+	if ((int)blockIdx.x < nb_nl) { n_local_body<FORM, NL_LANES>(nl, blockIdx.x, (unsigned)nb_nl); return; }
+	mark_hits_z_body(a, (blockIdx.x - nb_nl) * BLOCK + threadIdx.x);
+}
diff --git a/pangene_amd/csrc/hip/pga_host_branch.hpp b/pangene_amd/csrc/hip/pga_host_branch.hpp
--- a/pangene_amd/csrc/hip/pga_host_branch.hpp
+++ b/pangene_amd/csrc/hip/pga_host_branch.hpp
@@ -51,19 +51,25 @@
 
 extern "C" int pga_rep_pos(pga_ctx_t *c) { return rep_pos_impl(c, nullptr); }
 
-static int n_local_dev(pga_ctx *c, const int32_t *d_pairs, int64_t n, const int64_t *np_dev, int32_t local_dist, int32_t local_count, int32_t frag_mode, int32_t **cnt)
-{
-	int32_t *d_cnt = (int32_t *)c->pool.get(S_NLCNT, sizeof(int32_t) * (size_t)n + 16);
+struct NLocalRide { NLocalArgs a; unsigned nb; int lanes; };
+static int mark_hits_resident(pga_ctx *c, int64_t *n_marked, int32_t then_filter, const NLocalRide *ride);
+static int n_local_dev(pga_ctx *c, const int32_t *d_pairs, int64_t n, const int64_t *np_dev, int32_t local_dist, int32_t local_count, int32_t frag_mode, int32_t **cnt, int cnt_slot = S_NLCNT, int64_t seen = -1, int seg_shift = -1,
+                       NLocalRide *ride = nullptr)
+{
+	int32_t *d_cnt = (int32_t *)c->pool.get(cnt_slot, sizeof(int32_t) * (size_t)n + 16);
 	int4 *rp = (int4 *)c->pool.get(S_RP_SEG, 0);
 	if (!d_cnt || !rp) return PGA_ERR_NOMEM;
 	*cnt = d_cnt;
 	NLocalHz hz = { (const int32_t *)c->pool.get(S_RP_IV, 0), c->ctg_base, c->dcnt, (int32_t *)c->pool.get(S_HZLIST, sizeof(int32_t) * PGA_HAZARD_CAP) };
 	if (!hz.iv || !hz.list) return PGA_ERR_NOMEM;
-	const int64_t est = np_dev ? (c->br_np_seen > 0 ? c->br_np_seen : std::min<int64_t>(n, 1 << 18)) : n;
+	if (seen < 0) seen = c->br_np_seen;
+	const int64_t est = np_dev ? (seen > 0 ? seen : std::min<int64_t>(n, 1 << 18)) : n;
 	static const int lanes_env = [] { const char *e = getenv("PANGENE_NL_LANES"); return e ? atoi(e) : 0; }();
 	const int lanes = (lanes_env == 16 || lanes_env == 32 || lanes_env == 64) ? lanes_env : nl_lanes_for(c->n_genome);
-	const unsigned grid = (unsigned)std::max<int64_t>(1, std::min<int64_t>(nblk(est, BLOCK / WAVE * (WAVE / lanes)), 1 << 20));
-#define NL_LAUNCH(FORM, LANES) hipLaunchKernelGGL((k_n_local<FORM, LANES>), dim3(grid), dim3(BLOCK), 0, c->st, d_pairs, n, np_dev, c->n_genome, (const void *)rp, local_dist, local_count, frag_mode, d_cnt, hz, c->gate)
+	unsigned grid = (unsigned)std::max<int64_t>(1, std::min<int64_t>(nblk(est, BLOCK / WAVE * (WAVE / lanes)), 1 << 20));
+	if (seg_shift >= 0) grid = (grid + 7u) & ~7u;
+	if (ride) { *ride = NLocalRide{ NLocalArgs{d_pairs, n, np_dev, c->n_genome, (const void *)rp, local_dist, local_count, frag_mode, d_cnt, hz, seg_shift}, n ? grid : 0u, lanes }; return 0; }
+#define NL_LAUNCH(FORM, LANES) hipLaunchKernelGGL((k_n_local<FORM, LANES>), dim3(grid), dim3(BLOCK), 0, c->st, d_pairs, n, np_dev, c->n_genome, (const void *)rp, local_dist, local_count, frag_mode, d_cnt, hz, c->gate, seg_shift)
 #define NL_FORM(FORM) do { if (lanes == 16) NL_LAUNCH(FORM, 16); else if (lanes == 32) NL_LAUNCH(FORM, 32); else NL_LAUNCH(FORM, 64); } while (0)
 	if (n && c->rp_form == RP_COMPACT) NL_FORM(RP_COMPACT);
 	else if (n && c->rp_form == RP_WIDE) NL_FORM(RP_WIDE);
@@ -115,7 +121,7 @@
 	if (df) {
 		const int32_t *pc = (const int32_t *)c->pool.get(S_BR_PC, 0);
 		const unsigned nb_rep = df->rode >= 2 ? 0u : df->nb;
-		const LoopFront2 a = { (int)nb_rep, n_vtx, (n_vtx + RK_T - 1) / RK_T, vs, ve, s1, agid, c->br_par.diff, poff, pc + loop_btot_at(n_vtx), pc, pairs, c->br_cap, c->dcnt };
+		const LoopFront2 a = { (int)nb_rep, n_vtx, (n_vtx + RK_T - 1) / RK_T, vs, ve, s1, agid, c->br_par.diff, poff, pc + loop_btot_at(n_vtx), pc, pairs, c->br_cap, c->dcnt, c->br_lazy ? 1 : 0 };
 		const dim3 grid(nb_rep + nblk(n_vtx, BLOCK / WAVE));
 		const int form = c->rp_form;
 		if (df->cleared) {
@@ -129,8 +135,48 @@
 		}
 	} else
 	hipLaunchKernelGGL((k_br_wave<1>), dim3(nblk(n_vtx, BLOCK / WAVE)), dim3(BLOCK), 0, c->st, n_vtx, vs, ve, s1, agid, c->br_par.diff, poff, pairs, c->br_cap, (const int32_t *)c->pool.get(S_BR_PC, 0),
-	                   (const int32_t *)nullptr, 0.0, 0.0, (uint8_t *)nullptr, (int32_t *)nullptr, (int32_t *)nullptr, c->dcnt, (uint8_t *)nullptr, (const int64_t *)nullptr, c->gate);
+	                   (const int32_t *)nullptr, 0.0, 0.0, (uint8_t *)nullptr, (int32_t *)nullptr, (int32_t *)nullptr, c->dcnt, (uint8_t *)nullptr, (const int64_t *)nullptr, c->gate, BrLazy{c->br_lazy ? 1 : 0, nullptr, 0, nullptr, nullptr, nullptr});
 	return n_local_dev(c, pairs, c->br_cap, c->dcnt + 15, c->br_par.local_dist, c->br_par.local_count, c->br_par.frag_mode, cnt);
+}
+
+static inline int64_t *br_res_len(pga_ctx *c) { return c->br_lazy ? (int64_t *)c->pool.get(S_BR_RLEN, sizeof(int64_t) * BR_RSEG * BR_RSTRIDE) : (int64_t *)nullptr; }
+static int br_lazy_args(pga_ctx *c, int n_vtx, BrLazy *lz)
+{
+	*lz = BrLazy{0, nullptr, 0, nullptr, nullptr, nullptr};
+	if (!c->br_lazy) return 0;
+	int shift = 0;
+	while (((int64_t)BR_RSEG << shift) < c->br_rcap) ++shift;
+	c->br_rcap = (int64_t)BR_RSEG << shift;
+	lz->on = 1, lz->seg_shift = shift;
+	lz->rlen = br_res_len(c);
+	lz->rpairs = (int32_t *)c->pool.get(S_RPAIRS, sizeof(int32_t) * 2 * (size_t)c->br_rcap + 16);
+	lz->roff = (int32_t *)c->pool.get(S_BR_ROFF, sizeof(int32_t) * (size_t)n_vtx + 16);
+	lz->rmask = (unsigned long long *)c->pool.get(S_BR_RMASK, sizeof(unsigned long long) * (size_t)n_vtx + 16);
+	return (lz->rpairs && lz->rlen && lz->roff && lz->rmask) ? 0 : PGA_ERR_NOMEM;
+}
+static int branch_residual_counts(pga_ctx *c, const BrLazy &lz, NLocalRide *ride)
+{
+	int32_t *rcnt;
+	return lz.on ? n_local_dev(c, lz.rpairs, c->br_rcap, lz.rlen, c->br_par.local_dist, c->br_par.local_count, c->br_par.frag_mode, &rcnt, S_RNLCNT, std::min<int64_t>(c->br_rcap, std::max<int64_t>(c->br_res_seen, 1 << 12)), lz.seg_shift, ride) : 0;
+}
+static int branch_finish(pga_ctx *c, const BrLazy &lz, int n_vtx, int32_t *ndl)
+{
+	if (!lz.on) return 0;
+	const int32_t *rcnt = (const int32_t *)c->pool.get(S_RNLCNT, 0);
+	if (!rcnt) return PGA_ERR_NOMEM;
+	hipLaunchKernelGGL(k_br_finish, dim3(nblk(n_vtx, BLOCK / WAVE)), dim3(BLOCK), 0, c->st, n_vtx, (const int32_t *)c->pool.get(S_BR_VS, 0), (const int32_t *)c->pool.get(S_BR_VE, 0), rcnt, lz, ndl, c->dcnt, (const int64_t *)(c->dcnt + 15), (int64_t)c->br_cap, c->gate);
+	return 0;
+}
+static int branch_residual(pga_ctx *c, const BrLazy &lz, int n_vtx, int32_t *ndl)
+{
+	TRY(branch_residual_counts(c, lz, nullptr));
+	return branch_finish(c, lz, n_vtx, ndl);
+}
+static inline bool loop_res_cap_forced(const pga_ctx *c) { return getenv("PANGENE_LOOP_RES_CAP") != nullptr && !c->loop_room_given; }
+static void br_res_room(pga_ctx *c)
+{
+	c->br_rcap = std::max<int64_t>(c->br_rcap, std::max<int64_t>((int64_t)1 << 16, c->br_res_seen + c->br_res_seen / 4));
+	if (loop_res_cap_forced(c)) c->br_rcap = std::max<long long>(1, atoll(getenv("PANGENE_LOOP_RES_CAP")));
 }
 
 static int branch_pairs_impl(pga_ctx *c, const uint64_t *arc_x, const int32_t *arc_s1, int64_t n_arc, const int32_t *seg_gid, int32_t n_seg,
@@ -165,12 +211,12 @@
 		const RepFill &rf = df->rf;
 		const int64_t n_clear = (df->cleared && !df->rode) ? rf.n_ent : 0;
 		const int gl = df->rode ? 0 : rf.GL;
-		const LoopFront a = { n_vtx, nbc, gl, vs, ve, s1, branch_diff, pc, poff, pc + loop_btot_at(n_vtx), rf.flags, rf.goff, df->rx, rf.rp_out, n_clear, c->rp_form == RP_COMPACT ? 8 : 16, c->gate };
+		const LoopFront a = { n_vtx, nbc, gl, vs, ve, s1, branch_diff, pc, poff, pc + loop_btot_at(n_vtx), rf.flags, rf.goff, df->rx, rf.rp_out, n_clear, c->rp_form == RP_COMPACT ? 8 : 16, c->gate, br_res_len(c) };
 		hipLaunchKernelGGL(k_loop_front1, dim3((unsigned)(nbc + gl + (n_clear + RK_T - 1) / RK_T)), dim3(RK_T), 0, c->st, a);
 		if (c->br_cap < 4 * (int64_t)n_vtx && !loop_cap_forced(c)) c->br_cap = 4 * (int64_t)n_vtx;
 		return branch_enumerate(c, cnt, df);
 	}
-	hipLaunchKernelGGL(k_br_count, dim3(nblk(n_vtx)), dim3(BLOCK), 0, c->st, n_vtx, vs, ve, s1, branch_diff, pc, c->gate);
+	hipLaunchKernelGGL(k_br_count, dim3(nblk(n_vtx)), dim3(BLOCK), 0, c->st, n_vtx, vs, ve, s1, branch_diff, pc, c->gate, br_res_len(c));
 	if (one_wg) hipLaunchKernelGGL(k_pair_offsets, dim3(1), dim3(PO_THREADS), 0, c->st, (const int32_t *)pc, n_vtx, poff, c->dcnt, c->h_box, n_pairs ? -1ll : loop_cap_forced(c) ? (long long)c->br_cap : (long long)std::max<int64_t>(c->br_cap, 4 * (int64_t)n_vtx), c->gate);
 	else {
 		I32 *tile = (I32 *)c->pool.get(S_TILE, tile_buf_bytes(n_vtx));
@@ -428,8 +474,12 @@
 	}
 	static const bool no_skip = env_has("PANGENE_LOOP", "noskip");
 	const bool gated = !no_skip && (int64_t)c->round_tag + n_round + 4 < (int64_t)HA_TAG_MAX;
-	struct GateScope { pga_ctx *c; ~GateScope() { c->gate = Gate{nullptr, 0}, c->loop_gated = false, c->in_loop = false, c->ride_want = 0, c->ride_done = 0; } } gate_scope{c};
+	struct GateScope { pga_ctx *c; ~GateScope() { c->gate = Gate{nullptr, 0}, c->loop_gated = false, c->in_loop = false, c->br_lazy = false, c->ride_want = 0, c->ride_done = 0; } } gate_scope{c};
 	c->loop_gated = gated, c->in_loop = true;
+	c->br_lazy = !env_has("PANGENE_BR_LAZY", "0") && x == nullptr && !env_has("PANGENE_LOOP_FUSE", "0");
+	if (c->br_lazy) br_res_room(c);
+	BrLazy lz;
+	TRY(br_lazy_args(c, n_vtx, &lz));
 	static const int ride_env = [] { const char *e = getenv("PANGENE_LOOP_RIDE"); const int v = e ? atoi(e) : 2; return v < 0 ? 0 : v > 2 ? 2 : v; }();
 	int ride = 0;
 	c->ride_want = 0, c->ride_done = 0;
@@ -439,7 +489,7 @@
 		if (maxg <= (1 << 15)) ride = ride_env, c->ride_cpg = (int)std::max<int64_t>(1, (maxg + RK_CHUNK - 1) / RK_CHUNK);
 	}
 	const uint32_t tag_before = c->round_tag;
-	HIPCHK(hipMemsetAsync(c->dcnt + 16, 0, sizeof(int64_t), c->st));
+	HIPCHK(hipMemsetAsync(c->dcnt + 16, 0, 3 * sizeof(int64_t), c->st));
 	if (gated) HIPCHK(hipMemsetAsync(c->loopctl, 0xff, 4 * sizeof(int32_t), c->st));
 	static const int live_env = [] { const char *e = getenv("PANGENE_LIVE_LISTS"); return e ? atoi(e) : -1; }();
 	const bool live_ask = live_env != 0 && (live_env == 2 || N >= (1 << 21));
@@ -461,8 +511,12 @@
 			int32_t *sg = (int32_t *)c->pool.get(S_BR_SEGGID, 0), *dg = (int32_t *)c->pool.get(S_DEG, 0), *seg_cnt = (int32_t *)c->pool.get(S_SEGCNT, 0);
 			if (!aw || !vwk || !s1 || !agid || !vs || !ve || !poff || !grp || !sg || !dg || !seg_cnt) return PGA_ERR_NOMEM;
 			hipLaunchKernelGGL((k_br_wave<2>), dim3(nblk(n_vtx, BLOCK / WAVE)), dim3(BLOCK), 0, c->st, n_vtx, vs, ve, s1, agid, par->branch_diff, poff, (int32_t *)nullptr, (int64_t)c->br_cap, (const int32_t *)nullptr, (const int32_t *)c->pool.get(S_NLCNT, 0),
-			                   par->branch_diff_dist, par->branch_diff_cut, aw, grp, ndl, (int64_t *)nullptr, vwk, c->dcnt + 15, c->gate);
-			TRY(pga_mark_hits(c, nullptr, nullptr, 0, nullptr, 1));
+			                   par->branch_diff_dist, par->branch_diff_cut, aw, grp, ndl, (int64_t *)nullptr, vwk, c->dcnt + 15, c->gate, lz);
+			NLocalRide nlr;
+			const bool nl_rides = lz.on && c->NL > 0 && !env_has("PANGENE_BR_LAZY_RIDE", "0");
+			TRY(branch_residual_counts(c, lz, nl_rides ? &nlr : nullptr));
+			TRY(mark_hits_resident(c, nullptr, 1, nl_rides ? &nlr : nullptr));
+			TRY(branch_finish(c, lz, n_vtx, ndl));
 			c->gate = gated ? Gate{c->loopctl, r} : Gate{nullptr, 0};
 			if (r > 0) {
 				hipLaunchKernelGGL(k_round_del, dim3(nblk(S)), dim3(BLOCK), 0, c->st, S, (const int32_t *)ndl, max_tot_cnt[r], max_degree[r], max_dist_loci[r], (const int32_t *)sg, c->g2s, vs, ve, dg, seg_cnt, vwk, alive,
@@ -517,15 +571,15 @@
 		if (!h_ctl) return PGA_ERR_NOMEM;
 		HIPCHK(hipMemcpyAsync(h_ctl, c->loopctl, 4 * sizeof(int32_t), hipMemcpyDeviceToHost, c->st));
 	}
-	const size_t fetch_need = (((size_t)S + 128 + (par->final_on ? 4 * sizeof(int32_t) * (size_t)S + 64 : 0) + 15) & ~(size_t)15) + 64 + 16;
+	const size_t fetch_need = (((size_t)S + 128 + (par->final_on ? 4 * sizeof(int32_t) * (size_t)S + 64 : 0) + 15) & ~(size_t)15) + 64 + 32;
 	if (c->h_fetch_cap < fetch_need) {
 		c->h_fetch = c->pin.get(fetch_need + fetch_need / 2 + 512);
 		if (!c->h_fetch) return PGA_ERR_NOMEM;
 		c->h_fetch_cap = fetch_need + fetch_need / 2 + 512;
 	}
 	HIPCHK(hipMemcpyAsync(c->h_fetch, alive, (size_t)S, hipMemcpyDeviceToHost, c->st));
-	int64_t *h_need = (int64_t *)((char *)c->h_fetch + fetch_need - 16);
-	HIPCHK(hipMemcpyAsync(h_need, c->dcnt + 16, sizeof(int64_t), hipMemcpyDeviceToHost, c->st));
+	int64_t *h_need = (int64_t *)((char *)c->h_fetch + fetch_need - 32);
+	HIPCHK(hipMemcpyAsync(h_need, c->dcnt + 16, 3 * sizeof(int64_t), hipMemcpyDeviceToHost, c->st));
 	int32_t *h_fin = (int32_t *)((char *)c->h_fetch + (((size_t)S + 127) & ~(size_t)63));
 	if (par->final_on) {
 		HIPCHK(hipMemcpyAsync(h_fin, (const int32_t *)c->pool.get(S_SEGCNT, 0), sizeof(int32_t) * (size_t)n_vtx, hipMemcpyDeviceToHost, c->st));
@@ -548,6 +602,10 @@
 	}
 	c->br_np_seen = std::max<int64_t>(c->br_np_seen, c->h_cnt[15]);
 	if (getenv("PANGENE_TIMING")) fprintf(stderr, "[pga_branch_loop] counters after %d rounds: invariant %lld, table overflows (last round) %lld, sticky %lld, pairs (last round) %lld of capacity %lld\n", n_round, (long long)c->h_cnt[3], (long long)c->h_cnt[9], (long long)c->h_cnt[11], (long long)c->h_cnt[15], (long long)c->br_cap);
+	const int64_t res_need = h_need[2] * BR_RSEG;
+	if (c->br_lazy && getenv("PANGENE_TIMING")) fprintf(stderr, "[pga_branch_loop] lazy rounds: the longest segment of a residual list %lld of capacity %lld (%d segments)\n", (long long)h_need[2], (long long)(c->br_rcap / BR_RSEG), BR_RSEG);
+	const bool res_over = c->br_lazy && res_need > c->br_rcap;
+	if (c->br_lazy) c->br_res_seen = std::max<int64_t>(c->br_res_seen, res_need);
 	if (x && par->final_on) c->cur_tab = L.merged, c->cur_tab_n = c->h_cnt[10], c->table_sparse = false;
 	if (x) {
 		const int32_t *f = (const int32_t *)h_x;
@@ -570,6 +628,7 @@
 		const int64_t need = *h_need;
 		if (getenv("PANGENE_TIMING")) fprintf(stderr, "[pga_branch_loop] the longest pair list that did not fit: %lld (capacity %lld)\n", (long long)need, (long long)c->br_cap);
 		if (need > c->br_cap && c->h_cnt[9] == 0 && need + need / 4 <= ((int64_t)1 << 27)) { c->br_cap = need + need / 4, c->loop_room_given = true; return 4; }
+		if (need <= c->br_cap && res_over && c->h_cnt[9] == 0 && res_need + res_need / 4 <= ((int64_t)1 << 27)) { c->br_rcap = res_need + res_need / 4, c->loop_room_given = true; return 4; }
 		return 1;
 	}
 	memcpy(seg_alive, c->h_fetch, (size_t)S);
@@ -579,21 +638,38 @@
 	return 0;
 }
 
+static int mark_hits_resident(pga_ctx *c, int64_t *n_marked, int32_t then_filter, const NLocalRide *ride)
+{
+	TRY(ensure_half_arcs(c, c->ha_ori < 0 ? 0 : c->ha_ori));
+	const uint64_t *ax = (const uint64_t *)c->pool.get(S_ARCX, 0); const uint8_t *aw = (const uint8_t *)c->pool.get(S_ARCW, 0);
+	const int32_t *vs = (const int32_t *)c->pool.get(S_BR_VS, 0), *ve = (const int32_t *)c->pool.get(S_BR_VE, 0);
+	const uint8_t *vwk = (const uint8_t *)c->pool.get(S_VWK, 0);
+	if (!ax || !aw || !vs || !ve || !vwk) return PGA_ERR_NOMEM;
+	if (n_marked) HIPCHK(hipMemsetAsync(c->dcnt + 2, 0, sizeof(int64_t), c->st));
+	const MarkHitsZ a = { c->zx, c->zy, c->zg, c->hfk, c->hbk, c->round_tag, c->NL, c->g2s, ax, aw, vs, ve, vwk, c->flags,
+	                      n_marked ? c->dcnt + 2 : (int64_t *)nullptr, then_filter, n_marked ? Gate{nullptr, 0} : c->gate, c->gate.w ? c->loopctl : (int32_t *)nullptr, c->loop_round };
+	if (ride && ride->nb && c->NL && !n_marked) {
+		const dim3 grid(ride->nb + nblk(c->NL));
+#define MH_LAUNCH(FORM, LANES) hipLaunchKernelGGL((k_mark_hits_nl<FORM, LANES>), grid, dim3(BLOCK), 0, c->st, a, ride->a, (int)ride->nb)
+#define MH_FORM(FORM) do { if (ride->lanes == 16) MH_LAUNCH(FORM, 16); else if (ride->lanes == 32) MH_LAUNCH(FORM, 32); else MH_LAUNCH(FORM, 64); } while (0)
+		if (c->rp_form == RP_COMPACT) MH_FORM(RP_COMPACT);
+		else if (c->rp_form == RP_WIDE) MH_FORM(RP_WIDE);
+		else MH_FORM(RP_FULL);
+#undef MH_FORM
+#undef MH_LAUNCH
+	}
+	else if (c->NL) hipLaunchKernelGGL(k_mark_hits_z, dim3(nblk(c->NL)), dim3(BLOCK), 0, c->st, a);
+	if (then_filter) c->walk_valid = false, c->ha_valid = false;
+	return 0;
+}
+
 extern "C" int pga_mark_hits(pga_ctx_t *c, const uint64_t *arc_x, const uint8_t *arc_weak, int64_t n_arc, int64_t *n_marked, int32_t then_filter)
 {
 	const int N = c->N;
 	if (n_marked) *n_marked = 0;
 	if (N == 0) return 0;
 	if (arc_x == nullptr) {
-		TRY(ensure_half_arcs(c, c->ha_ori < 0 ? 0 : c->ha_ori));
-		const uint64_t *ax = (const uint64_t *)c->pool.get(S_ARCX, 0); const uint8_t *aw = (const uint8_t *)c->pool.get(S_ARCW, 0);
-		const int32_t *vs = (const int32_t *)c->pool.get(S_BR_VS, 0), *ve = (const int32_t *)c->pool.get(S_BR_VE, 0);
-		const uint8_t *vwk = (const uint8_t *)c->pool.get(S_VWK, 0);
-		if (!ax || !aw || !vs || !ve || !vwk) return PGA_ERR_NOMEM;
-		if (n_marked) HIPCHK(hipMemsetAsync(c->dcnt + 2, 0, sizeof(int64_t), c->st));
-		if (c->NL) hipLaunchKernelGGL(k_mark_hits_z, dim3(nblk(c->NL)), dim3(BLOCK), 0, c->st, c->zx, c->zy, c->zg, c->hfk, c->hbk, c->round_tag, c->NL, c->g2s, ax, aw, vs, ve, vwk, c->flags,
-		                   n_marked ? c->dcnt + 2 : (int64_t *)nullptr, then_filter, n_marked ? Gate{nullptr, 0} : c->gate, c->gate.w ? c->loopctl : (int32_t *)nullptr, c->loop_round);
-		if (then_filter) c->walk_valid = false, c->ha_valid = false;
+		TRY(mark_hits_resident(c, n_marked, then_filter, nullptr));
 	} else {
 		uint64_t *ax = (uint64_t *)c->pool.get(S_ARCX, sizeof(uint64_t) * (size_t)n_arc + 16);
 		uint8_t *aw = (uint8_t *)c->pool.get(S_ARCW, (size_t)n_arc + 16);
diff --git a/pangene_amd/csrc/hip/pga_host_context.hpp b/pangene_amd/csrc/hip/pga_host_context.hpp
--- a/pangene_amd/csrc/hip/pga_host_context.hpp
+++ b/pangene_amd/csrc/hip/pga_host_context.hpp
@@ -128,7 +128,7 @@
 enum {
 	S_KEY_A, S_KEY_B, S_VAL_A, S_VAL_B, S_TABLE, S_TILE, S_I32_A, S_I32_B, S_I32_C, S_TAB_A, S_TAB_B, S_TAB_C, S_TAB_D,
 	S_TDIST, S_TS1, S_TS2, S_TGEN, S_SDIST, S_SS1, S_SS2, S_SGEN, S_HEAD, S_SLOT, S_ARCS, S_SEGCNT, S_BITS, S_TRIPLES,
-	S_WALK_VAL, S_WALK_PREV, S_PERM, S_OVPOS, S_OVFILE, S_RUNSTART, S_CDN, S_MG_KEY, S_MG_VAL, S_MG_SRC, S_MG_OUT, S_MG_HEAD, S_MG_SLOT, S_MG_RUN, S_BR_S1, S_BR_GID, S_BR_VS, S_BR_VE, S_BR_PC, S_BR_POFF, S_BR_GRP, S_BR_NDL, S_BR_SEGGID, S_PAIRS, S_NLCNT, S_ARCX, S_ARCW, S_WEAKNEW, S_RP_SEG, S_RP_R, S_RP_CM, S_RP_POS, S_RP_IV, S_DL, S_SCRATCH, S_UPLOAD, S_RAW, S_ARC_STAGE, S_GMETA, S_GOFF, S_DEG, S_BIGLIST, S_STAGE_SID, S_STATS, S_G2S, S_MISC, S_SLOW, S_HZLIST, S_VWK, S_XG_BUF, S_XG_OUT, S_XG_OUT2, S_XSTAT, S_GSLIST, S_UPLOAD2, S_BINS, S_FIN_ID, S_FRONT,
+	S_WALK_VAL, S_WALK_PREV, S_PERM, S_OVPOS, S_OVFILE, S_RUNSTART, S_CDN, S_MG_KEY, S_MG_VAL, S_MG_SRC, S_MG_OUT, S_MG_HEAD, S_MG_SLOT, S_MG_RUN, S_BR_S1, S_BR_GID, S_BR_VS, S_BR_VE, S_BR_PC, S_BR_POFF, S_BR_GRP, S_BR_NDL, S_BR_SEGGID, S_PAIRS, S_NLCNT, S_ARCX, S_ARCW, S_WEAKNEW, S_RP_SEG, S_RP_R, S_RP_CM, S_RP_POS, S_RP_IV, S_DL, S_SCRATCH, S_UPLOAD, S_RAW, S_ARC_STAGE, S_GMETA, S_GOFF, S_DEG, S_BIGLIST, S_STAGE_SID, S_STATS, S_G2S, S_MISC, S_SLOW, S_HZLIST, S_VWK, S_XG_BUF, S_XG_OUT, S_XG_OUT2, S_XSTAT, S_GSLIST, S_UPLOAD2, S_BINS, S_FIN_ID, S_FRONT, S_RPAIRS, S_RNLCNT, S_BR_ROFF, S_BR_RMASK, S_BR_RLEN,
 	S_COUNT
 };
 
@@ -217,6 +217,7 @@
 	unsigned long long sync_epoch = 0, arc_epoch = 0; bool arc_deferred = false, arc_done = false, force_sort_once = false, sweep_done = false; std::vector<int32_t> def_host;
 	int4 *yrecA = 0, *yrecB = 0; bool yrec_valid = false;
 	int64_t br_np_seen = 0;
+	bool br_lazy = false; int64_t br_rcap = 0, br_res_seen = 0;
 	int64_t br_n = 0, br_np = 0, br_cap = 0; int32_t br_S = 0;
 	struct { double diff; int32_t local_dist, local_count, frag_mode; } br_par = { 0, 0, 0, 0 };
 	int32_t *h_ndl = nullptr; size_t h_ndl_cap = 0;
diff --git a/pangene_amd/csrc/hip/pga_host_selftest.hpp b/pangene_amd/csrc/hip/pga_host_selftest.hpp
--- a/pangene_amd/csrc/hip/pga_host_selftest.hpp
+++ b/pangene_amd/csrc/hip/pga_host_selftest.hpp
@@ -198,3 +198,77 @@
 	(void)hipFree(d_sums); (void)hipFree(d_key); (void)hipFree(d_mx); (void)hipFree(d_gid); (void)hipFree(d_rep1); (void)hipFree(d_words); (void)hipFree(d_rep);
 	return 0;
 }
+
+extern "C" int pga_selftest_branch(const int32_t *vs, const int32_t *ve, const int32_t *s1, const int32_t *agid, int32_t n_vtx, int64_t n_arc, const int32_t *rp, int32_t Q, int32_t GL,
+                                   double bd, double bdist, double bcut, int32_t local_dist, int32_t local_count, int32_t lazy, int64_t res_cap, int32_t gate_closed,
+                                   uint8_t *aw, int32_t *ndl, uint8_t *vwk, int64_t *lens)
+{
+	int ndev = 0;
+	if (hipGetDeviceCount(&ndev) != hipSuccess || ndev <= 0) return PGA_ERR_NO_DEVICE;
+	if (n_vtx <= 0 || n_vtx > PO_THREADS * PO_MAX_ITEMS || n_arc <= 0 || Q <= 0 || GL <= 0 || !vs || !ve || !s1 || !agid || !rp || !aw || !ndl || !vwk || !lens) return PGA_ERR_ARG;
+	for (int v = 0; v < n_vtx; ++v) if (vs[v] < 0 || ve[v] < vs[v] || ve[v] > n_arc) return PGA_ERR_ARG;
+	for (int64_t i = 0; i < n_arc; ++i) if (agid[i] < 0 || agid[i] >= Q || s1[i] <= 0) return PGA_ERR_ARG;
+	pga_ctx c;
+	HIPCHK(hipStreamCreateWithFlags(&c.st, hipStreamNonBlocking));
+	TRY(dalloc(&c, &c.dcnt, 24)); TRY(dalloc(&c, &c.loopctl, 4)); TRY(dalloc_commit(&c));
+	HIPCHK(hipHostMalloc((void **)&c.h_cnt, 24 * sizeof(int64_t), hipHostMallocDefault));
+	HIPCHK(hipHostGetDevicePointer((void **)&c.h_box, c.h_cnt, 0));
+	c.n_genome = GL, c.Q = Q, c.rp_form = RP_FULL;
+	c.br_n = n_arc, c.br_S = n_vtx / 2, c.br_np = -1;
+	c.br_par.diff = bd, c.br_par.local_dist = local_dist, c.br_par.local_count = local_count, c.br_par.frag_mode = 0;
+	auto up = [&](int slot, const void *src, size_t bytes) -> void * { void *d = c.pool.get(slot, bytes + 16); if (d && hipMemcpyAsync(d, src, bytes, hipMemcpyHostToDevice, c.st) != hipSuccess) d = nullptr; return d; };
+	int32_t *d_vs = (int32_t *)up(S_BR_VS, vs, sizeof(int32_t) * (size_t)n_vtx), *d_ve = (int32_t *)up(S_BR_VE, ve, sizeof(int32_t) * (size_t)n_vtx);
+	int32_t *d_s1 = (int32_t *)up(S_BR_S1, s1, sizeof(int32_t) * (size_t)n_arc), *d_gid = (int32_t *)up(S_BR_GID, agid, sizeof(int32_t) * (size_t)n_arc);
+	void *d_rp = up(S_RP_SEG, rp, sizeof(int4) * (size_t)Q * (size_t)GL);
+	uint8_t *d_aw = (uint8_t *)up(S_ARCW, aw, (size_t)n_arc), *d_vwk = (uint8_t *)up(S_VWK, vwk, (size_t)n_vtx);
+	int32_t *d_ndl = (int32_t *)up(S_BR_NDL, ndl, sizeof(int32_t) * (size_t)n_vtx);
+	int32_t *pc = (int32_t *)c.pool.get(S_BR_PC, sizeof(int32_t) * (loop_btot_at(n_vtx) + 64) + 16), *poff = (int32_t *)c.pool.get(S_BR_POFF, sizeof(int32_t) * (size_t)n_vtx + 16);
+	int32_t *grp = (int32_t *)c.pool.get(S_BR_GRP, sizeof(int32_t) * (size_t)n_arc + 16);
+	int rc = (d_vs && d_ve && d_s1 && d_gid && d_rp && d_aw && d_vwk && d_ndl && pc && poff && grp && c.pool.get(S_RP_IV, 16)) ? 0 : PGA_ERR_NOMEM;
+	if (rc == 0 && (hipMemsetAsync(c.dcnt, 0, 24 * sizeof(int64_t), c.st) != hipSuccess || hipMemsetAsync(c.loopctl, 0xff, 4 * sizeof(int32_t), c.st) != hipSuccess)) rc = PGA_ERR_NO_DEVICE;
+	int64_t worst = 16;
+	for (int v = 0; v < n_vtx; ++v) worst += (int64_t)(ve[v] - vs[v]) * (ve[v] - vs[v]);
+	c.br_cap = worst;
+	c.gate = gate_closed ? Gate{c.loopctl, 0} : Gate{nullptr, 0};
+	c.br_lazy = lazy != 0;
+	c.br_rcap = res_cap > 0 ? res_cap : (int64_t)1 << 16;
+	if (rc == 0 && c.br_lazy && (!br_res_len(&c) || hipMemsetAsync(br_res_len(&c), 0, sizeof(int64_t) * BR_RSEG * BR_RSTRIDE, c.st) != hipSuccess)) rc = PGA_ERR_NOMEM;
+	int attempt = 0;
+	for (; rc == 0; ++attempt) {
+		BrLazy lz;
+		if ((rc = br_lazy_args(&c, n_vtx, &lz)) != 0) break;
+		(void)hipMemsetAsync(c.dcnt + 11, 0, sizeof(int64_t), c.st);
+		(void)hipMemsetAsync(c.dcnt + 15, 0, 4 * sizeof(int64_t), c.st);
+		hipLaunchKernelGGL(k_br_count, dim3(nblk(n_vtx)), dim3(BLOCK), 0, c.st, n_vtx, (const int32_t *)d_vs, (const int32_t *)d_ve, (const int32_t *)d_s1, bd, pc, c.gate, br_res_len(&c));
+		hipLaunchKernelGGL(k_pair_offsets, dim3(1), dim3(PO_THREADS), 0, c.st, (const int32_t *)pc, n_vtx, poff, c.dcnt, c.h_box, (long long)c.br_cap, c.gate);
+		int32_t *cnt;
+		if ((rc = branch_enumerate(&c, &cnt)) != 0) break;
+		hipLaunchKernelGGL((k_br_wave<2>), dim3(nblk(n_vtx, BLOCK / WAVE)), dim3(BLOCK), 0, c.st, n_vtx, (const int32_t *)d_vs, (const int32_t *)d_ve, (const int32_t *)d_s1, (const int32_t *)d_gid, bd, (const int32_t *)poff, (int32_t *)nullptr, (int64_t)c.br_cap,
+		                   (const int32_t *)nullptr, (const int32_t *)cnt, bdist, bcut, d_aw, grp, d_ndl, (int64_t *)nullptr, d_vwk, (const int64_t *)(c.dcnt + 15), c.gate, lz);
+		if ((rc = branch_residual(&c, lz, n_vtx, d_ndl)) != 0) break;
+		if (hipMemcpyAsync(c.h_cnt, c.dcnt, 24 * sizeof(int64_t), hipMemcpyDeviceToHost, c.st) != hipSuccess || hipStreamSynchronize(c.st) != hipSuccess) { rc = PGA_ERR_NO_DEVICE; break; }
+		if (c.h_cnt[11] && c.br_lazy && c.h_cnt[18] * BR_RSEG > c.br_rcap && attempt == 0) {
+			c.br_rcap = c.h_cnt[18] * BR_RSEG + c.h_cnt[18] * BR_RSEG / 4;
+			(void)hipMemcpyAsync(d_aw, aw, (size_t)n_arc, hipMemcpyHostToDevice, c.st); (void)hipMemcpyAsync(d_vwk, vwk, (size_t)n_vtx, hipMemcpyHostToDevice, c.st);
+			(void)hipMemcpyAsync(d_ndl, ndl, sizeof(int32_t) * (size_t)n_vtx, hipMemcpyHostToDevice, c.st);
+			continue;
+		}
+		++attempt;
+		break;
+	}
+	if (rc == 0) {
+		lens[0] = c.h_cnt[15], lens[1] = 0, lens[2] = attempt, lens[3] = c.h_cnt[11];
+		int64_t seg_len[BR_RSEG] = { 0 };
+		if (c.br_lazy && hipMemcpy2D(seg_len, sizeof(int64_t), br_res_len(&c), sizeof(int64_t) * BR_RSTRIDE, sizeof(int64_t), BR_RSEG, hipMemcpyDeviceToHost) != hipSuccess) rc = PGA_ERR_NO_DEVICE;
+		for (int k = 0; k < BR_RSEG; ++k) lens[1] += seg_len[k];
+		if (hipMemcpy(aw, d_aw, (size_t)n_arc, hipMemcpyDeviceToHost) != hipSuccess || hipMemcpy(vwk, d_vwk, (size_t)n_vtx, hipMemcpyDeviceToHost) != hipSuccess ||
+		    hipMemcpy(ndl, d_ndl, sizeof(int32_t) * (size_t)n_vtx, hipMemcpyDeviceToHost) != hipSuccess) rc = PGA_ERR_NO_DEVICE;
+	}
+	(void)hipStreamSynchronize(c.st);
+	(void)hipHostFree(c.h_cnt); c.h_cnt = nullptr, c.h_box = nullptr;
+	c.pool.release();
+	for (void *q : c.owned) (void)hipFree(q);
+	dev_big_free(c.arena, c.arena_cap), c.arena = nullptr;
+	(void)hipStreamDestroy(c.st); c.st = nullptr;
+	return rc;
+}
```

Result: faster. 244.3 (median of 6 runs) (+7.5%).
